# LiHaoy-ux/DQO-MAP

Hardware: AMD Instinct MI355X
Metric: mapping iters/sec (fwd+bwd raster) @ 500k Gaussians 1200×680; PSNR vs ref (higher is better)
Workload: dtype f32; 1 GPU; cfg3: surfel room, ONE map of 500000 Gaussians, 1200x680, 8 object ids, SH degree 3, per-object render (object gate) + per-object masked loss (sum over objects of 0.8 L1 colour + 1.0 depth L1 on the object's own mask) + attach loss, raster fwd+bwd + Adam (6 groups); path=fused (hipGraph replays of 4 iterations each); rccl_ranks=1, backend=none (one rank), list_split=0, list_split_backward=0, graph_unroll=4, sync_mode=lazy, selfcheck=skipped, P=500000, P_visible=196562, view=room, adam=exact-sparse, adam_rows_touched=148371, attach_loss_members=49997

## Files before the change

dqo-map_amd/_dqo_native.py:

```python
import ctypes
import os

_HERE = os.path.dirname(os.path.abspath(__file__))
LIB_PATH = os.path.join(_HERE, "lib", "libdqoraster.so")

c_f = ctypes.c_float
c_i32 = ctypes.c_int32
c_vp = ctypes.c_void_p


class DqoRastParams(ctypes.Structure):
    _fields_ = [("P", c_i32), ("D", c_i32), ("M", c_i32), ("W", c_i32), ("H", c_i32), ("prefiltered", c_i32), ("debug", c_i32),
                ("tanfovx", c_f), ("tanfovy", c_f), ("cx", c_f), ("cy", c_f), ("scale_modifier", c_f), ("color_sigma", c_f),
                ("opaque_threshold", c_f), ("depth_threshold", c_f), ("normal_threshold", c_f), ("T_threshold", c_f)]


class DqoRastInputs(ctypes.Structure):
    _fields_ = [(n, c_vp) for n in ("bg", "means3D", "shs", "colors_precomp", "opacities", "scales", "rotations", "cov3D_precomp",
                                    "viewmatrix", "projmatrix", "campos", "tile_mask", "row_flags")]


class DqoRastOutputs(ctypes.Structure):
    _fields_ = [(n, c_vp) for n in ("out_color", "out_depth", "out_hit_color", "out_hit_depth", "out_hit_color_weight",
                                    "out_hit_depth_weight", "out_T", "n_touched", "radii")]


class DqoLossTap(ctypes.Structure):
    _fields_ = [("gt_color", c_vp), ("gt_depth", c_vp), ("render_mask", c_vp), ("out_color", c_vp), ("out_depth", c_vp),
                ("color_weight", c_f), ("depth_weight", c_f), ("add_depth_thres", c_f), ("loss_out", c_vp), ("grad_scale", c_vp),
                ("per_object", c_i32)]


class DqoObjectGate(ctypes.Structure):
    _fields_ = [("gaussian_object", c_vp), ("pixel_object", c_vp), ("tile_objects", c_vp)]


class DqoRastCtx(ctypes.Structure):
    _fields_ = [("geom", c_vp), ("geom_bytes", ctypes.c_size_t), ("binning", c_vp), ("binning_bytes", ctypes.c_size_t),
                ("image", c_vp), ("image_bytes", ctypes.c_size_t), ("inst_capacity", ctypes.c_int64), ("tile_bucket_capacity", c_i32), ("keep_tile_order", c_i32), ("loss_tap", c_vp),
                ("object_gate", c_vp), ("list_split", c_i32), ("frame_prezeroed", c_i32)]


class DqoRastGrads(ctypes.Structure):
    _fields_ = [(n, c_vp) for n in ("dL_dmeans3D", "dL_dsh", "dL_dcolors", "dL_dopacity", "dL_dscales", "dL_drotations", "dL_dcov3D",
                                    "dL_dmeans2D")] + [("skip_culled_rows", c_i32)]


class DqoRastParamInputs(ctypes.Structure):
    _fields_ = [("features_dc", c_vp), ("features_rest", c_vp), ("rest", c_i32), ("opacity_raw", c_vp), ("scaling_raw", c_vp),
                ("rotation_raw", c_vp)]


class DqoRastParamGrads(ctypes.Structure):
    _fields_ = [(n, c_vp) for n in ("dL_dfeatures_dc", "dL_dfeatures_rest", "dL_dopacity_raw", "dL_dscaling_raw", "dL_drotation_raw")]


class DqoRastHeader(ctypes.Structure):
    _fields_ = [("num_rendered", ctypes.c_uint32), ("num_tiles", ctypes.c_uint32), ("overflow", ctypes.c_uint32),
                ("max_tile_count", ctypes.c_uint32), ("num_visible", ctypes.c_uint32), ("num_candidates", ctypes.c_uint32),
                ("stage", ctypes.c_uint32), ("reserved", ctypes.c_uint32)]


class DqoProfileEntry(ctypes.Structure):
    _fields_ = [("name", ctypes.c_char * 48), ("total_ms", ctypes.c_double), ("calls", ctypes.c_uint32)]


class DqoAdamStep(ctypes.Structure):
    _fields_ = ([("P", c_i32), ("M", c_i32), ("step", c_i32), ("beta1", c_f), ("beta2", c_f), ("eps", c_f), ("lr_xyz", c_f),
                 ("lr_f_dc", c_f), ("lr_f_rest", c_f), ("lr_opacity", c_f), ("lr_scaling", c_f), ("lr_rotation", c_f)] +
                [(n, c_vp) for n in ("xyz", "shs", "opacity_raw", "scaling_raw", "rotation_raw", "g_means3D", "g_sh", "g_opacity",
                                     "g_scales", "g_rotations", "m_xyz", "m_shs", "m_opacity", "m_scaling", "m_rotation", "v_xyz",
                                     "v_shs", "v_opacity", "v_scaling", "v_rotation", "act_opacity", "act_scales", "act_rotations", "radii", "step_dev", "moment_live",
                                     "attach_mask", "init_xyz", "init_scaling_raw", "init_rotation_raw")] +
                [("attach_count", c_i32), ("attach_partial", c_vp), ("frame_header", c_vp), ("block_ticket", c_vp), ("bias_table", c_vp), ("attach_gains", c_vp),
                 ("row_flags", c_vp), ("confidence", c_vp), ("lr_table", c_vp), ("record_ctx", c_vp), ("record_W", c_i32), ("record_H", c_i32)])

ROW_FROZEN, ROW_HIDDEN = 1, 2


class DqoAdamTensor(ctypes.Structure):
    _fields_ = [("p", c_vp), ("g", c_vp), ("m", c_vp), ("v", c_vp), ("n", ctypes.c_int64), ("lr", ctypes.c_double)]


class DqoLifecycle(ctypes.Structure):
    _fields_ = ([(n, c_i32) for n in ("P", "W", "H", "tick", "unstable_time_window", "delete_thresh", "stable_oversized", "use_votes")] +
                [(n, c_f) for n in ("stable_confidence_thres", "add_color_thres", "add_depth_thres")] +
                [(n, c_vp) for n in ("xyz", "opacity_raw", "scaling_raw", "confidence", "alive", "row_flags", "stable", "add_tick",
                                     "depth_error_counter", "color_error_counter", "park", "vote", "workspace")] +
                [("workspace_bytes", ctypes.c_size_t), ("stats", c_vp), ("render_header", c_vp)])


class DqoGrowthSample(ctypes.Structure):
    _fields_ = ([(n, c_i32) for n in ("W", "H", "first_frame", "uniform_sample_num", "capacity", "key_bits", "M", "identity_rotation")] +
                [("seed", ctypes.c_uint64)] +
                [(n, c_f) for n in ("add_transmission_thres", "add_depth_thres", "add_color_thres", "transmission_sample_ratio",
                                    "error_sample_ratio", "init_opacity")] +
                [(n, c_vp) for n in ("vertex", "normal", "color", "depth", "instance", "T", "render_depth", "render_color", "depth_index",
                                     "xyz", "scales", "rotations", "opacity", "shs", "obj_id", "out_normal", "pixel", "header", "workspace")] +
                [("workspace_bytes", ctypes.c_size_t)])


EXPORTS = ("dqo_abi_version", "dqo_abi_sizeof", "dqo_last_error", "dqo_profile_enable", "dqo_profile_collect", "dqo_map_activate",
           "dqo_map_loss_workspace_bytes", "dqo_map_loss_fwd_bwd", "dqo_map_ssim_workspace_bytes", "dqo_map_ssim_fwd_bwd", "dqo_map_adam_step", "dqo_adam_multi_dev", "dqo_map_attach_workspace_bytes",
           "dqo_map_attach_loss_fwd_bwd", "dqo_adam_multi", "dqo_accumulate_gaussian_error", "dqo_accumulate_gaussian_confidence", "dqo_rast_geom_bytes", "dqo_rast_image_bytes",
           "dqo_rast_binning_bytes", "dqo_rast_binning_bytes_bucketed",
           "dqo_rast_backward_workspace_bytes", "dqo_rast_forward_prepare", "dqo_rast_read_header", "dqo_rast_forward_render",
           "dqo_rast_forward", "dqo_rast_forward_async", "dqo_rast_backward", "dqo_rast_backward_adam", "dqo_mark_visible", "dqo_knn3_workspace_bytes", "dqo_knn3",
           "dqo_quadric_iou_fwd_bwd", "dqo_quadric_adam", "dqo_tile_count_mask", "dqo_transmission_mask", "dqo_tile_color_error", "dqo_knn3_query_workspace_bytes",
           "dqo_knn3_query", "dqo_knn3_query_within", "dqo_knn3_query_grouped", "dqo_icp_workspace_bytes", "dqo_icp_normal_equations",
           "dqo_attach_pixels", "dqo_attach_decide", "dqo_growth_scales", "dqo_growth_inside", "dqo_error_maps", "dqo_map_history_merge",
           "dqo_rast_forward_prepare_params", "dqo_rast_forward_render_params", "dqo_rast_forward_async_params", "dqo_rast_backward_params",
           "dqo_icp_gauss_newton", "dqo_track_preprocess_workspace_bytes", "dqo_track_preprocess", "dqo_track_pyramid_pixels",
           "dqo_track_pyramid_workspace_bytes", "dqo_track_pyramid", "dqo_track_fill_model_depth", "dqo_track_p2p_workspace_bytes",
           "dqo_track_p2p_loss", "dqo_map_lifecycle_workspace_bytes", "dqo_map_lifecycle_vote", "dqo_map_lifecycle_rows",
           "dqo_growth_sample_workspace_bytes", "dqo_growth_sample", "dqo_eval_picture_workspace_bytes", "dqo_eval_picture",
           "dqo_eval_ms_ssim_workspace_bytes", "dqo_eval_ms_ssim",
           "dqo_nn1_workspace_bytes", "dqo_nn1", "dqo_eval_pcd_workspace_bytes", "dqo_eval_pcd", "dqo_window_masks_workspace_bytes",
           "dqo_window_masks")

_lib = None


def lib():
    global _lib
    if _lib is None:
        import torch
        if not os.path.exists(LIB_PATH):
            raise RuntimeError(f"{LIB_PATH} not found: the HIP extension is not built (run __graft_entry__.build()). "
                               "There is no CPU fallback for this operator.")
        L = ctypes.CDLL(LIB_PATH)
        L.dqo_last_error.restype = ctypes.c_char_p
        for n in ("dqo_rast_geom_bytes", "dqo_rast_image_bytes", "dqo_rast_binning_bytes", "dqo_rast_backward_workspace_bytes",
                  "dqo_knn3_workspace_bytes"):
            getattr(L, n).restype = ctypes.c_size_t
        L.dqo_rast_geom_bytes.argtypes = [c_i32, c_i32, c_i32]
        L.dqo_rast_image_bytes.argtypes = [c_i32, c_i32]
        L.dqo_rast_binning_bytes.argtypes = [ctypes.c_int64]
        L.dqo_rast_binning_bytes_bucketed.restype = ctypes.c_size_t
        L.dqo_rast_binning_bytes_bucketed.argtypes = [ctypes.c_int64, c_i32, c_i32, c_i32]
        L.dqo_rast_backward_workspace_bytes.argtypes = [ctypes.c_int64]
        L.dqo_knn3_workspace_bytes.argtypes = [c_i32]
        P = ctypes.POINTER
        L.dqo_rast_forward_prepare.argtypes = [P(DqoRastParams), P(DqoRastInputs), P(DqoRastOutputs), P(DqoRastCtx), c_vp]
        L.dqo_rast_forward_render.argtypes = L.dqo_rast_forward_prepare.argtypes
        L.dqo_rast_forward.argtypes = L.dqo_rast_forward_prepare.argtypes
        L.dqo_rast_forward_async.argtypes = L.dqo_rast_forward_prepare.argtypes[:4] + [c_vp, c_vp, c_vp]
        L.dqo_rast_read_header.argtypes = [P(DqoRastCtx), P(DqoRastHeader), c_vp]
        L.dqo_rast_backward.argtypes = [P(DqoRastParams), P(DqoRastInputs), P(DqoRastCtx), c_vp, c_vp, c_vp, P(DqoRastGrads), c_vp,
                                        ctypes.c_size_t, c_vp]
        L.dqo_rast_backward_adam.argtypes = [P(DqoRastParams), P(DqoRastInputs), P(DqoRastCtx), c_vp, c_vp, P(DqoAdamStep), c_vp,
                                             ctypes.c_size_t, c_vp]
        L.dqo_rast_forward_prepare_params.argtypes = [P(DqoRastParams), P(DqoRastInputs), P(DqoRastParamInputs), P(DqoRastOutputs),
                                                      P(DqoRastCtx), c_vp]
        L.dqo_rast_forward_render_params.argtypes = L.dqo_rast_forward_prepare_params.argtypes
        L.dqo_rast_forward_async_params.argtypes = L.dqo_rast_forward_prepare_params.argtypes[:5] + [c_vp, c_vp, c_vp]
        L.dqo_rast_backward_params.argtypes = [P(DqoRastParams), P(DqoRastInputs), P(DqoRastParamInputs), P(DqoRastCtx), c_vp, c_vp, c_vp,
                                               P(DqoRastGrads), P(DqoRastParamGrads), c_vp, ctypes.c_size_t, c_vp]
        L.dqo_mark_visible.argtypes = [c_i32, c_vp, c_vp, c_vp, c_vp, c_vp]
        L.dqo_knn3.argtypes = [c_i32, c_vp, c_vp, c_vp, c_vp, ctypes.c_size_t, c_vp]
        L.dqo_quadric_iou_fwd_bwd.argtypes = [c_i32] + [c_vp] * 12
        L.dqo_quadric_adam.argtypes = [c_i32, c_i32] + [c_vp] * 9
        L.dqo_map_activate.argtypes = [c_i32] + [c_vp] * 7
        L.dqo_map_loss_workspace_bytes.restype = ctypes.c_size_t
        L.dqo_map_loss_workspace_bytes.argtypes = []
        L.dqo_map_ssim_workspace_bytes.restype = ctypes.c_size_t
        L.dqo_map_ssim_workspace_bytes.argtypes = [c_i32, c_i32]
        L.dqo_map_ssim_fwd_bwd.argtypes = [c_i32, c_i32, c_vp, c_vp, c_f, c_vp, c_vp, c_i32, c_vp, c_vp, ctypes.c_size_t, c_vp]
        L.dqo_map_loss_fwd_bwd.argtypes = [c_i32, c_i32] + [c_vp] * 6 + [c_f, c_f, c_f] + [c_vp] * 4 + [ctypes.c_size_t, c_vp]
        L.dqo_map_adam_step.argtypes = [P(DqoAdamStep), c_vp]
        L.dqo_map_attach_workspace_bytes.restype = ctypes.c_size_t
        L.dqo_map_attach_workspace_bytes.argtypes = [c_i32]
        L.dqo_adam_multi.argtypes = [c_vp, c_i32, c_i32, ctypes.c_double, ctypes.c_double, ctypes.c_double, c_vp]
        L.dqo_adam_multi_dev.argtypes = [c_vp, c_i32, c_vp, c_i32, ctypes.c_double, ctypes.c_double, ctypes.c_double, c_vp]
        L.dqo_map_attach_loss_fwd_bwd.argtypes = [c_i32] + [c_vp] * 7 + [c_i32] + [c_vp] * 5 + [ctypes.c_size_t, c_vp]
        L.dqo_accumulate_gaussian_error.argtypes = [c_i32] * 3 + [c_vp] * 5 + [c_f] * 3 + [c_i32] + [c_vp] * 6
        L.dqo_accumulate_gaussian_confidence.argtypes = [c_i32] * 3 + [c_vp] * 7
        L.dqo_knn3_query_workspace_bytes.restype = ctypes.c_size_t
        L.dqo_knn3_query_workspace_bytes.argtypes = [c_i32, c_i32]
        L.dqo_knn3_query.argtypes = [c_i32, c_vp, c_i32, c_vp, c_vp, c_vp, c_vp, ctypes.c_size_t, c_vp]
        L.dqo_knn3_query_within.argtypes = [c_i32, c_vp, c_i32, c_vp, c_f, c_vp, c_vp, c_vp, ctypes.c_size_t, c_vp]
        L.dqo_knn3_query_grouped.argtypes = [c_i32, c_vp, c_vp, c_i32, c_vp, c_vp, c_vp, c_f, c_vp, c_vp, c_vp, ctypes.c_size_t, c_vp]
        L.dqo_attach_pixels.argtypes = [c_i32, c_vp, c_vp, c_f, c_f, c_f, c_f, c_i32, c_i32] + [c_vp] * 5
        L.dqo_attach_decide.argtypes = [c_i32] + [c_vp] * 10 + [c_f, c_f, c_vp, c_vp]
        L.dqo_growth_scales.argtypes = [c_i32] + [c_vp] * 7 + [c_f, c_f, c_f, c_vp, c_vp, c_vp]
        L.dqo_growth_inside.argtypes = [c_i32] + [c_vp] * 5
        L.dqo_error_maps.argtypes = [c_i32, c_i32] + [c_vp] * 9
        L.dqo_icp_workspace_bytes.restype = ctypes.c_size_t
        L.dqo_icp_workspace_bytes.argtypes = []
        L.dqo_icp_normal_equations.argtypes = [c_i32, c_i32] + [c_vp] * 5 + [c_f] * 6 + [c_vp] * 4 + [ctypes.c_size_t, c_vp]
        L.dqo_icp_gauss_newton.argtypes = [c_i32, c_i32] + [c_vp] * 6 + [c_f] * 4 + [c_vp] * 2 + [ctypes.c_size_t, c_vp]
        L.dqo_track_preprocess_workspace_bytes.restype = ctypes.c_size_t
        L.dqo_track_preprocess_workspace_bytes.argtypes = [c_i32, c_i32]
        L.dqo_track_preprocess.argtypes = [c_i32, c_i32, c_vp, c_vp] + [c_f] * 3 + [c_i32] + [c_vp] * 6 + [ctypes.c_size_t, c_vp]
        L.dqo_track_pyramid_pixels.restype = ctypes.c_int64
        L.dqo_track_pyramid_pixels.argtypes = [c_i32, c_i32, c_i32]
        L.dqo_track_pyramid_workspace_bytes.restype = ctypes.c_size_t
        L.dqo_track_pyramid_workspace_bytes.argtypes = []
        L.dqo_track_pyramid.argtypes = [c_i32, c_i32, c_i32] + [c_vp] * 5 + [ctypes.c_size_t, c_vp]
        L.dqo_track_fill_model_depth.argtypes = [c_i32, c_i32] + [c_vp] * 4 + [c_f, c_f, c_vp]
        L.dqo_track_p2p_workspace_bytes.restype = ctypes.c_size_t
        L.dqo_track_p2p_workspace_bytes.argtypes = []
        L.dqo_track_p2p_loss.argtypes = [c_i32, c_i32] + [c_vp] * 4 + [c_f] + [c_vp] * 5 + [ctypes.c_size_t, c_vp]
        L.dqo_tile_count_mask.argtypes = [c_i32, c_i32, c_vp, c_vp, c_vp]
        L.dqo_transmission_mask.argtypes = [c_i32, c_i32, c_vp, c_vp, c_vp, c_vp, c_vp]
        L.dqo_tile_color_error.argtypes = [c_i32, c_i32, c_vp, c_vp, c_vp, c_vp, c_vp]
        L.dqo_window_masks_workspace_bytes.restype = ctypes.c_size_t
        L.dqo_window_masks_workspace_bytes.argtypes = [c_i32, c_i32]
        L.dqo_window_masks.argtypes = [c_i32, c_i32, c_i32, c_vp, c_vp, c_vp, c_f, c_i32, c_vp, c_vp, c_vp, c_vp, c_vp, ctypes.c_size_t, c_vp]
        L.dqo_map_history_merge.argtypes = [c_i32, c_i32, c_f, c_i32] + [c_vp] * 12
        L.dqo_map_lifecycle_workspace_bytes.restype = ctypes.c_size_t
        L.dqo_map_lifecycle_workspace_bytes.argtypes = [c_i32]
        L.dqo_map_lifecycle_vote.argtypes = [P(DqoLifecycle)] + [c_vp] * 7
        L.dqo_map_lifecycle_rows.argtypes = [P(DqoLifecycle), c_vp]
        L.dqo_growth_sample_workspace_bytes.restype = ctypes.c_size_t
        L.dqo_growth_sample_workspace_bytes.argtypes = [c_i32, c_i32]
        L.dqo_growth_sample.argtypes = [P(DqoGrowthSample), c_vp]
        L.dqo_eval_picture_workspace_bytes.restype = ctypes.c_size_t
        L.dqo_eval_picture_workspace_bytes.argtypes = [c_i32, c_i32]
        L.dqo_eval_picture.argtypes = [c_i32, c_i32] + [c_vp] * 5 + [c_f, c_f, c_vp, c_vp, c_i32, c_vp, ctypes.c_size_t, c_vp]
        L.dqo_eval_ms_ssim_workspace_bytes.restype = ctypes.c_size_t
        L.dqo_eval_ms_ssim_workspace_bytes.argtypes = [c_i32, c_i32]
        L.dqo_eval_ms_ssim.argtypes = [c_i32, c_i32, c_vp, c_vp, c_vp, c_vp, c_i32, c_vp, ctypes.c_size_t, c_vp]
        L.dqo_nn1_workspace_bytes.restype = ctypes.c_size_t
        L.dqo_nn1_workspace_bytes.argtypes = [c_i32, c_i32]
        L.dqo_nn1.argtypes = [c_i32, c_vp, c_vp, c_i32] + [c_vp] * 7 + [ctypes.c_size_t, c_vp]
        L.dqo_eval_pcd_workspace_bytes.restype = ctypes.c_size_t
        L.dqo_eval_pcd_workspace_bytes.argtypes = [c_i32, c_i32]
        L.dqo_eval_pcd.argtypes = [c_i32, c_vp, c_vp, c_i32, c_vp, c_vp, c_vp, c_i32, ctypes.POINTER(c_f), c_vp, c_i32, c_vp, ctypes.c_size_t, c_vp]
        L.dqo_profile_enable.argtypes = [ctypes.c_int]
        L.dqo_profile_collect.argtypes = [P(DqoProfileEntry), ctypes.c_int, ctypes.c_int]
        if L.dqo_abi_version() != 5:
            raise RuntimeError("libdqoraster.so ABI version mismatch")
        L.dqo_abi_sizeof.restype = ctypes.c_size_t
        L.dqo_abi_sizeof.argtypes = [c_i32]
        for k, st in enumerate((DqoRastParams, DqoRastInputs, DqoRastOutputs, DqoRastCtx, DqoRastGrads, DqoRastHeader, DqoProfileEntry,
                                DqoAdamStep, DqoLossTap, DqoObjectGate, DqoAdamTensor, DqoRastParamInputs, DqoRastParamGrads, None,
                                DqoLifecycle, DqoGrowthSample)):
            if st is not None and L.dqo_abi_sizeof(k) != ctypes.sizeof(st):
                raise RuntimeError(f"libdqoraster.so: struct {st.__name__} is {L.dqo_abi_sizeof(k)} bytes in the library, "
                                   f"{ctypes.sizeof(st)} in the binding")
        _lib = L
    return _lib


def check(rc):
    if rc != 0:
        raise RuntimeError(lib().dqo_last_error().decode() or f"libdqoraster error {rc}")


def ptr(t):
    if t is None or t.numel() == 0:
        return None
    return t.data_ptr()


def require_gpu(*tensors):
    for t in tensors:
        if t is not None and t.numel() > 0 and not t.is_cuda:
            raise RuntimeError("libdqoraster operators need GPU (ROCm) tensors; there is no CPU path. Got a tensor on "
                               f"{t.device}.")


def current_stream():
    import torch
    return torch.cuda.current_stream().cuda_stream


def profile_enable(on):
    lib().dqo_profile_enable(1 if on else 0)


def profile_collect(reset=True):
    buf = (DqoProfileEntry * 64)()
    n = lib().dqo_profile_collect(buf, 64, 1 if reset else 0)
    return {buf[i].name.decode(): (buf[i].total_ms, buf[i].calls) for i in range(n)}
```

dqo-map_amd/csrc/dqo_capi.hip:

```cpp
#include <stdarg.h>
#include <stdio.h>
#include <string.h>

#include "dqo_common.h"

static thread_local char g_err[512] = "";

void dqo_set_error(const char* fmt, ...) {
    va_list ap;
    va_start(ap, fmt);
    vsnprintf(g_err, sizeof(g_err), fmt, ap);
    va_end(ap);
}

int dqo_launch_mark_visible(int P, const float* means3D, const float* view, const float* proj, uint8_t* present, hipStream_t s);
int dqo_launch_knn3(int P, const float* xyz, float* mean_d2, int32_t* idx3, void* ws, size_t ws_bytes, hipStream_t s);
size_t dqo_knn3_ws_bytes(int P);
size_t dqo_knn3_query_ws_bytes(int Q, int R);
int dqo_launch_knn3_query(int Q, const float* q_xyz, int R, const float* r_xyz, float* dist2, int32_t* idx3, void* ws, size_t ws_bytes,
                          hipStream_t s, float bound2, const int32_t* q_group = nullptr, const int32_t* r_group = nullptr,
                          const float* group_box = nullptr);
int dqo_launch_quadric_iou(int B, const float* axes, const float* R, const float* center, const float* P34, const float* obs,
                           float* bbox, float* loss, int32_t* valid, float* g_axes, float* g_R, float* g_center, hipStream_t s);
int dqo_launch_quadric_adam(int n_obj, int n_iters, const int32_t* view_offset, const float* P34_views, const float* obs_views,
// ... 23 lines not shown
size_t dqo_icp_ws_bytes(void);
int dqo_launch_icp(int H, int W, const float* vertex0, const float* vertex1, const float* normal0, const float* normal1, const float* pose10,
                   float fx, float fy, float cx, float cy, float dist_thr, float normal_thr, float* JtJ, float* JtR, int32_t* valid_count,
                   void* ws, hipStream_t s);
int dqo_launch_icp_gauss_newton(int H, int W, const float* vertex0, const float* vertex1, const float* normal0, const float* normal1, float* pose10,
                                const float* K, float k_scale, float dist_thr, float normal_thr, float damping, int32_t* valid_count, void* ws,
                                hipStream_t s);
size_t dqo_track_preprocess_ws_bytes(int H, int W);
int dqo_launch_track_preprocess(int H, int W, const float* depth, const float* K, float min_depth, float max_depth,
                                float conf_thr, int filter, float* depth_out, float* vertex_out, float* normal_out, float* conf_out,
                                uint8_t* invalid_out, void* ws, hipStream_t s);
size_t dqo_track_pyramid_ws_bytes(void);
int64_t dqo_track_pyramid_pixel_count(int H, int W, int levels);
int dqo_launch_track_pyramid(int H, int W, int levels, const float* depth, const float* K, float* vertex, float* normal,
                             void* ws, hipStream_t s);
int dqo_launch_track_fill(int H, int W, float* render_depth, const float* frame_depth, const float* render_normal, const float* frame_normal,
                          float dist_thr, float normal_thr, hipStream_t s);
size_t dqo_track_p2p_ws_bytes(void);
int dqo_launch_track_p2p(int H, int W, const float* vertex0, const float* vertex1, const float* normal0, const float* pose10, float fail_thr,
                         const int32_t* valid_count, float* loss, int32_t* success, float* valid_ratio, void* ws, hipStream_t s);
int dqo_launch_tile_count(int W, int H, int mode, const uint8_t* mask_in, const float* T_map, uint8_t* mask_out, int32_t* tile_count,
                          int32_t* total, hipStream_t s);
int dqo_launch_tile_color_error(int W, int H, const float* render, const float* gt, float* err_px, float* tile_sum, hipStream_t s);
size_t dqo_window_masks_ws_bytes(int W, int H);
int dqo_launch_window_masks(int W, int H, int mode, const float* T_map, const float* render, const float* gt, float tile_mask_ratio, int k,
                            uint8_t* render_mask, int32_t* tile_mask, float* ratio_out, const DqoRastHeader* header, void* ws, hipStream_t s);
int dqo_launch_growth_scales(int n, const float* xyz, const int32_t* obj, const float* radius, const int32_t* i_new, const float* d2_old,
                             const int32_t* i_old, const float* extra_radius, float reach2, float min_radius, float max_radius, float* scales,
                             uint8_t* invalid, hipStream_t s);
int dqo_launch_growth_inside(int n, const float* d2, const int32_t* idx, const float* radius, uint8_t* inside, hipStream_t s);
int dqo_launch_error_maps(int64_t HW, const float* gt_color, const float* gt_depth, const float* render, const float* depth,
                          const int32_t* depth_index, const uint8_t* mask, float* color_err, float* depth_err, hipStream_t s);
size_t dqo_lifecycle_ws_bytes(int64_t P);
int dqo_launch_lifecycle_vote(const DqoLifecycle* a, const float* gt_color, const float* gt_depth, const float* render, const float* depth,
                              const int32_t* depth_index, const int32_t* color_index, hipStream_t s);
int dqo_launch_lifecycle_rows(const DqoLifecycle* a, hipStream_t s);
size_t dqo_sample_ws_bytes(int64_t HW);
int dqo_launch_growth_sample(const DqoGrowthSample* a, hipStream_t s);
size_t dqo_nn1_ws_bytes(int Q, int R);
int dqo_launch_nn1(int Q, const float* q_xyz, const uint8_t* q_keep, int R, const float* r_xyz, const uint8_t* r_keep, const float* q_xform,
                   const float* r_xform, float* dist2, int32_t* idx, void* ws, hipStream_t s);
size_t dqo_eval_pcd_ws_bytes(int n_gt, int n_rec);
int dqo_launch_eval_pcd(int n_gt, const float* gt_xyz, const uint8_t* gt_keep, int n_rec, const float* rec_xyz, const uint8_t* rec_keep,
                        const float* rec_xform, int n_thres, const float* thres, float* out_row, void* ws, hipStream_t s);
size_t dqo_eval_ws_bytes(int64_t HW);
size_t dqo_msssim_ws_bytes(int W, int H);
int dqo_launch_msssim(int W, int H, const float* render, const float* gt_color, const DqoRastHeader* header, float* out_row, void* ws,
                      hipStream_t s);
int dqo_launch_eval_picture(int W, int H, const float* render, const float* gt_color, const float* depth, const float* gt_depth,
                            const int32_t* depth_index, float min_depth, float max_depth, const DqoRastHeader* header, float* out_row,
                            void* ws, hipStream_t s);
int dqo_launch_attach_pixels(int n, const float* xyz, const float* V, float fx, float fy, float cx, float cy, int W, int H,
                             const int32_t* pixel_object, int32_t* lin, int32_t* sparse, unsigned long long* tile_objects, hipStream_t s);
int dqo_launch_attach_decide(int n, const float* xyz, const float* opacity, const int32_t* obj, const int32_t* lin, const int32_t* hit_index,
                             const float* hit_weight, const float* sxyz, const float* scaling_raw, const float* rotation_raw,
                             const int32_t* gobj, float plane_thr, float opacity_low, uint8_t* out, hipStream_t s);
int dqo_launch_tap_report(const DqoGeomLayout& g, const DqoTapDev& tap, hipStream_t s);
int dqo_launch_accumulate_confidence(int H, int W, int P, const int32_t* index, const float* confidence, float* gmax, float* gmin,
                                     float* gmean, int32_t* counter, hipStream_t s);
int dqo_launch_accumulate_error(int H, int W, int P, const float* color_err, const float* depth_err, const float* normal_err,
                                const int32_t* color_index, const int32_t* depth_index, float color_thr, float depth_thr,
                                float normal_thr, int check_max, float* gs_color, float* gs_depth, float* gs_normal, float* rescale,
                                int32_t* counters, hipStream_t s);

#include <map>
#include <mutex>
#include <string>
#include <vector>
int g_dqo_profile_on = 0;
namespace {
std::mutex g_profile_mu;
struct Pending {
    std::string name;
    hipEvent_t start, stop;
};
std::vector<Pending> g_pending;
std::vector<hipEvent_t> g_event_pool;
std::map<std::string, std::pair<double, uint32_t>> g_profile_acc;
hipEvent_t take_event() {
    if (!g_event_pool.empty()) {
        hipEvent_t e = g_event_pool.back();
        g_event_pool.pop_back();
        return e;
    }
    hipEvent_t e;
    (void)hipEventCreate(&e);
    return e;
}
}
static thread_local size_t t_pending_idx = 0;
void dqo_profile_before(const char* name, hipStream_t s) {
    std::lock_guard<std::mutex> lk(g_profile_mu);
    Pending p{name, take_event(), take_event()};
    (void)hipEventRecord(p.start, s);
    t_pending_idx = g_pending.size();
    g_pending.push_back(p);
}
void dqo_profile_after(hipStream_t s) {
    std::lock_guard<std::mutex> lk(g_profile_mu);
    if (t_pending_idx < g_pending.size()) (void)hipEventRecord(g_pending[t_pending_idx].stop, s);
}

extern "C" {

#define DQO_API __attribute__((visibility("default")))

DQO_API int dqo_profile_enable(int on) {
    g_dqo_profile_on = on ? 1 : 0;
    return DQO_OK;
}

DQO_API int dqo_profile_collect(DqoProfileEntry* out, int max_entries, int reset) {
    std::lock_guard<std::mutex> lk(g_profile_mu);
    for (auto& p : g_pending) {
        float ms = 0.f;
        if (hipEventSynchronize(p.stop) == hipSuccess && hipEventElapsedTime(&ms, p.start, p.stop) == hipSuccess) {
            auto& a = g_profile_acc[p.name];
            a.first += ms;
            a.second += 1;
        }
        g_event_pool.push_back(p.start);
        g_event_pool.push_back(p.stop);
    }
    g_pending.clear();
    int n = 0;
    for (auto& kv : g_profile_acc) {
        if (n >= max_entries || out == nullptr) break;
        strncpy(out[n].name, kv.first.c_str(), sizeof(out[n].name) - 1);
        out[n].name[sizeof(out[n].name) - 1] = 0;
        out[n].total_ms = kv.second.first;
        out[n].calls = kv.second.second;
        n++;
    }
    if (reset) g_profile_acc.clear();
    return n;
}

DQO_API int dqo_abi_version(void) { return DQO_ABI_VERSION; }
DQO_API size_t dqo_abi_sizeof(int32_t which) {
    static const size_t sz[] = {sizeof(DqoRastParams), sizeof(DqoRastInputs), sizeof(DqoRastOutputs), sizeof(DqoRastCtx), sizeof(DqoRastGrads),
                                sizeof(DqoRastHeader), sizeof(DqoProfileEntry), sizeof(DqoAdamStep), sizeof(DqoLossTap), sizeof(DqoObjectGate),
                                sizeof(DqoAdamTensor), sizeof(DqoRastParamInputs), sizeof(DqoRastParamGrads), 0 ,
                                sizeof(DqoLifecycle), sizeof(DqoGrowthSample)};
    return (which >= 0 && which < (int32_t)(sizeof(sz) / sizeof(sz[0]))) ? sz[which] : 0;
}
DQO_API const char* dqo_last_error(void) { return g_err; }

DQO_API size_t dqo_rast_geom_bytes(int32_t P, int32_t W, int32_t H) {
    (void)W;
    (void)H;
    return dqo_geom_layout(nullptr, P < 0 ? 0 : P).total;
}
DQO_API size_t dqo_rast_image_bytes(int32_t W, int32_t H) { return dqo_image_layout(nullptr, W, H).total; }
DQO_API size_t dqo_rast_binning_bytes(int64_t cap) { return dqo_bin_layout(nullptr, cap < 0 ? 0 : cap, cap < 0 ? 0 : cap, 0).total; }
DQO_API size_t dqo_rast_binning_bytes_bucketed(int64_t cap, int32_t W, int32_t H, int32_t bucket) {
    if (cap < 0) cap = 0;
    if (bucket <= 0 || W <= 0 || H <= 0) return dqo_rast_binning_bytes(cap);
    return dqo_bin_layout(nullptr, cap, dqo_list_cap(cap, W, H, bucket), bucket).total;
}
DQO_API size_t dqo_rast_backward_workspace_bytes(int64_t cap) { return dqo_bwd_ws_bytes(cap); }

static int check_common(const DqoRastParams* p, const DqoRastInputs* in, const DqoRastCtx* ctx) {
    DQO_CHECK_ARG(p && in && ctx, "null params / inputs / ctx");
    DQO_CHECK_ARG(p->P >= 0 && p->W > 0 && p->H > 0, "bad sizes P=%d W=%d H=%d", p->P, p->W, p->H);
    DQO_CHECK_ARG(p->D >= 0 && p->D <= 3, "sh degree %d out of range 0..3", p->D);
    DQO_CHECK_ARG((p->W + DQO_TILE - 1) / DQO_TILE < 65536 && (p->H + DQO_TILE - 1) / DQO_TILE < 65536, "image too large");
    DQO_CHECK_ARG(in->viewmatrix && in->projmatrix && in->campos && in->bg, "viewmatrix/projmatrix/campos/bg must be given");
    if (p->P > 0) {
        DQO_CHECK_ARG(in->means3D && in->opacities, "means3D / opacities missing");
        DQO_CHECK_ARG((in->shs != nullptr) != (in->colors_precomp != nullptr),
                      "Please provide excatly one of either SHs or precomputed colors!");
        DQO_CHECK_ARG(in->cov3D_precomp == nullptr,
                      "cov3D_precomp is not supported by the depth rasteriser: its blend kernel reads scales/rotations (forward.cu:780)");
        DQO_CHECK_ARG(in->scales && in->rotations, "scales and rotations are required");
        if (in->shs) DQO_CHECK_ARG(p->M >= (p->D + 1) * (p->D + 1), "sh has %d coefficients, degree %d needs %d", p->M, p->D, (p->D + 1) * (p->D + 1));
        if (in->colors_precomp == nullptr && p->M == 0) {
            dqo_set_error("For non-RGB, provide precomputed Gaussian colors!");
            return DQO_ERR_INVALID_ARG;
        }
    }
    DQO_CHECK_ARG(ctx->geom && ctx->geom_bytes >= dqo_rast_geom_bytes(p->P, p->W, p->H), "geom buffer too small (%zu < %zu)",
                  ctx->geom_bytes, dqo_rast_geom_bytes(p->P, p->W, p->H));
    DQO_CHECK_ARG(ctx->image && ctx->image_bytes >= dqo_rast_image_bytes(p->W, p->H), "image buffer too small (%zu < %zu)",
                  ctx->image_bytes, dqo_rast_image_bytes(p->W, p->H));
    return DQO_OK;
}

static int check_outputs(const DqoRastParams* p, const DqoRastOutputs* o) {
    DQO_CHECK_ARG(o, "null outputs");
    DQO_CHECK_ARG(o->out_color && o->out_depth && o->out_hit_color && o->out_hit_depth && o->out_hit_color_weight &&
                      o->out_hit_depth_weight && o->out_T,
                  "null image output");
    if (p->P > 0) DQO_CHECK_ARG(o->n_touched && o->radii, "null n_touched / radii");
    return DQO_OK;
}

DQO_API int dqo_rast_forward_prepare(const DqoRastParams* p, const DqoRastInputs* in, DqoRastOutputs* out, DqoRastCtx* ctx, void* stream) {
    int rc = check_common(p, in, ctx);
    if (rc) return rc;
    rc = check_outputs(p, out);
    if (rc) return rc;
    rc = dqo_launch_forward_prepare(p, in, out, ctx, (hipStream_t)stream);
    if (rc) return rc;
    return dqo_launch_mark_header_stage0(p, ctx, (hipStream_t)stream);
}

DQO_API int dqo_rast_read_header(const DqoRastCtx* ctx, DqoRastHeader* host_out, void* stream) {
    DQO_CHECK_ARG(ctx && ctx->geom && host_out, "null ctx / out");
    static thread_local uint32_t buf[128 + 64 * DQO_SPREAD];
    DQO_CHECK_HIP(hipMemcpyAsync(buf, ctx->geom, sizeof(buf), hipMemcpyDeviceToHost, (hipStream_t)stream));
    DQO_CHECK_HIP(hipStreamSynchronize((hipStream_t)stream));
    memcpy(host_out, buf, sizeof(DqoRastHeader));
    if (host_out->stage == 2u) return host_out->overflow ? DQO_ERR_OVERFLOW : DQO_OK;
    uint32_t nv = 0, nc = 0;
    for (int j = 0; j < DQO_SPREAD; j++) nv += buf[128 + 64 * j], nc += buf[128 + 64 * j + 1];
    memset(host_out, 0, sizeof(*host_out));
    host_out->stage = 1u;
    host_out->num_visible = nv;
    host_out->num_candidates = nc;
    return host_out->overflow ? DQO_ERR_OVERFLOW : DQO_OK;
}

static int check_render(const DqoRastParams* p, const DqoRastInputs* in, DqoRastOutputs* out, DqoRastCtx* ctx) {
    int rc = check_common(p, in, ctx);
    if (rc) return rc;
    rc = check_outputs(p, out);
    if (rc) return rc;
    DQO_CHECK_ARG(ctx->inst_capacity >= 0 && ctx->inst_capacity < (int64_t)0xffffffffll, "bad inst_capacity");
    DQO_CHECK_ARG(ctx->inst_capacity == 0 || ctx->binning, "null binning buffer");
    DQO_CHECK_ARG(ctx->tile_bucket_capacity >= 0, "negative tile_bucket_capacity");
    DQO_CHECK_ARG(ctx->loss_tap == nullptr || (ctx->loss_tap->gt_color && ctx->loss_tap->gt_depth && ctx->loss_tap->loss_out &&
                                               ctx->loss_tap->grad_scale), "loss tap with a null pointer");
    DQO_CHECK_ARG(ctx->object_gate == nullptr || (ctx->object_gate->gaussian_object && ctx->object_gate->pixel_object),
                  "object gate with a null pointer");
    DQO_CHECK_ARG(ctx->loss_tap == nullptr || !ctx->loss_tap->per_object || ctx->object_gate, "a per-object loss tap needs the object gate");
    if (ctx->binning_bytes < dqo_rast_binning_bytes_bucketed(ctx->inst_capacity, p->W, p->H, ctx->tile_bucket_capacity)) {
        dqo_set_error("binning buffer too small (%zu < %zu)", ctx->binning_bytes,
                      dqo_rast_binning_bytes_bucketed(ctx->inst_capacity, p->W, p->H, ctx->tile_bucket_capacity));
        return DQO_ERR_WORKSPACE;
    }
    return DQO_OK;
}

DQO_API int dqo_rast_forward_render(const DqoRastParams* p, const DqoRastInputs* in, DqoRastOutputs* out, DqoRastCtx* ctx, void* stream) {
    const int rc = check_render(p, in, out, ctx);
    if (rc) return rc;
    return dqo_launch_forward_render(p, in, out, ctx, (hipStream_t)stream);
}

DQO_API int dqo_rast_forward(const DqoRastParams* p, const DqoRastInputs* in, DqoRastOutputs* out, DqoRastCtx* ctx, void* stream) {
    int rc = check_render(p, in, out, ctx);
    if (rc) return rc;
    rc = dqo_launch_forward_prepare(p, in, out, ctx, (hipStream_t)stream);
    if (rc) return rc;
    return dqo_launch_forward_render(p, in, out, ctx, (hipStream_t)stream);
}

DQO_API int dqo_rast_forward_async(const DqoRastParams* p, const DqoRastInputs* in, DqoRastOutputs* out, DqoRastCtx* ctx,
                                   DqoRastHeader* header_host, void* header_event, void* stream) {
    int rc = check_render(p, in, out, ctx);
    if (rc) return rc;
    rc = dqo_launch_forward_prepare(p, in, out, ctx, (hipStream_t)stream);
    if (rc) return rc;
    return dqo_launch_forward_render(p, in, out, ctx, (hipStream_t)stream, header_host, (hipEvent_t)header_event);
}

static int rast_backward(const DqoRastParams* p, const DqoRastInputs* in, const DqoRastCtx* ctx, const float* dL_dcolor, const float* dL_ddepth,
                         const int32_t* hit_image, DqoRastGrads* g, void* ws, size_t ws_bytes, hipStream_t stream, const DqoShRest* pf,
                         float* dL_drest) {
    int rc = check_common(p, in, ctx);
    if (rc) return rc;
    DQO_CHECK_ARG(g, "null grads");
    if (p->P == 0) {
        if (ctx->loss_tap == nullptr) return DQO_OK;
        return dqo_launch_tap_report(dqo_geom_layout(ctx->geom, 0), dqo_tap_dev(ctx->loss_tap), (hipStream_t)stream);
    }
    DQO_CHECK_ARG((dL_dcolor && dL_ddepth) || ctx->loss_tap, "null upstream gradients");
    DQO_CHECK_ARG(ctx->loss_tap == nullptr || (ctx->loss_tap->gt_color && ctx->loss_tap->gt_depth && ctx->loss_tap->out_color &&
                                               ctx->loss_tap->out_depth && ctx->loss_tap->loss_out && ctx->loss_tap->grad_scale),
                  "loss tap with a null pointer");
    DQO_CHECK_ARG(g->dL_dmeans3D && g->dL_dopacity && g->dL_dscales && g->dL_drotations, "null gradient output");
    DQO_CHECK_ARG(p->M == 0 || g->dL_dsh, "null dL_dsh");
    DQO_CHECK_ARG(ctx->binning || ctx->inst_capacity == 0, "null binning buffer");
    if (ws_bytes < dqo_rast_backward_workspace_bytes(ctx->inst_capacity) || (ws == nullptr && ctx->inst_capacity > 0)) {
        dqo_set_error("backward workspace too small (%zu < %zu)", ws_bytes, dqo_rast_backward_workspace_bytes(ctx->inst_capacity));
        return DQO_ERR_WORKSPACE;
    }
    return dqo_launch_backward(p, in, ctx, dL_dcolor, dL_ddepth, hit_image, g, ws, ws_bytes, stream, pf, dL_drest);
}

DQO_API int dqo_rast_backward(const DqoRastParams* p, const DqoRastInputs* in, const DqoRastCtx* ctx, const float* dL_dcolor,
                              const float* dL_ddepth, const int32_t* hit_image, DqoRastGrads* g, void* ws, size_t ws_bytes, void* stream) {
    return rast_backward(p, in, ctx, dL_dcolor, dL_ddepth, hit_image, g, ws, ws_bytes, (hipStream_t)stream, nullptr, nullptr);
}

static int pf_inputs(const DqoRastParams* p, const DqoRastInputs* in, const DqoRastParamInputs* pin, DqoRastParams* p2, DqoRastInputs* in2,
                     DqoShRest* rest) {
    DQO_CHECK_ARG(p && in && pin, "null params / inputs / parameter inputs");
    DQO_CHECK_ARG(in->shs == nullptr && in->opacities == nullptr && in->scales == nullptr && in->rotations == nullptr,
                  "parameter form: DqoRastInputs.shs / opacities / scales / rotations must be NULL (they come from DqoRastParamInputs)");
    DQO_CHECK_ARG(in->colors_precomp == nullptr, "parameter form: colors_precomp is not supported");
    DQO_CHECK_ARG(pin->rest >= 0, "parameter form: negative rest coefficient count %d", pin->rest);
    DQO_CHECK_ARG(p->M == 1 + pin->rest, "parameter form: params M = %d, must be 1 + rest = %d", p->M, 1 + pin->rest);
    DQO_CHECK_ARG(p->D < 0 || p->D > 3 || 1 + pin->rest >= (p->D + 1) * (p->D + 1),
                  "parameter form: features_rest has %d coefficients, degree %d needs %d", pin->rest, p->D, (p->D + 1) * (p->D + 1) - 1);
    if (p->P > 0) {
// ... 610 lines not shown
```

dqo-map_amd/csrc/dqo_common.h:

```cpp
#pragma once
#include <hip/hip_runtime.h>
#include <stdint.h>

#include "../../include/dqo_raster.h"
#include "dqo_activate.h"

#define DQO_TILE 16
#define DQO_WAVE 64
#define DQO_SPREAD 64
#define DQO_GATE_OBJECTS 64
#define DQO_OBJ_SPREAD 16
#ifndef DQO_TSTRIDE
#define DQO_TSTRIDE 64
#endif

void dqo_set_error(const char* fmt, ...);
#define DQO_CHECK_ARG(cond, ...)          \
    do {                                  \
        if (!(cond)) {                    \
            dqo_set_error(__VA_ARGS__);   \
            return DQO_ERR_INVALID_ARG;   \
        }                                 \
    } while (0)
#define DQO_CHECK_HIP(expr)                                                          \
// ... 57 lines not shown
    float4* grad_sum;
    size_t total;
};

static inline DqoGeomLayout dqo_geom_layout(void* base, int64_t P) {
    DqoGeomLayout L;
    char* p = (char*)base;
    auto take = [&](size_t bytes) {
        char* r = p;
        p += dqo_align_up(bytes, 256);
        return r;
    };
    L.header = (DqoRastHeader*)take(256);
    L.counters = (uint32_t*)take(256);
    L.spread = (uint32_t*)take(256 * DQO_SPREAD);
    L.obj_tap = (unsigned long long*)take(sizeof(unsigned long long) * 4 * DQO_GATE_OBJECTS * DQO_OBJ_SPREAD);
    L.conic_opacity = (float4*)take(sizeof(float4) * P);
    L.xy_depth = (float4*)take(sizeof(float4) * P);
    L.rgb_smax = (float4*)take(sizeof(float4) * P);
    L.normal_c = (float4*)take(sizeof(float4) * P);
    L.point_c = (float4*)take(sizeof(float4) * P);
    L.drgb_dir = (float4*)take(sizeof(float4) * 3 * P);
    L.rect16 = (uint2*)take(sizeof(uint2) * P);
    L.tiles_touched = (uint32_t*)take(sizeof(uint32_t) * P);
    L.slot_base = (uint32_t*)take(sizeof(uint32_t) * P);
    L.clamped = (uint8_t*)take(P);
    L.grad_sum = (float4*)take(sizeof(float4) * 4 * P);
    L.total = (size_t)(p - (char*)base);
    return L;
}

struct DqoTapDev {
    const float* gt_color;
    const float* gt_depth;
    const uint8_t* mask;
    const float* out_color;
    const float* out_depth;
    float color_weight, depth_weight, add_depth_thres;
    float* loss_out;
    float* scale;
    int per_object;
};
struct DqoGateDev {
    const int32_t* gobj;
    const int32_t* pobj;
};
static inline DqoGateDev dqo_gate_dev(const DqoObjectGate* g) {
    DqoGateDev d;
    d.gobj = g ? g->gaussian_object : nullptr, d.pobj = g ? g->pixel_object : nullptr;
    return d;
}
static inline DqoTapDev dqo_tap_dev(const DqoLossTap* t) {
    DqoTapDev d;
    d.per_object = 0;
    if (t == nullptr) {
        d.gt_color = d.gt_depth = d.out_color = d.out_depth = nullptr, d.mask = nullptr, d.loss_out = d.scale = nullptr;
        d.color_weight = d.depth_weight = d.add_depth_thres = 0.f;
        return d;
    }
    d.per_object = t->per_object;
    d.gt_color = t->gt_color, d.gt_depth = t->gt_depth, d.mask = t->render_mask, d.out_color = t->out_color, d.out_depth = t->out_depth;
    d.color_weight = t->color_weight, d.depth_weight = t->depth_weight, d.add_depth_thres = t->add_depth_thres;
    d.loss_out = t->loss_out, d.scale = t->grad_scale;
    return d;
}
constexpr double DQO_TAP_FIXED = 4294967296.0;
#ifdef __HIPCC__
typedef unsigned dqo_swap_uint2 __attribute__((ext_vector_type(2)));
template <int D>
__device__ __forceinline__ uint32_t dqo_lane_xor(uint32_t x, int lane) {
    if constexpr (D == 1) return (uint32_t)__builtin_amdgcn_update_dpp(0, (int)x, 0xB1, 0xF, 0xF, false);
    else if constexpr (D == 2) return (uint32_t)__builtin_amdgcn_update_dpp(0, (int)x, 0x4E, 0xF, 0xF, false);
    else if constexpr (D == 4) {
        const int t = __builtin_amdgcn_update_dpp(0, (int)x, 0x104, 0xF, 0x5, false);
        return (uint32_t)__builtin_amdgcn_update_dpp(t, (int)x, 0x114, 0xF, 0xA, false);
    } else if constexpr (D == 8) return (uint32_t)__builtin_amdgcn_update_dpp(0, (int)x, 0x128, 0xF, 0xF, false);
    else if constexpr (D == 16) {
        const dqo_swap_uint2 r = __builtin_amdgcn_permlane16_swap(x, x, false, false);
        return (lane & 16) ? r.x : r.y;
    } else {
        static_assert(D == 32, "power of two up to 32");
        const dqo_swap_uint2 r = __builtin_amdgcn_permlane32_swap(x, x, false, false);
        return (lane & 32) ? r.x : r.y;
    }
}
__device__ __forceinline__ float dqo_wave_sum_xor(float x, int lane) {
    x += __uint_as_float(dqo_lane_xor<32>(__float_as_uint(x), lane));
    x += __uint_as_float(dqo_lane_xor<16>(__float_as_uint(x), lane));
    x += __uint_as_float(dqo_lane_xor<8>(__float_as_uint(x), lane));
    x += __uint_as_float(dqo_lane_xor<4>(__float_as_uint(x), lane));
    x += __uint_as_float(dqo_lane_xor<2>(__float_as_uint(x), lane));
    x += __uint_as_float(dqo_lane_xor<1>(__float_as_uint(x), lane));
    return x;
}
__device__ __forceinline__ uint32_t dqo_wave_max_u32(uint32_t x, int lane) {
    x = max(x, dqo_lane_xor<32>(x, lane)), x = max(x, dqo_lane_xor<16>(x, lane)), x = max(x, dqo_lane_xor<8>(x, lane));
    x = max(x, dqo_lane_xor<4>(x, lane)), x = max(x, dqo_lane_xor<2>(x, lane)), x = max(x, dqo_lane_xor<1>(x, lane));
    return x;
}
__device__ __forceinline__ uint32_t dqo_wave_sum_u32(uint32_t x, int lane) {
    x += dqo_lane_xor<32>(x, lane), x += dqo_lane_xor<16>(x, lane), x += dqo_lane_xor<8>(x, lane);
    x += dqo_lane_xor<4>(x, lane), x += dqo_lane_xor<2>(x, lane), x += dqo_lane_xor<1>(x, lane);
    return x;
}
template <int D>
__device__ __forceinline__ double dqo_lane_xor_f64(double x, int lane) {
    return __hiloint2double((int)dqo_lane_xor<D>((uint32_t)__double2hiint(x), lane), (int)dqo_lane_xor<D>((uint32_t)__double2loint(x), lane));
}
__device__ __forceinline__ double dqo_wave_sum_f64(double x, int lane) {
    x += dqo_lane_xor_f64<32>(x, lane), x += dqo_lane_xor_f64<16>(x, lane), x += dqo_lane_xor_f64<8>(x, lane);
    x += dqo_lane_xor_f64<4>(x, lane), x += dqo_lane_xor_f64<2>(x, lane), x += dqo_lane_xor_f64<1>(x, lane);
    return x;
}
__device__ __forceinline__ void dqo_tap_counts(const uint32_t* spread, int lane, uint32_t& n_col, uint32_t& n_dep) {
    uint32_t a = 0u, b = 0u;
    for (int j = lane; j < DQO_SPREAD; j += 64) {
        const unsigned long long* l = reinterpret_cast<const unsigned long long*>(spread + (size_t)j * 64 + 8);
        a += (uint32_t)l[1], b += (uint32_t)l[3];
    }
    n_col = dqo_wave_sum_u32(a, lane), n_dep = dqo_wave_sum_u32(b, lane);
}
__device__ __forceinline__ void dqo_tap_totals(const uint32_t* spread, int lane, double tot[4]) {
    unsigned long long t[4] = {0ull, 0ull, 0ull, 0ull};
    for (int j = lane; j < DQO_SPREAD; j += 64) {
        const unsigned long long* l = reinterpret_cast<const unsigned long long*>(spread + (size_t)j * 64 + 8);
#pragma unroll
        for (int c = 0; c < 4; c++) t[c] += l[c];
    }
#pragma unroll
    for (int off = 32; off > 0; off >>= 1)
#pragma unroll
        for (int c = 0; c < 4; c++) t[c] += (unsigned long long)__shfl_xor((long long)t[c], off);
    tot[0] = (double)t[0] / DQO_TAP_FIXED, tot[1] = (double)t[1], tot[2] = (double)t[2] / DQO_TAP_FIXED, tot[3] = (double)t[3];
}
__device__ __forceinline__ unsigned long long dqo_tap_fixed(float s) {
    return (s >= 0.f && s < 2147483648.f) ? (unsigned long long)((double)s * DQO_TAP_FIXED + 0.5) : ~0ull >> 1;
}
#endif

static inline int dqo_list_split(const DqoRastCtx* ctx) { return ctx->list_split <= 0 ? 0 : (ctx->list_split < 64 ? 64 : ctx->list_split); }
struct DqoImageLayout {
    uint32_t* tile_count;
    uint32_t* tile_flag;
    uint32_t* tile_cursor;
    uint2* ranges;
    uint32_t* walk4;
    uint32_t* tile_order;
    uint4* slot_info;
    float* final_T;
    uint32_t* n_contrib;
    uint32_t* hit_pos;
    uint32_t* long_tiles;
    uint32_t* split_tiles;
    size_t total;
};

static inline DqoImageLayout dqo_image_layout(void* base, int W, int H) {
    DqoImageLayout L;
    const size_t gx = (W + DQO_TILE - 1) / DQO_TILE, gy = (H + DQO_TILE - 1) / DQO_TILE;
    const size_t T = gx * gy, HW = (size_t)W * H;
    char* p = (char*)base;
    auto take = [&](size_t bytes) {
        char* r = p;
        p += dqo_align_up(bytes, 256);
        return r;
    };
    L.tile_count = (uint32_t*)take(4 * T * DQO_TSTRIDE);
    L.tile_flag = (uint32_t*)take(4 * T);
    L.tile_cursor = (uint32_t*)take(4 * T * DQO_TSTRIDE);
    L.ranges = (uint2*)take(8 * T);
    L.walk4 = (uint32_t*)take(16 * T);
    L.tile_order = (uint32_t*)take(4 * 8 * ((T + 7) / 8));
    L.slot_info = (uint4*)take(16 * 8 * ((T + 7) / 8));
    L.final_T = (float*)take(4 * HW);
    L.n_contrib = (uint32_t*)take(4 * HW);
    L.hit_pos = (uint32_t*)take(4 * HW);
    L.long_tiles = (uint32_t*)take(4 * T);
    L.split_tiles = (uint32_t*)take(4 * T);
    L.total = (size_t)(p - (char*)base);
    return L;
}

struct DqoBinLayout {
    uint4* recs;
    uint32_t* point_list;
    uint32_t* slot_list;
    uint8_t* live_q;
    uint2* slot_info;
    uint32_t* slot_gid;
    uint32_t* rec_valid;
    int64_t list_cap;
    int32_t bucket;
    size_t total;
};
static inline int64_t dqo_list_cap(int64_t cap, int W, int H, int bucket) {
    const int64_t T = (int64_t)((W + DQO_TILE - 1) / DQO_TILE) * ((H + DQO_TILE - 1) / DQO_TILE);
    return bucket > 0 ? T * bucket : cap;
}

static inline DqoBinLayout dqo_bin_layout(void* base, int64_t cap, int64_t list_cap, int bucket) {
    DqoBinLayout L;
    L.list_cap = list_cap, L.bucket = bucket;
    char* p = (char*)base;
    auto take = [&](size_t bytes) {
        char* r = p;
        p += dqo_align_up(bytes, 256);
        return r;
    };
    L.recs = (uint4*)take(16 * (size_t)list_cap);
    L.point_list = (uint32_t*)take(4 * (size_t)list_cap);
    L.slot_list = (uint32_t*)take(4 * (size_t)list_cap);
    L.live_q = (uint8_t*)take(4 * (size_t)list_cap);
    L.slot_info = (uint2*)take(8 * (size_t)cap);
    L.slot_gid = (uint32_t*)take(4 * (size_t)cap);
    L.rec_valid = (uint32_t*)take(4 * (size_t)cap);
    L.total = (size_t)(p - (char*)base);
    return L;
}

struct __attribute__((aligned(16))) DqoGradRec {
    float dcolor[3];
    float m1[2];
    float m2[3];
    float m0;
    float hit[5];
    float pad[2];
};
static_assert(sizeof(DqoGradRec) == 64, "record must be one 64-byte line");

static inline size_t dqo_bwd_recs_bytes(int64_t cap) { return dqo_align_up(sizeof(DqoGradRec) * 4 * (size_t)(cap < 0 ? 0 : cap), 256); }
static inline size_t dqo_bwd_ws_bytes(int64_t cap) { return dqo_bwd_recs_bytes(cap) + 256; }

__host__ __device__ static inline int dqo_spread_index(int logical, int P) {
    const int G = (P + 15) >> 4;
    const int rows = (G + 15) >> 4;
    const int L = logical >> 4;
    const int phys = (L & 15) * rows + (L >> 4);
    return phys < G ? phys * 16 + (logical & 15) : P;
}

static inline int dqo_spread_blocks(int P) {
    const int G = (P + 15) >> 4, rows = (G + 15) >> 4;
    return (rows * 16 * 16 + 255) / 256;
}

struct DqoView {
    const float* view;
    const float* proj;
    const float* campos;
    const float* bg;
    float tanfovx, tanfovy, focal_x, focal_y, cx, cy;
    float scale_mod, color_sigma, opaque_thr, depth_thr, normal_thr, T_thr;
    int W, H, gx, gy;
    int P, D, M;
    const uint8_t* row_flags;
};

struct DqoK1Late {
    DqoView v;
    const float *means3D, *scales, *rotations, *shs, *colors_precomp;
    int first_block;
};

static inline DqoView dqo_make_view(const DqoRastParams* p, const DqoRastInputs* in) {
    DqoView v;
    v.view = in->viewmatrix;
    v.row_flags = in->row_flags;
    v.proj = in->projmatrix;
    v.campos = in->campos;
    v.bg = in->bg;
    v.tanfovx = p->tanfovx;
    v.tanfovy = p->tanfovy;
    v.focal_y = p->H / (2.0f * p->tanfovy);
    v.focal_x = p->W / (2.0f * p->tanfovx);
    v.cx = p->cx;
    v.cy = p->cy;
    v.scale_mod = p->scale_modifier;
    v.color_sigma = p->color_sigma;
    v.opaque_thr = p->opaque_threshold;
    v.depth_thr = p->depth_threshold;
    v.normal_thr = p->normal_threshold;
    v.T_thr = p->T_threshold;
    v.W = p->W;
    v.H = p->H;
    v.gx = (p->W + DQO_TILE - 1) / DQO_TILE;
    v.gy = (p->H + DQO_TILE - 1) / DQO_TILE;
    v.P = p->P;
    v.D = p->D;
    v.M = p->M;
    return v;
}

static inline size_t dqo_frame_scalar_words(const DqoRastCtx* ctx) {
    const size_t obj_words = (ctx->loss_tap != nullptr && ctx->loss_tap->per_object)
                                 ? sizeof(unsigned long long) * 4 * DQO_GATE_OBJECTS * DQO_OBJ_SPREAD / 4 : 0;
    return (256 + 256 * DQO_SPREAD) / 4 + obj_words;
}

#define DQO_CLEARED_STAMP 0xC1EA5EDu
bool dqo_fuse_k1(const DqoRastParams* p, const DqoRastCtx* ctx);

__device__ __forceinline__ void dqo_header_from_spread(const DqoGeomLayout& g, int64_t capacity, int bucket, int lane) {
    uint32_t nv = 0, nc = 0, mx = 0, nt = 0, total = 0;
    for (int j = lane; j < DQO_SPREAD; j += 64) {
        const uint32_t* line = g.spread + (size_t)j * 64;
        nv += line[0], nc += line[1], mx = max(mx, line[2]), nt += line[3], total += line[4] + line[5];
    }
#pragma unroll
    for (int off = 32; off > 0; off >>= 1) {
        nv += __shfl_xor((int)nv, off), nc += __shfl_xor((int)nc, off), nt += __shfl_xor((int)nt, off);
        total += __shfl_xor((int)total, off);
        mx = max(mx, (uint32_t)__shfl_xor((int)mx, off));
    }
    if (lane == 0) {
        DqoRastHeader h;
        h.num_rendered = total;
        h.num_tiles = nt;
        (void)capacity;
        h.overflow = (g.counters[7] != 0u || g.counters[8] != 0u || mx > (uint32_t)bucket) ? 1u : 0u;
        h.max_tile_count = mx;
        h.num_visible = nv;
        h.num_candidates = nc;
        h.stage = 2u, h.reserved = 0u;
        *g.header = h;
    }
}

bool dqo_skip_long_sort(const DqoRastParams* p, const DqoRastCtx* ctx);

int dqo_launch_zero_words(uint32_t* p, size_t n_words, hipStream_t s);

int dqo_launch_bin_count_k1(const DqoView& v, const DqoRastInputs* in, const DqoRastOutputs* out, const int32_t* gobj, const DqoGeomLayout& g,
                            const DqoImageLayout& img, const DqoBinLayout& bin, int64_t capacity, const unsigned long long* tile_objects,
                            hipStream_t s, bool pf = false);
int dqo_launch_forward_prepare(const DqoRastParams* p, const DqoRastInputs* in, DqoRastOutputs* out, DqoRastCtx* ctx, hipStream_t s,
                               const DqoShRest* pf = nullptr);
int dqo_launch_mark_header_stage0(const DqoRastParams* p, DqoRastCtx* ctx, hipStream_t s);
int dqo_launch_forward_render(const DqoRastParams* p, const DqoRastInputs* in, DqoRastOutputs* out, DqoRastCtx* ctx, hipStream_t s,
                              DqoRastHeader* header_host = nullptr, hipEvent_t header_event = nullptr, const DqoShRest* pf = nullptr);
int dqo_launch_backward(const DqoRastParams* p, const DqoRastInputs* in, const DqoRastCtx* ctx, const float* dL_dcolor,
                        const float* dL_ddepth, const int32_t* hit_image, DqoRastGrads* g, void* ws, size_t ws_bytes, hipStream_t s,
                        const DqoShRest* pf = nullptr, float* dL_drest = nullptr);
```

dqo-map_amd/csrc/rast_binning.hip:

```cpp
#include "dqo_common.h"
#include "dqo_cull.h"
#include "dqo_k1_early.h"

namespace {

constexpr int BIN_THREADS = 256;
constexpr int BIN_CHUNK = BIN_THREADS;
constexpr int BIN_WINDOW = 16384;
constexpr int BIN_FLIGHT = 4;
#ifndef BIN_WAVES
#define BIN_WAVES 8
#endif

__device__ __forceinline__ uint32_t lane_id() { return __builtin_amdgcn_mbcnt_hi(~0u, __builtin_amdgcn_mbcnt_lo(~0u, 0u)); }

__device__ __forceinline__ uint32_t popcount_range(const uint32_t* bits, uint32_t a, uint32_t b) {
    if (a >= b) return 0;
    uint32_t wa = a >> 5, wb = (b - 1) >> 5;
    const uint32_t ma = ~0u << (a & 31), mb = ~0u >> (31 - ((b - 1) & 31));
    if (wa == wb) return __popc(bits[wa] & ma & mb);
    uint32_t n = __popc(bits[wa] & ma) + __popc(bits[wb] & mb);
    for (uint32_t w = wa + 1; w < wb; w++) n += __popc(bits[w]);
    return n;
}

__device__ __forceinline__ uint32_t block_exclusive_scan(uint32_t v, uint32_t* s_wave, uint32_t lane, uint32_t wave, uint32_t* total) {
    uint32_t incl = v;
    incl += (uint32_t)__builtin_amdgcn_update_dpp(0, (int)incl, 0x111, 0xF, 0xF, false);
    incl += (uint32_t)__builtin_amdgcn_update_dpp(0, (int)incl, 0x112, 0xF, 0xF, false);
    incl += (uint32_t)__builtin_amdgcn_update_dpp(0, (int)incl, 0x114, 0xF, 0xF, false);
    incl += (uint32_t)__builtin_amdgcn_update_dpp(0, (int)incl, 0x118, 0xF, 0xF, false);
    incl += (uint32_t)__builtin_amdgcn_update_dpp(0, (int)incl, 0x142, 0xA, 0xF, false);
    incl += (uint32_t)__builtin_amdgcn_update_dpp(0, (int)incl, 0x143, 0xC, 0xF, false);
    __syncthreads();
    if (lane == 63) s_wave[wave] = incl;
    __syncthreads();
    uint32_t wbase = 0, tot = 0;
#pragma unroll
    for (uint32_t w = 0; w < BIN_THREADS / 64; w++) {
        const uint32_t t = s_wave[w];
        if (w < wave) wbase += t;
        tot += t;
    }
    *total = tot;
    return wbase + incl - v;
}

struct Cand {
    int gi, tile;
};

struct DqoK1Raw {
    DqoView v;
    const float *means3D, *scales, *rotations, *opacities;
    const int32_t* gobj;
    int32_t *radii_out, *n_touched_out;
};

template <bool K1, bool PF>
__global__ __launch_bounds__(BIN_THREADS, BIN_WAVES) void bin_count_kernel(int P, int gx, const int32_t* __restrict__ tile_mask, DqoGeomLayout g,
                                                                uint32_t* __restrict__ tile_count, uint32_t* __restrict__ tile_flag,
                                                                DqoBinLayout bin, int64_t capacity,
                                                                const unsigned long long* __restrict__ tile_objects, const DqoK1Raw k1,
                                                                const uint8_t* __restrict__ row_flags) {
    static_assert(K1 || !PF, "the parameter form only differs in the early part");
    __shared__ uint32_t s_off[BIN_CHUNK + 1];
    __shared__ uint2 s_rect[BIN_CHUNK];
    __shared__ float4 s_con[BIN_CHUNK];
    __shared__ float4 s_xyq[BIN_CHUNK];
    __shared__ uint32_t s_cnt[BIN_CHUNK];
    __shared__ uint32_t s_prev[BIN_CHUNK];
    __shared__ uint32_t s_gb[BIN_CHUNK];
    __shared__ uint32_t s_bits[BIN_WINDOW / 32];
    __shared__ uint32_t s_wave[BIN_THREADS / 64];
    __shared__ uint32_t s_base;
    __shared__ int s_gobj[BIN_CHUNK];
    const int tid = threadIdx.x;
    const uint32_t lane = lane_id(), wave = tid >> 6;
    const int chunk0 = blockIdx.x * BIN_CHUNK;
    const int my_idx = dqo_spread_index(chunk0 + tid, P);

    uint32_t area = 0;
    {
        uint2 rc = make_uint2(0u, 0u);
        float4 co = make_float4(0.f, 0.f, 0.f, 0.f), xy = co;
        if constexpr (K1) {
            float view[16], proj[16];
#pragma unroll
            for (int i = 0; i < 16; i++) view[i] = k1.v.view[i], proj[i] = k1.v.proj[i];
            if (blockIdx.x == 0 && tid == 0) {
                g.header->stage = 1u;
                if (g.counters[9] != DQO_CLEARED_STAMP) atomicOr(&g.counters[8], 1u);
                g.counters[9] = 0u;
            }
            bool vis = false;
            uint32_t ncand = 0;
            if (my_idx < P) {
                const K1Early e = k1_early<false, PF>(k1.v, view, proj, 0.f, 0.f, 0.f, my_idx, k1.means3D, k1.scales, k1.rotations, k1.opacities,
                                                  nullptr, nullptr, k1.gobj, g, k1.radii_out, k1.n_touched_out, DqoShRest{});
                rc = make_uint2((uint32_t)e.rminx | ((uint32_t)e.rmaxx << 16), (uint32_t)e.rminy | ((uint32_t)e.rmaxy << 16));
                co = e.co, xy = e.xy;
                ncand = (uint32_t)((e.rmaxx - e.rminx) * (e.rmaxy - e.rminy));
                area = ncand;
                vis = e.radius > 0;
            }
            const uint32_t nv = (uint32_t)__popcll(__builtin_amdgcn_ballot_w64(vis));
            const uint32_t nc = dqo_wave_sum_u32(ncand, (int)lane);
            if (lane == 0 && (nv | nc) != 0u) {
                uint32_t* const my_line = g.spread + (size_t)((blockIdx.x * (BIN_THREADS / 64) + wave) % DQO_SPREAD) * 64;
                if (nv) atomicAdd(&my_line[0], nv);
                if (nc) atomicAdd(&my_line[1], nc);
            }
        } else if (my_idx < P) {
            rc = g.rect16[my_idx];
            co = g.conic_opacity[my_idx];
            xy = g.xy_depth[my_idx];
            area = ((rc.x >> 16) - (rc.x & 0xffffu)) * ((rc.y >> 16) - (rc.y & 0xffffu));
        }
        s_rect[tid] = rc;
        if (area) {
            s_con[tid] = co;
            s_xyq[tid] = make_float4(xy.x, xy.y, dqo_q_threshold(co.w), xy.z);
            s_gobj[tid] = __float_as_int(xy.w);
        }
        s_cnt[tid] = 0;
        s_prev[tid] = 0;
    }
    uint32_t total;
    const uint32_t my_off = block_exclusive_scan(area, s_wave, lane, wave, &total);
    s_off[tid] = my_off;
    if (tid == BIN_THREADS - 1) s_off[BIN_CHUNK] = total;
    __syncthreads();
    if (total == 0) {
        if (my_idx < P) g.tiles_touched[my_idx] = 0, g.slot_base[my_idx] = 0;
        return;
    }

    auto decode = [&](uint32_t w) {
        int lo = 0, hi = BIN_CHUNK;
        while (hi - lo > 1) {
            const int mid = (lo + hi) >> 1;
            if (s_off[mid] <= w) lo = mid;
            else hi = mid;
        }
        const uint32_t r = w - s_off[lo];
        const uint2 rc = s_rect[lo];
        const uint32_t minx = rc.x & 0xffffu, rw = (rc.x >> 16) - minx, miny = rc.y & 0xffffu;
        const uint32_t ry = r / rw, rx = r - ry * rw;
        Cand c;
        c.gi = lo;
        c.tile = (int)((miny + ry) * (uint32_t)gx + minx + rx);
        return c;
    };
    auto cull_window = [&](uint32_t win, uint32_t wend, bool flag_dead) {
        for (int i = tid; i < BIN_WINDOW / 32; i += BIN_THREADS) s_bits[i] = 0;
        __syncthreads();
        for (uint32_t w = win + tid; w < wend; w += BIN_THREADS) {
            const Cand c = decode(w);
            if (tile_mask != nullptr && !tile_mask[c.tile]) continue;
            const float4 co = s_con[c.gi], xyq = s_xyq[c.gi];
            const int x = c.tile % gx, y = c.tile / gx;
            bool live = dqo_splat_hits_rect(xyq.x, xyq.y, co.x, co.y, co.z, xyq.z, (float)(x * DQO_TILE), (float)(y * DQO_TILE),
                                            (float)(x * DQO_TILE + DQO_TILE - 1), (float)(y * DQO_TILE + DQO_TILE - 1));
            if (tile_objects != nullptr) live = live && ((tile_objects[c.tile] >> (s_gobj[c.gi] & 63)) & 1ull) != 0ull;
            if (live) {
                atomicOr(&s_bits[(w - win) >> 5], 1u << ((w - win) & 31));
            } else if (flag_dead && tile_flag[c.tile] == 0u) {
                tile_flag[c.tile] = 1u;
            }
        }
        __syncthreads();
    };
    auto carry_window = [&](uint32_t win, uint32_t wend, uint32_t* acc) {
        const uint32_t a = max(my_off, win), b = min(my_off + area, wend);
        if (a < b) acc[tid] += popcount_range(s_bits, a - win, b - win);
    };

    const bool one_window = total <= (uint32_t)BIN_WINDOW;
    for (uint32_t win = 0; win < total; win += BIN_WINDOW) {
        const uint32_t wend = min(total, win + (uint32_t)BIN_WINDOW);
        cull_window(win, wend, true);
        carry_window(win, wend, s_cnt);
        if (!one_window) __syncthreads();
    }
    const bool no_slots = bin.bucket > 0 && row_flags != nullptr && my_idx < P && (row_flags[my_idx] & DQO_ROW_FROZEN) != 0u;
    const uint32_t my_cnt = no_slots ? 0u : s_cnt[tid];
    __shared__ uint8_t s_noslot[BIN_CHUNK];
    s_noslot[tid] = no_slots ? (uint8_t)1 : (uint8_t)0;
    if (row_flags != nullptr && bin.bucket > 0) {
        const uint32_t nf = dqo_wave_sum_u32(no_slots ? s_cnt[tid] : 0u, (int)lane);
        if (lane == 0 && nf != 0u) atomicAdd(&g.spread[(size_t)((blockIdx.x * (BIN_THREADS / 64) + wave) % DQO_SPREAD) * 64 + 5], nf);
    }
    uint32_t block_live;
    const uint32_t my_gb = block_exclusive_scan(my_cnt, s_wave, lane, wave, &block_live);
    s_gb[tid] = my_gb;
    if (tid == 0) {
        if (block_live == 0u) {
            s_base = 0u;
        } else if (bin.bucket <= 0) {
            s_base = atomicAdd(&g.counters[0], block_live);
        } else {
            const uint32_t regions = min((uint32_t)DQO_SPREAD, max(1u, gridDim.x / 16u));
            const uint32_t r = blockIdx.x % regions, share = (uint32_t)(capacity / regions);
            const uint32_t off = atomicAdd(&g.spread[(size_t)r * 64 + 4], block_live);
            if (off + block_live > share) {
                g.counters[7] = 1u;
                s_base = (uint32_t)capacity;
            } else {
                s_base = r * share + off;
            }
        }
    }
    __syncthreads();
    const uint32_t base = s_base;
    if (my_idx < P) {
        g.tiles_touched[my_idx] = my_cnt;
        g.slot_base[my_idx] = base + my_gb;
    }
    if (block_live == 0) return;
    if (bin.bucket > 0) {
        for (uint32_t i = tid; i < block_live; i += BIN_THREADS)
            if ((int64_t)(base + i) < capacity) bin.rec_valid[base + i] = 0u;
    }

    for (uint32_t win = 0; win < total; win += BIN_WINDOW) {
        const uint32_t wend = min(total, win + (uint32_t)BIN_WINDOW);
        if (!one_window) cull_window(win, wend, false);
        for (uint32_t w0 = win + tid; w0 < wend; w0 += BIN_THREADS * BIN_FLIGHT) {
            uint32_t slot[BIN_FLIGHT], rank[BIN_FLIGHT];
            int tile[BIN_FLIGHT], gid[BIN_FLIGHT];
            float depth[BIN_FLIGHT];
            bool ok[BIN_FLIGHT];
#pragma unroll
            for (int u = 0; u < BIN_FLIGHT; u++) {
                const uint32_t w = w0 + u * BIN_THREADS;
                ok[u] = w < wend && ((s_bits[(w - win) >> 5] >> ((w - win) & 31)) & 1u);
                if (ok[u]) {
                    const Cand c = decode(w);
                    const uint32_t first = max(s_off[c.gi], win);
                    slot[u] = s_noslot[c.gi] ? 0xffffffffu : base + s_gb[c.gi] + s_prev[c.gi] + popcount_range(s_bits, first - win, w - win);
                    tile[u] = c.tile;
                    gid[u] = dqo_spread_index(chunk0 + c.gi, P);
                    depth[u] = s_xyq[c.gi].w;
                    rank[u] = atomicAdd(&tile_count[(size_t)c.tile * DQO_TSTRIDE], 1u);
                }
            }
#pragma unroll
            for (int u = 0; u < BIN_FLIGHT; u++) {
                if (ok[u] && ((int64_t)slot[u] < capacity || slot[u] == 0xffffffffu)) {
                    if (bin.bucket > 0) {
                        if (rank[u] < (uint32_t)bin.bucket) {
                            const size_t pos = (size_t)tile[u] * (size_t)bin.bucket + rank[u];
                            bin.recs[pos] = make_uint4((uint32_t)gid[u], __float_as_uint(depth[u]), slot[u], 0u);
                        }
                    } else {
                        bin.slot_info[slot[u]] = make_uint2((uint32_t)tile[u], rank[u]);
                        bin.slot_gid[slot[u]] = (uint32_t)gid[u];
                    }
                }
            }
        }
        if (!one_window) {
            __syncthreads();
            carry_window(win, wend, s_prev);
            __syncthreads();
        }
    }
}

__global__ __launch_bounds__(256) void bin_place_kernel(DqoGeomLayout g, DqoImageLayout img, DqoBinLayout bin, int64_t capacity) {
    const int64_t slot = (int64_t)blockIdx.x * blockDim.x + threadIdx.x;
    const int64_t n = min((int64_t)g.counters[0], capacity);
    if (slot >= n) return;
    const uint2 info = bin.slot_info[slot];
    const uint32_t gid = bin.slot_gid[slot];
    const uint2 range = img.ranges[info.x];
    const uint32_t pos = range.x + info.y;
    if (pos >= range.y) {
        bin.rec_valid[slot] = 0u;
        return;
    }
    bin.recs[pos] = make_uint4(gid, __float_as_uint(g.xy_depth[gid].z), (uint32_t)slot, 0u);
    bin.rec_valid[slot] = 0u;
}

}

int dqo_launch_bin_count(int P, int gx, const int32_t* tile_mask, const DqoGeomLayout& g, const DqoImageLayout& img, const DqoBinLayout& bin,
                         int64_t capacity, const unsigned long long* tile_objects, hipStream_t s, const uint8_t* row_flags) {
    DqoK1Raw none{};
    DQO_LAUNCH("bin_count_kernel", (bin_count_kernel<false, false>), dim3(dqo_spread_blocks(P)), dim3(BIN_THREADS), s, P, gx, tile_mask, g,
               img.tile_count, img.tile_flag, bin, capacity, tile_objects, none, row_flags);
    return DQO_OK;
}

int dqo_launch_bin_count_k1(const DqoView& v, const DqoRastInputs* in, const DqoRastOutputs* out, const int32_t* gobj, const DqoGeomLayout& g,
                            const DqoImageLayout& img, const DqoBinLayout& bin, int64_t capacity, const unsigned long long* tile_objects,
                            hipStream_t s, bool pf) {
    DqoK1Raw k1;
    k1.v = v, k1.means3D = in->means3D, k1.scales = in->scales, k1.rotations = in->rotations, k1.opacities = in->opacities;
    k1.gobj = gobj, k1.radii_out = out->radii, k1.n_touched_out = out->n_touched;
#define DQO_BIN_K1(PF)                                                                                                                \
    DQO_LAUNCH(PF ? "bin_count_pf_kernel" : "bin_count_kernel", (bin_count_kernel<true, PF>), dim3(dqo_spread_blocks(v.P)), dim3(BIN_THREADS), \
               s, v.P, v.gx, in->tile_mask, g, img.tile_count, img.tile_flag, bin, capacity, tile_objects, k1, v.row_flags)
    if (pf) DQO_BIN_K1(true);
    else DQO_BIN_K1(false);
#undef DQO_BIN_K1
    return DQO_OK;
}

int dqo_launch_bin_place(const DqoGeomLayout& g, const DqoImageLayout& img, const DqoBinLayout& bin, int64_t capacity, hipStream_t s) {
    if (capacity <= 0) return DQO_OK;
    DQO_LAUNCH("bin_place_kernel", bin_place_kernel, dim3((unsigned)((capacity + 255) / 256)), dim3(256), s, g, img, bin, capacity);
    return DQO_OK;
}
```

dqo-map_amd/csrc/rast_forward.hip:

```cpp
#include <cstdlib>

#include "dqo_common.h"
#include "dqo_cull.h"
#include "dqo_gauss_chain.h"
#include "dqo_k1_early.h"

#ifndef K1_WAVES
#define K1_WAVES 4
#endif
#ifndef SORTW_WAVES
#define SORTW_WAVES 7
#endif
#ifndef SORTW_LATE_WAVES
#define SORTW_LATE_WAVES 4
#endif
namespace {

__device__ __forceinline__ uint32_t lane_id() { return __builtin_amdgcn_mbcnt_hi(~0u, __builtin_amdgcn_mbcnt_lo(~0u, 0u)); }

constexpr int K1_THREADS = 256;
constexpr int K1_ITEMS = 1;

template <bool LATE, bool PF>
__global__ __launch_bounds__(K1_THREADS, K1_WAVES) void preprocess_kernel(const DqoView v, const float* __restrict__ means3D,
// ... 400 lines not shown
    else if (n <= 256) wave_sort_tile<4>(bin, rg.x, n, lane);
    else wave_sort_tile<8>(bin, rg.x, n, lane);
}

constexpr int SORTL_SEG = 4096;
constexpr int SORTL_RUN = SORTP_RUN;

template <bool LATE, bool PF>
__global__ __launch_bounds__(SORT_THREADS, LATE ? 4 : 6) void tile_sort_kernel(int T, DqoImageLayout img, DqoBinLayout bin, DqoGeomLayout g, int64_t capacity,
                                                                 int keep_order, const DqoK1Late late, const DqoFormArg<PF, DqoShRest> rest_arg) {
    static_assert(LATE || !PF, "the parameter form only differs in the late part");
    DqoShRest rest{};
    if constexpr (PF) rest = rest_arg;
    if constexpr (LATE) {
        if ((int)blockIdx.x >= late.first_block) {
            k1_late_block<SORT_THREADS, PF>(late, g, (int)blockIdx.x - late.first_block, rest);
            return;
        }
    }
    const uint32_t sort_blocks = LATE ? (uint32_t)late.first_block : gridDim.x;
    __shared__ uint64_t s_keys[SORTL_SEG];
    __shared__ uint32_t s_vals[SORTL_SEG];
    if (keep_order && blockIdx.x == 0 && threadIdx.x < 64) dqo_header_from_spread(g, capacity, bin.bucket, (int)threadIdx.x);
    const int tid = threadIdx.x, wave = tid >> 6, lane = tid & 63;
    const uint32_t n_long = min(g.counters[1], (uint32_t)T);
    for (uint32_t q = blockIdx.x; q < n_long; q += sort_blocks) {
    const uint32_t tile = img.long_tiles[q];
    const uint2 rg = img.ranges[tile];
    const int n = (int)(rg.y - rg.x);
    uint4* gr = bin.recs + rg.x;
    int n2 = 2 * SORTL_RUN;
    while (n2 < n) n2 <<= 1;
    const int seg_len = min(n2, SORTL_SEG);

    auto lds_step = [&](int k, int j, bool flip) {
        for (int t = tid; t < seg_len / 2; t += SORT_THREADS) {
            int i, p;
            if (flip) {
                const int h = k >> 1, blk = t / h, off = t - blk * h;
                i = blk * k + off, p = blk * k + k - 1 - off;
            } else {
                i = 2 * j * (t / j) + (t % j), p = i + j;
            }
            const uint64_t a = s_keys[i], b = s_keys[p];
            if (a > b) {
                s_keys[i] = b, s_keys[p] = a;
                const uint32_t va = s_vals[i];
                s_vals[i] = s_vals[p], s_vals[p] = va;
            }
        }
        __syncthreads();
    };
    auto runs_in_registers = [&](bool full_sort) {
        for (int run = wave; run < seg_len / SORTL_RUN; run += SORT_THREADS / 64) {
            uint64_t key[SORTP_E];
            uint32_t val[SORTP_E];
            const int base = run * SORTL_RUN + lane * SORTP_E;
#pragma unroll
            for (int r = 0; r < SORTP_E; r++) key[r] = s_keys[base + r], val[r] = s_vals[base + r];
            if (full_sort) wave_bitonic<SORTP_E>(key, val, lane);
            else wave_bitonic_phase<SORTP_E>(key, val, lane, 2 * SORTL_RUN);
#pragma unroll
            for (int r = 0; r < SORTP_E; r++) s_keys[base + r] = key[r], s_vals[base + r] = val[r];
        }
        __syncthreads();
    };
    auto load_segment = [&](int s0) {
        for (int i = tid; i < seg_len; i += SORT_THREADS) {
            const bool in = s0 + i < n;
            const uint4 e = in ? gr[s0 + i] : make_uint4(~0u, ~0u, 0u, 0u);
            s_keys[i] = ((uint64_t)e.y << 32) | e.x;
            s_vals[i] = e.z;
        }
        __syncthreads();
    };
    auto store_segment = [&](int s0, bool final_lists) {
        for (int i = tid; i < seg_len; i += SORT_THREADS) {
            if (s0 + i >= n) continue;
            if (final_lists) {
                bin.point_list[rg.x + s0 + i] = (uint32_t)(s_keys[i] & 0xffffffffu);
                bin.slot_list[rg.x + s0 + i] = s_vals[i];
            } else {
                gr[s0 + i] = make_uint4((uint32_t)s_keys[i], (uint32_t)(s_keys[i] >> 32), s_vals[i], 0u);
            }
        }
        __syncthreads();
    };
    const int nseg = n2 / seg_len;
    for (int sg = 0; sg < nseg; sg++) {
        load_segment(sg * seg_len);
        runs_in_registers(true);
        for (int k = 2 * SORTL_RUN; k <= seg_len; k <<= 1) {
            lds_step(k, 0, true);
            for (int j = k >> 2; j >= SORTL_RUN; j >>= 1) lds_step(k, j, false);
            runs_in_registers(false);
        }
        store_segment(sg * seg_len, nseg == 1);
    }
    for (int k = 2 * seg_len; k <= n2 && nseg > 1; k <<= 1) {
        for (int j = k >> 1; j >= seg_len; j >>= 1) {
            const bool flip = j == (k >> 1);
            for (int t = tid; t < n2 / 2; t += SORT_THREADS) {
                int i, p;
                if (flip) {
                    const int blk = t / j, off = t - blk * j;
                    i = blk * k + off, p = blk * k + k - 1 - off;
                } else {
                    i = 2 * j * (t / j) + (t % j), p = i + j;
                }
                if (p < n) {
                    const uint4 a = gr[i], b = gr[p];
                    if ((((uint64_t)a.y << 32) | a.x) > (((uint64_t)b.y << 32) | b.x)) gr[i] = b, gr[p] = a;
                }
            }
            __syncthreads();
        }
        const bool last = (k << 1) > n2;
        for (int sg = 0; sg < nseg; sg++) {
            if (sg * seg_len >= n) break;
            load_segment(sg * seg_len);
            for (int j = seg_len >> 1; j >= SORTL_RUN; j >>= 1) lds_step(2 * j, j, false);
            runs_in_registers(false);
            store_segment(sg * seg_len, last);
        }
    }
    }
}

__global__ void zero_words_kernel(uint32_t* __restrict__ p, size_t n) {
    const size_t i = (size_t)blockIdx.x * blockDim.x + threadIdx.x;
    if (i < n) p[i] = 0u;
}

__global__ void mark_visible_kernel(int P, const float* __restrict__ means3D, const float* __restrict__ view,
                                    const float* __restrict__ proj, uint8_t* __restrict__ present) {
#pragma clang fp contract(off)
    const int idx = blockIdx.x * blockDim.x + threadIdx.x;
    if (idx >= P) return;
    const float px = means3D[3 * idx], py = means3D[3 * idx + 1], pz = means3D[3 * idx + 2];
    const float hx = proj[0] * px + proj[4] * py + proj[8] * pz + proj[12];
    const float hy = proj[1] * px + proj[5] * py + proj[9] * pz + proj[13];
    const float hw = proj[3] * px + proj[7] * py + proj[11] * pz + proj[15];
    const float p_w = 1.0f / (hw + 0.0000001f);
    const float projx = hx * p_w, projy = hy * p_w;
    const float tvz = view[2] * px + view[6] * py + view[10] * pz + view[14];
    present[idx] = !(tvz <= 0.2f || (double)projx < -1.3 || (double)projx > 1.3 || (double)projy < -1.3 || (double)projy > 1.3);
}

}

int dqo_launch_blend_forward(const DqoView& v, const DqoGeomLayout& g, const DqoImageLayout& img, const DqoBinLayout& bin,
                             const DqoRastOutputs& out, int T, const DqoTapDev& tap, const DqoGateDev& gate, int list_split, hipStream_t s,
                             int64_t header_capacity);
int dqo_launch_bin_count(int P, int gx, const int32_t* tile_mask, const DqoGeomLayout& g, const DqoImageLayout& img, const DqoBinLayout& bin,
                         int64_t capacity, const unsigned long long* tile_objects, hipStream_t s, const uint8_t* row_flags);
int dqo_launch_bin_place(const DqoGeomLayout& g, const DqoImageLayout& img, const DqoBinLayout& bin, int64_t capacity, hipStream_t s);

int dqo_launch_zero_words(uint32_t* p, size_t n_words, hipStream_t s) {
    if (n_words == 0) return DQO_OK;
    DQO_LAUNCH("zero_words_kernel", zero_words_kernel, dim3((unsigned)((n_words + 255) / 256)), dim3(256), s, p, n_words);
    return DQO_OK;
}

int dqo_launch_forward_prepare(const DqoRastParams* p, const DqoRastInputs* in, DqoRastOutputs* out, DqoRastCtx* ctx, hipStream_t s,
                               const DqoShRest* pf) {
    const DqoView v = dqo_make_view(p, in);
    DqoGeomLayout g = dqo_geom_layout(ctx->geom, p->P);
    DqoImageLayout img = dqo_image_layout(ctx->image, p->W, p->H);
    const int T = v.gx * v.gy;
    if (!(ctx->frame_prezeroed != 0 && p->P > 0)) {
        int rc = dqo_launch_zero_words(reinterpret_cast<uint32_t*>(g.header), 256 / 4 + dqo_frame_scalar_words(ctx), s);
        if (rc) return rc;
    }
    const size_t zero_words = (size_t)((img.tile_flag + T) - img.tile_count);
    if (p->P <= 0) {
        int rc = dqo_launch_zero_words(img.tile_count, zero_words, s);
        if (rc) return rc;
    }
    if (p->P > 0 && !dqo_fuse_k1(p, ctx)) {
        const int per_block = K1_THREADS * K1_ITEMS;
        const int grid = (p->P + per_block - 1) / per_block;
        const int32_t* gobj = ctx->object_gate ? ctx->object_gate->gaussian_object : nullptr;
        const int prez = ctx->frame_prezeroed != 0 ? 1 : 0;
        const DqoShRest rest = pf != nullptr ? *pf : DqoShRest{};
#define DQO_K1(LATE, PF)                                                                                                                \
    DQO_LAUNCH(PF ? "preprocess_pf_kernel" : "preprocess_kernel", (preprocess_kernel<LATE, PF>), dim3(grid), dim3(K1_THREADS), s, v,     \
               in->means3D, in->scales, in->rotations, in->opacities, in->shs, dqo_form_arg<!PF>(in->colors_precomp), in->tile_mask, g, \
               out->radii, out->n_touched, img.tile_count, zero_words, gobj, prez, dqo_form_arg<PF>(rest))
        const bool late_here = dqo_k1_where(p->P) == 0;
        if (pf != nullptr) {
            if (late_here) DQO_K1(true, true);
            else DQO_K1(false, true);
        } else {
            if (late_here) DQO_K1(true, false);
            else DQO_K1(false, false);
        }
#undef DQO_K1
    }
    return DQO_OK;
}

int dqo_launch_forward_render(const DqoRastParams* p, const DqoRastInputs* in, DqoRastOutputs* out, DqoRastCtx* ctx, hipStream_t s,
                              DqoRastHeader* header_host, hipEvent_t header_event, const DqoShRest* pf) {
    const DqoView v = dqo_make_view(p, in);
    DqoGeomLayout g = dqo_geom_layout(ctx->geom, p->P);
    DqoImageLayout img = dqo_image_layout(ctx->image, p->W, p->H);
    const int bucket = ctx->tile_bucket_capacity;
    const int64_t cap = (int64_t)ctx->inst_capacity;
    DqoBinLayout bin = dqo_bin_layout(ctx->binning, cap, dqo_list_cap(cap, p->W, p->H, bucket), bucket);
    const int T = v.gx * v.gy;
    if (p->P > 0) {
        const unsigned long long* tobj = ctx->object_gate ? reinterpret_cast<const unsigned long long*>(ctx->object_gate->tile_objects) : nullptr;
        int rc = dqo_fuse_k1(p, ctx) ? dqo_launch_bin_count_k1(v, in, out, ctx->object_gate ? ctx->object_gate->gaussian_object : nullptr, g, img,
                                                               bin, cap, tobj, s, pf != nullptr)
                                     : dqo_launch_bin_count(p->P, v.gx, in->tile_mask, g, img, bin, cap, tobj, s, v.row_flags);
        if (rc) return rc;
    }
    const int keep_order = (bucket > 0 && ctx->keep_tile_order != 0 && p->P > 0) ? 1 : 0;
    if (!keep_order) DQO_LAUNCH("tile_scan_kernel", tile_scan_kernel, dim3(1), dim3(SCAN_THREADS), s, T, img, g, cap, bucket);
    if (p->P > 0) {
        if (bucket <= 0) {
            int rc = dqo_launch_bin_place(g, img, bin, cap, s);
            if (rc) return rc;
        }
        const int slots = 8 * ((T + 7) / 8);
        DqoK1Late late;
        late.v = v, late.means3D = in->means3D, late.scales = in->scales, late.rotations = in->rotations, late.shs = in->shs;
        late.colors_precomp = in->colors_precomp, late.first_block = slots;
        const DqoShRest rest = pf != nullptr ? *pf : DqoShRest{};
        const int where = dqo_k1_where(p->P);
        const int late_w = where == 1 ? (p->P + SORTW_THREADS - 1) / SORTW_THREADS : 0;
#define DQO_SORTW(LATE, PF)                                                                                                          \
    DQO_LAUNCH(PF ? "tile_sort_wave_pf_kernel" : "tile_sort_wave_kernel", (tile_sort_wave_kernel<LATE, PF>), dim3(slots + late_w), \
               dim3(SORTW_THREADS), s, T, img, bin, g, cap, keep_order, dqo_list_split(ctx), late, dqo_form_arg<PF>(rest))
        if (where == 1 && pf != nullptr) DQO_SORTW(true, true);
        else if (where == 1) DQO_SORTW(true, false);
        else DQO_SORTW(false, false);
#undef DQO_SORTW
        if (dqo_skip_long_sort(p, ctx)) {
        } else {
            if (where == 2) late.first_block = SORT_GRID;
            const int late_l = where == 2 ? (p->P + SORT_THREADS - 1) / SORT_THREADS : 0;
#define DQO_SORTL(LATE, PF)                                                                                                 \
    DQO_LAUNCH(PF ? "tile_sort_pf_kernel" : "tile_sort_kernel", (tile_sort_kernel<LATE, PF>), dim3(SORT_GRID + late_l), \
               dim3(SORT_THREADS), s, T, img, bin, g, cap, keep_order, late, dqo_form_arg<PF>(rest))
            if (where == 2 && pf != nullptr) DQO_SORTL(true, true);
            else if (where == 2) DQO_SORTL(true, false);
            else DQO_SORTL(false, false);
#undef DQO_SORTL
        }
    }
    const bool header_in_blend = dqo_skip_long_sort(p, ctx);
    auto hand_over_header = [&]() -> int {
        if (header_host != nullptr) DQO_CHECK_HIP(hipMemcpyAsync(header_host, g.header, sizeof(DqoRastHeader), hipMemcpyDeviceToHost, s));
        if (header_event != nullptr) DQO_CHECK_HIP(hipEventRecord(header_event, s));
        return DQO_OK;
    };
    if (!header_in_blend) {
        const int rc = hand_over_header();
        if (rc) return rc;
    }
    const int rc = dqo_launch_blend_forward(v, g, img, bin, *out, T, dqo_tap_dev(ctx->loss_tap), dqo_gate_dev(ctx->object_gate),
                                            dqo_list_split(ctx), s, header_in_blend ? cap : (int64_t)-1);
    if (rc) return rc;
    return header_in_blend ? hand_over_header() : DQO_OK;
}

int dqo_launch_mark_header_stage0(const DqoRastParams* p, DqoRastCtx* ctx, hipStream_t s) {
    if (!dqo_fuse_k1(p, ctx)) return DQO_OK;
    DqoGeomLayout g = dqo_geom_layout(ctx->geom, p->P);
    return dqo_launch_zero_words(&g.header->stage, 1, s);
}

bool dqo_skip_long_sort(const DqoRastParams* p, const DqoRastCtx* ctx) {
    return p->P > 0 && ctx->tile_bucket_capacity > 0 && ctx->tile_bucket_capacity <= SORTW_CAP && ctx->keep_tile_order != 0 &&
           dqo_k1_where(p->P) != 2 && dqo_list_split(ctx) == 0;
}

bool dqo_fuse_k1(const DqoRastParams* p, const DqoRastCtx* ctx) {
    static const bool on = [] {
        const char* e = getenv("DQO_K1_FUSE");
        return !(e != nullptr && e[0] == '0');
    }();
    return on && ctx->frame_prezeroed != 0 && p->P > 0 && ctx->tile_bucket_capacity > 0 && dqo_k1_where(p->P) != 0;
}

int dqo_launch_mark_visible(int P, const float* means3D, const float* view, const float* proj, uint8_t* present, hipStream_t s) {
    if (P <= 0) return DQO_OK;
    DQO_LAUNCH("mark_visible_kernel", mark_visible_kernel, dim3((P + 255) / 256), dim3(256), s, P, means3D, view, proj, present);
    return DQO_OK;
}
```

dqo-map_amd/diff_gaussian_rasterization_depth/__init__.py:

```python
import ctypes
from typing import NamedTuple

import torch
import torch.nn as nn

import _dqo_native as N

import threading
import weakref

_lock = threading.RLock()
_list_split = 0
_sync_mode = "exact"
_cap_hint = {}
_pending = []
_last = {"num_rendered": None, "num_visible": None, "header": None}
_ring = {}
_RING = 64
_pool = {}
_pool_on = True
_POOL_SETS = 3
_POOL_KEYS = 4
_shape_hint = {}


class _CtxSet:
    __slots__ = ("geom", "img", "binning", "cap", "bucket", "order_valid", "clean", "leased",
                 "captured")


class _Lease:
    __slots__ = ("set",)

    def __init__(self, s):
        self.set = s
        s.leased = True

    def __del__(self):
        self.set.leased = False


class _Pinned:
    __slots__ = ("set",)

    def __init__(self, s):
        self.set = s
        s.leased = True


_captured = []


def take_captured_contexts():
    with _lock:
        out = list(_captured)
        del _captured[:]
    return out


def set_context_pool(on):
    global _pool_on
    with _lock:
        _pool_on = bool(on)
        if not _pool_on:
            _pool.clear()


def _bucket_for(longest):
    b = 256
    while b < 2 * longest:
        b *= 2
    if b == 2048 and 1.3 * longest <= 1024:
        b = 1024
    return b


def _pooled_set(lib, key, stream, dev, W, H, pin=False):
    if not _pool_on:
        return None
    hint = _shape_hint.get(key)
    if hint is None or hint[1] <= 0:
        return None
    cap, bucket = int(hint[0] * 1.25) + 4096, _bucket_for(hint[1])
    if pin:
        for pkey, sets in _pool.items():
            if (pkey[0],) + pkey[2:] != key:
                continue
            for cs in sets:
                if not cs.leased and cs.cap >= cap and cs.bucket >= bucket:
                    sets.remove(cs)
                    return cs
    pkey = (key[0], stream) + key[1:]
    sets = _pool.pop(pkey, [])
    _pool[pkey] = sets
    while len(_pool) > _POOL_KEYS:
        del _pool[next(iter(_pool))]
    for cs in sets:
        if not cs.leased and cs.cap >= cap and cs.bucket >= bucket:
            return cs
    sets[:] = [cs for cs in sets if cs.leased or (cs.cap >= cap and cs.bucket >= bucket)]
    if len(sets) >= _POOL_SETS:
        return None
    u8 = dict(dtype=torch.uint8, device=dev)
    cs = _CtxSet()
    cs.cap, cs.bucket = int(cap * 1.2), bucket
    cs.geom = torch.empty((lib.dqo_rast_geom_bytes(key[1], W, H),), **u8)
    cs.img = torch.empty((lib.dqo_rast_image_bytes(W, H),), **u8)
    cs.binning = torch.empty((lib.dqo_rast_binning_bytes_bucketed(cs.cap, W, H, cs.bucket),), **u8)
    cs.order_valid = cs.clean = cs.leased = False
    if not pin:
        sets.append(cs)
    return cs


def _ring_slot(dev_index):
    ring, pos = _ring.setdefault(dev_index, ([], [0]))
    if len(ring) < _RING:
        host, ev = torch.empty((8,), dtype=torch.int32).pin_memory(), torch.cuda.Event()
        host.zero_()
        ev.record()
        ring.append((host, ev, host.data_ptr(), ev.cuda_event))
        return ring[-1]
    pos[0] = (pos[0] + 1) % _RING
    slot = ring[pos[0]]
    if any(p[1] is slot[0] for p in _pending):
        _verify_pending(block=True)
    return slot


def last_header():
    hd = _last["header"]
    if hd is None:
        return None
    if torch.is_tensor(hd):
        h = hd[:32].view(torch.int32).cpu().tolist()
        return dict(num_rendered=h[0], num_tiles=h[1], overflow=h[2], max_tile_count=h[3], num_visible=h[4], num_candidates=h[5])
    ev, host = hd
    ev.synchronize()
    h = host.tolist()
    return dict(num_rendered=h[0], num_tiles=h[1], overflow=h[2], max_tile_count=h[3], num_visible=h[4], num_candidates=h[5])


def last_num_rendered():
    return _last["num_rendered"]


def set_list_split(longer_than):
    global _list_split
    if int(longer_than) < 0:
        raise ValueError("list_split is 0 (off) or a list length")
    _list_split = int(longer_than)


def set_sync_mode(mode):
    global _sync_mode
    if mode not in ("exact", "lazy", "deferred", "graph"):
        raise ValueError(mode)
    if _pending:
        _verify_pending(block=True)
    _sync_mode = mode
    if mode == "exact":
        with _lock:
            _pool.clear()


def set_capacity(P, W, H, instances, device_index=None):
    dev_index = torch.cuda.current_device() if device_index is None else int(device_index)
    key = (dev_index, int(P), int(W), int(H))
    with _lock:
        _cap_hint[key] = max(_cap_hint.get(key, 0), int(instances))


def verify_pending():
    _verify_pending(block=True)


def _verify_pending(block):
    err = None
    with _lock:
        keep = []
        for i, (ev, host, key, cap, pooled) in enumerate(_pending):
            if not block and not ev.query():
                keep.append((ev, host, key, cap, pooled))
                continue
            ev.synchronize()
            n, overflow = int(host[0]), int(host[2])
            _cap_hint[key] = max(_cap_hint.get(key, 0), int(n * 1.25) + 4096)
            sh = _shape_hint.setdefault(key, [0, 0])
            sh[0], sh[1] = max(sh[0], int(host[5])), max(sh[1], int(host[3]))
            if overflow and pooled:
                sh[0] = max(sh[0], int(cap * 1.2))
            if overflow:
                keep.extend(_pending[i + 1:])
                err = (n, cap, pooled)
                break
        _pending[:] = keep
    if err is not None and err[2]:
        raise RuntimeError(f"diff_gaussian_rasterization_depth (lazy mode, pooled context): a previous forward produced {err[0]} "
                           f"Gaussian-tile instances or a tile list that did not fit its context ({err[1]} instance slots in per-tile "
                           "buckets); its outputs are invalid. The sizes have been raised — re-run that iteration (or use "
                           "set_sync_mode('exact')).")
    if err is not None:
        raise RuntimeError(f"diff_gaussian_rasterization_depth (lazy mode): a previous forward produced {err[0]} Gaussian-tile "
                           f"instances but only {err[1]} fitted its binning buffer; its outputs are invalid. The capacity has "
                           "been raised — re-run that iteration (or use set_sync_mode('exact')).")


_gate_checked = {}


def _check_gate_ids(gaussian_object, pixel_object):
    if _sync_mode == "graph":
        return
    for t, lo_ok in ((gaussian_object, False), (pixel_object, True)):
        hit = _gate_checked.get(id(t))
        if hit is not None and hit[0]() is t and hit[1] == t._version:
            continue
        if t.numel():
            mn, mx = int(t.min().item()), int(t.max().item())
            if mx > 63 or (mn < 0 and not lo_ok):
                raise RuntimeError("object gate: object ids must lie in [0, 64) (negative pixel ids = no owner); got "
                                   f"[{mn}, {mx}] in {'pixel_object' if lo_ok else 'gaussian_object'}")
        key = id(t)
        _gate_checked[key] = (weakref.ref(t, lambda _r, k=key: _gate_checked.pop(k, None)), t._version)


def gate_ids_checked(t):
    key = id(t)
    _gate_checked[key] = (weakref.ref(t, lambda _r, k=key: _gate_checked.pop(k, None)), t._version)


def _f32(t, name):
    if t.dtype != torch.float32:
        raise RuntimeError(f"expected scalar type Float but found {t.dtype} ({name})")
    return t.contiguous()


def rasterize_gaussians(means3D, sh, colors_precomp, opacities, scales, rotations, cov3Ds_precomp, tile_mask, raster_settings):
    return _RasterizeGaussians.apply(means3D, sh, colors_precomp, opacities, scales, rotations, cov3Ds_precomp, tile_mask,
                                     raster_settings)


def rasterize_gaussians_gated(means3D, sh, colors_precomp, opacities, scales, rotations, cov3Ds_precomp, tile_mask, raster_settings,
                              gaussian_object, pixel_object, tile_objects=None):
    return _RasterizeGaussians.apply(means3D, sh, colors_precomp, opacities, scales, rotations, cov3Ds_precomp, tile_mask,
                                     raster_settings, gaussian_object, pixel_object, tile_objects)


def _params(rs, P, M):
    return N.DqoRastParams(P=P, D=int(rs.sh_degree), M=M, W=int(rs.image_width), H=int(rs.image_height),
                           prefiltered=int(bool(rs.prefiltered)), debug=int(bool(rs.debug)), tanfovx=float(rs.tanfovx),
                           tanfovy=float(rs.tanfovy), cx=float(rs.cx), cy=float(rs.cy), scale_modifier=float(rs.scale_modifier),
                           color_sigma=float(rs.color_sigma), opaque_threshold=float(rs.opaque_threshold),
                           depth_threshold=float(rs.depth_threshold), normal_threshold=float(rs.normal_threshold),
                           T_threshold=float(rs.T_threshold))


def _inputs(rs, means3D, sh, colors_precomp, opacities, scales, rotations, cov3Ds_precomp, tile_mask, row_flags=None):
    return N.DqoRastInputs(bg=N.ptr(rs.bg), means3D=N.ptr(means3D), shs=N.ptr(sh), colors_precomp=N.ptr(colors_precomp),
                           opacities=N.ptr(opacities), scales=N.ptr(scales), rotations=N.ptr(rotations),
                           cov3D_precomp=N.ptr(cov3Ds_precomp), viewmatrix=N.ptr(rs.viewmatrix), projmatrix=N.ptr(rs.projmatrix),
                           campos=N.ptr(rs.campos), tile_mask=N.ptr(tile_mask), row_flags=N.ptr(row_flags))


def _new_outputs(P, H, W, device):
    f32, i32 = dict(dtype=torch.float32, device=device), dict(dtype=torch.int32, device=device)
    out = (torch.empty((3, H, W), **f32), torch.empty((1, H, W), **f32), torch.empty((1, H, W), **i32), torch.empty((1, H, W), **i32),
           torch.empty((1, H, W), **f32), torch.empty((1, H, W), **f32), torch.empty((1, H, W), **f32), torch.empty((P,), **i32),
           torch.empty((P,), **i32))
    return out, N.DqoRastOutputs(*(N.ptr(t) for t in out))


def _forward_call(lib, stage, params, inputs, pinputs, outputs, cctx, *rest):
    if pinputs is None:
        return getattr(lib, "dqo_rast_forward_" + stage)(ctypes.byref(params), ctypes.byref(inputs), ctypes.byref(outputs),
                                                         ctypes.byref(cctx), *rest)
    return getattr(lib, "dqo_rast_forward_" + stage + "_params")(ctypes.byref(params), ctypes.byref(inputs), ctypes.byref(pinputs),
                                                                 ctypes.byref(outputs), ctypes.byref(cctx), *rest)


def _forward(ctx, means3D, sh, colors_precomp, opacities, scales, rotations, cov3Ds_precomp, tile_mask, raster_settings,
             gaussian_object=None, pixel_object=None, tile_objects=None, pf=None):
    rs = raster_settings
    lib = N.lib()
    if means3D.ndimension() != 2 or means3D.size(1) != 3:
        raise RuntimeError("means3D must have dimensions (num_points, 3)")
    N.require_gpu(means3D, sh, colors_precomp, opacities, scales, rotations, cov3Ds_precomp, tile_mask, rs.bg, rs.viewmatrix,
                  rs.projmatrix, rs.campos)
    if not means3D.is_cuda:
        raise RuntimeError("libdqoraster operators need GPU (ROCm) tensors; there is no CPU path.")
    dev = means3D.device
    means3D, opacities = _f32(means3D, "means3D"), _f32(opacities, "opacities")
    sh, colors_precomp = _f32(sh, "sh"), _f32(colors_precomp, "colors_precomp")
    scales, rotations, cov3Ds_precomp = _f32(scales, "scales"), _f32(rotations, "rotations"), _f32(cov3Ds_precomp, "cov3D_precomp")
    bg, view, proj, campos = (_f32(rs.bg, "bg"), _f32(rs.viewmatrix, "viewmatrix"), _f32(rs.projmatrix, "projmatrix"),
                              _f32(rs.campos, "campos"))
    rs = rs._replace(bg=bg, viewmatrix=view, projmatrix=proj, campos=campos)
    if tile_mask is not None:
        if tile_mask.dtype != torch.int32:
            raise RuntimeError(f"expected scalar type Int but found {tile_mask.dtype} (tile_mask)")
        tile_mask = tile_mask.contiguous()
    P = means3D.size(0)
    H, W = int(rs.image_height), int(rs.image_width)
    M = sh.size(1) if sh.numel() != 0 else 0
    pinputs = None
    if pf is not None:
        f_dc, f_rest, o_raw, s_raw, r_raw = pf
        M = 1 + f_rest.size(1)
        pinputs = N.DqoRastParamInputs(features_dc=N.ptr(f_dc), features_rest=N.ptr(f_rest), rest=M - 1, opacity_raw=N.ptr(o_raw),
                                       scaling_raw=N.ptr(s_raw), rotation_raw=N.ptr(r_raw))
    gate = None
    if (gaussian_object is None) != (pixel_object is None):
        raise RuntimeError("object gate: gaussian_object and pixel_object go together")
    if gaussian_object is not None:
        N.require_gpu(gaussian_object, pixel_object)
        if gaussian_object.dtype != torch.int32 or pixel_object.dtype != torch.int32:
            raise RuntimeError("expected scalar type Int (object gate)")
        if gaussian_object.numel() != P or pixel_object.numel() != H * W:
            raise RuntimeError("object gate: gaussian_object must have num_points elements, pixel_object H x W")
        gaussian_object, pixel_object = gaussian_object.contiguous(), pixel_object.contiguous()
        _check_gate_ids(gaussian_object, pixel_object)
        gate = N.DqoObjectGate(gaussian_object=N.ptr(gaussian_object), pixel_object=N.ptr(pixel_object))
        if tile_objects is not None:
            N.require_gpu(tile_objects)
            if tile_objects.dtype != torch.int64 or tile_objects.numel() != ((H + 15) // 16) * ((W + 15) // 16):
                raise RuntimeError("object gate: tile_objects must be int64 with ceil(H/16) x ceil(W/16) elements")
            tile_objects = tile_objects.contiguous()
            gate.tile_objects = N.ptr(tile_objects)
    elif tile_objects is not None:
        raise RuntimeError("object gate: tile_objects without gaussian_object / pixel_object")
    row_flags = getattr(ctx, "row_flags", None)
    if row_flags is not None:
        N.require_gpu(row_flags)
        if row_flags.dtype != torch.uint8 or row_flags.numel() != P or not row_flags.is_contiguous():
            raise RuntimeError("row_flags must be a contiguous uint8 tensor with num_points elements")
    u8 = dict(dtype=torch.uint8, device=dev)
    with torch.cuda.device(dev):
        stream = N.current_stream()
        out, outputs = _new_outputs(P, H, W, dev)
        _, _, hit_color, hit_depth, _, _, _, n_touched, radii = out
        geomBuffer = torch.empty((lib.dqo_rast_geom_bytes(P, W, H),), **u8)
        imgBuffer = torch.empty((lib.dqo_rast_image_bytes(W, H),), **u8)
        params = _params(rs, P, M)
        inputs = _inputs(rs, means3D, sh, colors_precomp, opacities, scales, rotations, cov3Ds_precomp, tile_mask, row_flags=row_flags)
        cctx = N.DqoRastCtx(geom=geomBuffer.data_ptr(), geom_bytes=geomBuffer.numel(), binning=None, binning_bytes=0,
                            image=imgBuffer.data_ptr(), image_bytes=imgBuffer.numel(), inst_capacity=0, list_split=_list_split)
        if gate is not None:
            cctx.object_gate = ctypes.addressof(gate)
        key = (dev.index, P, W, H)
        cap = None
        lease = None
        if _sync_mode == "graph":
            with _lock:
                cap = _cap_hint.get(key)
            if cap is None:
                raise RuntimeError("diff_gaussian_rasterization_depth ('graph' mode): no instance capacity known for "
                                   f"P={P}, {W}x{H}: run one forward in 'lazy' mode first (the warm-up before the capture) or call "
                                   "set_capacity(P, W, H, instances)")
            num_rendered = -1
            with _lock:
                capturing = P > 0 and torch.cuda.is_current_stream_capturing()
                pooled = _pooled_set(lib, key, stream, dev, W, H, pin=True) if capturing else None
                if pooled is not None:
                    lease = _Pinned(pooled)
                    _captured.append(pooled)
                    geomBuffer, imgBuffer, binningBuffer, cap = pooled.geom, pooled.img, pooled.binning, pooled.cap
                    cctx.geom, cctx.geom_bytes = geomBuffer.data_ptr(), geomBuffer.numel()
                    cctx.image, cctx.image_bytes = imgBuffer.data_ptr(), imgBuffer.numel()
                    cctx.tile_bucket_capacity = pooled.bucket
                    cctx.keep_tile_order = 1 if pooled.order_valid else 0
                    cctx.frame_prezeroed = 1 if (pooled.clean and _list_split == 0 and any(ctx.needs_input_grad)) else 0
                    pooled.clean = False
                    pooled.captured = (int(cctx.keep_tile_order), int(cctx.frame_prezeroed))
                else:
                    binningBuffer = torch.empty((lib.dqo_rast_binning_bytes(cap),), **u8)
            cctx.binning, cctx.binning_bytes, cctx.inst_capacity = binningBuffer.data_ptr(), binningBuffer.numel(), cap
            N.check(_forward_call(lib, "async", params, inputs, pinputs, outputs, cctx, None, None, stream))
            _last["header"] = geomBuffer
        elif _sync_mode != "exact":
            _verify_pending(block=False)
            with _lock:
                cap = _cap_hint.get(key)
        if _sync_mode == "graph":
            pass
        elif cap is None:
            N.check(_forward_call(lib, "prepare", params, inputs, pinputs, outputs, cctx, stream))
            hdr = N.DqoRastHeader()
            N.check(lib.dqo_rast_read_header(ctypes.byref(cctx), ctypes.byref(hdr), stream))
            num_rendered = int(hdr.num_candidates)
            cap = max(num_rendered, 1)
            if _sync_mode == "exact":
                _last["num_rendered"], _last["num_visible"] = num_rendered, int(hdr.num_visible)
            else:
                cap = num_rendered + 4096
                with _lock:
                    cap = _cap_hint[key] = max(_cap_hint.get(key, 0), cap)
                num_rendered = -1
            binningBuffer = torch.empty((lib.dqo_rast_binning_bytes(cap),), **u8)
            cctx.binning, cctx.binning_bytes, cctx.inst_capacity = binningBuffer.data_ptr(), binningBuffer.numel(), cap
            N.check(_forward_call(lib, "render", params, inputs, pinputs, outputs, cctx, stream))
            if _sync_mode == "exact":
                _last["header"] = geomBuffer
            else:
                with _lock:
                    host, ev, _, _ = _ring_slot(dev.index)
                    host.copy_(geomBuffer[:32].view(torch.int32), non_blocking=True)
                    ev.record()
                    _pending.append((ev, host, key, cap, False))
                    _last["header"] = (ev, host)
        else:
            num_rendered = -1
            with _lock:
                pooled = _pooled_set(lib, key, stream, dev, W, H) if P > 0 else None
                if pooled is not None:
                    lease = _Lease(pooled)
                    geomBuffer, imgBuffer, binningBuffer, cap = pooled.geom, pooled.img, pooled.binning, pooled.cap
                    cctx.geom, cctx.geom_bytes = geomBuffer.data_ptr(), geomBuffer.numel()
                    cctx.image, cctx.image_bytes = imgBuffer.data_ptr(), imgBuffer.numel()
                    cctx.tile_bucket_capacity = pooled.bucket
                    cctx.keep_tile_order = 1 if pooled.order_valid else 0
                    cctx.frame_prezeroed = 1 if (pooled.clean and _list_split == 0) else 0
                    pooled.clean = False
                else:
                    binningBuffer = torch.empty((lib.dqo_rast_binning_bytes(cap),), **u8)
                cctx.binning, cctx.binning_bytes, cctx.inst_capacity = binningBuffer.data_ptr(), binningBuffer.numel(), cap
                host, ev, host_ptr, ev_handle = _ring_slot(dev.index)
                N.check(_forward_call(lib, "async", params, inputs, pinputs, outputs, cctx, host_ptr, ev_handle, stream))
                if pooled is not None:
                    pooled.order_valid = True
                _pending.append((ev, host, key, cap, pooled is not None))
                _last["header"] = (ev, host)
    if hasattr(ctx, "set_materialize_grads"):
        ctx.set_materialize_grads(False)
    ctx.pooled = lease
    ctx.raster_settings = rs
    ctx.num_rendered = num_rendered
    ctx.inst_capacity = cap
    ctx.list_split = _list_split
    ctx.M = M
    ctx.object_gate = None if gate is None else (gaussian_object, pixel_object)
    ctx.save_for_backward(colors_precomp, hit_depth, means3D, scales, rotations, cov3Ds_precomp, radii, sh, geomBuffer,
                          binningBuffer, imgBuffer, opacities, tile_mask if tile_mask is not None else torch.empty(0),
                          *(pf if pf is not None else ()))
    ctx.mark_non_differentiable(hit_color, hit_depth, n_touched, radii)
    return out


def _backward(ctx, grad_out_color, grad_out_depth):
    rs = ctx.raster_settings
    lib = N.lib()
    (colors_precomp, hit_depth, means3D, scales, rotations, cov3Ds_precomp, radii, sh, geomBuffer, binningBuffer, imgBuffer,
     opacities, tile_mask) = ctx.saved_tensors[:13]
    pf = ctx.saved_tensors[13:] or None
    if tile_mask.numel() == 0:
        tile_mask = None
    if _sync_mode in ("lazy", "deferred"):
        _verify_pending(block=(_sync_mode == "lazy"))
    P, M = means3D.size(0), ctx.M
    H, W = int(rs.image_height), int(rs.image_width)
    dev = means3D.device
    f32 = dict(dtype=torch.float32, device=dev)
    if grad_out_color is None:
        grad_out_color = torch.zeros((3, H, W), **f32)
    if grad_out_depth is None:
        grad_out_depth = torch.zeros((1, H, W), **f32)
    grad_out_color, grad_out_depth = _f32(grad_out_color, "grad_out_color"), _f32(grad_out_depth, "grad_out_depth")
    with torch.cuda.device(dev):
        stream = N.current_stream()
        want_colors, want_cov = colors_precomp.numel() != 0, cov3Ds_precomp.numel() != 0
        g_means3D = torch.empty((P, 3), **f32)
        g_colors = torch.empty((P, 3), **f32) if want_colors else None
        g_opacity = torch.empty((P, 1), **f32)
        g_cov3D = torch.empty((P, 6), **f32) if want_cov else None
        g_sh = torch.empty((P, M, 3), **f32) if pf is None else None
        g_scales = torch.empty((P, 3), **f32)
        g_rot = torch.empty((P, 4), **f32)
        pinputs = pgrads = None
        if pf is not None:
            f_dc, f_rest, o_raw, s_raw, r_raw = pf
            g_dc, g_rest = torch.empty((P, 1, 3), **f32), torch.empty((P, M - 1, 3), **f32)
            pinputs = N.DqoRastParamInputs(features_dc=N.ptr(f_dc), features_rest=N.ptr(f_rest), rest=M - 1,
                                           opacity_raw=N.ptr(o_raw), scaling_raw=N.ptr(s_raw), rotation_raw=N.ptr(r_raw))
            pgrads = N.DqoRastParamGrads(dL_dfeatures_dc=N.ptr(g_dc), dL_dfeatures_rest=N.ptr(g_rest), dL_dopacity_raw=N.ptr(g_opacity),
                                         dL_dscaling_raw=N.ptr(g_scales), dL_drotation_raw=N.ptr(g_rot))
        if P > 0:
            cap = ctx.inst_capacity
            ws = torch.empty((lib.dqo_rast_backward_workspace_bytes(cap),), dtype=torch.uint8, device=dev)
            params = _params(rs, P, M)
            inputs = _inputs(rs, means3D, sh, colors_precomp, opacities, scales, rotations, cov3Ds_precomp, tile_mask,
                             row_flags=getattr(ctx, "row_flags", None))
            cctx = N.DqoRastCtx(geom=geomBuffer.data_ptr(), geom_bytes=geomBuffer.numel(), binning=binningBuffer.data_ptr(),
                                binning_bytes=binningBuffer.numel(), image=imgBuffer.data_ptr(), image_bytes=imgBuffer.numel(),
                                inst_capacity=cap, list_split=getattr(ctx, "list_split", 0))
            lease = getattr(ctx, "pooled", None)
            if lease is not None:
                cctx.tile_bucket_capacity = lease.set.bucket
                cctx.frame_prezeroed = 1 if cctx.list_split == 0 else 0
            if getattr(ctx, "object_gate", None) is not None:
                gate = N.DqoObjectGate(gaussian_object=N.ptr(ctx.object_gate[0]), pixel_object=N.ptr(ctx.object_gate[1]))
                cctx.object_gate = ctypes.addressof(gate)
            grads = N.DqoRastGrads(dL_dmeans3D=g_means3D.data_ptr(), dL_dsh=N.ptr(g_sh), dL_dcolors=N.ptr(g_colors),
                                   dL_dopacity=g_opacity.data_ptr(), dL_dscales=g_scales.data_ptr(),
                                   dL_drotations=g_rot.data_ptr(), dL_dcov3D=N.ptr(g_cov3D), dL_dmeans2D=None,
                                   skip_culled_rows=1 if getattr(ctx, "sparse_grad_rows", False) else 0)
            if pf is None:
                N.check(lib.dqo_rast_backward(ctypes.byref(params), ctypes.byref(inputs), ctypes.byref(cctx),
                                              grad_out_color.data_ptr(), grad_out_depth.data_ptr(), hit_depth.data_ptr(),
                                              ctypes.byref(grads), ws.data_ptr(), ws.numel(), stream))
            else:
                grads.dL_dopacity = grads.dL_dscales = grads.dL_drotations = None
                N.check(lib.dqo_rast_backward_params(ctypes.byref(params), ctypes.byref(inputs), ctypes.byref(pinputs),
                                                     ctypes.byref(cctx), grad_out_color.data_ptr(), grad_out_depth.data_ptr(),
                                                     hit_depth.data_ptr(), ctypes.byref(grads), ctypes.byref(pgrads), ws.data_ptr(),
                                                     ws.numel(), stream))
            if lease is not None and cctx.frame_prezeroed:
                with _lock:
                    lease.set.clean = True
    if pf is not None:
        if P == 0:
            g_dc, g_rest = torch.empty((0, 1, 3), **f32), torch.empty((0, M - 1, 3), **f32)
        return (g_means3D, g_dc, g_rest, g_opacity.view_as(pf[2]), g_scales, g_rot)
    def slot(g, inp):
        return g if (g is not None and inp.numel() != 0) else None
    return (g_means3D, slot(g_sh, sh), slot(g_colors, colors_precomp), g_opacity.view_as(opacities) if opacities.numel() else None,
            slot(g_scales, scales), slot(g_rot, rotations), slot(g_cov3D, cov3Ds_precomp), None, None, None, None, None)


class _RasterizeGaussians(torch.autograd.Function):
    @staticmethod
    def forward(ctx, means3D, sh, colors_precomp, opacities, scales, rotations, cov3Ds_precomp, tile_mask, raster_settings,
                gaussian_object=None, pixel_object=None, tile_objects=None):
        return _forward(ctx, means3D, sh, colors_precomp, opacities, scales, rotations, cov3Ds_precomp, tile_mask, raster_settings,
                        gaussian_object, pixel_object, tile_objects)

    @staticmethod
    def backward(ctx, grad_out_color, grad_out_depth, grad_hit_color, grad_hit_depth, grad_hit_color_weight,
                 grad_hit_depth_weight, grad_T_map, grad_n_touched, _):
        return _backward(ctx, grad_out_color, grad_out_depth)


def rasterize_gaussian_params(means3D, features_dc, features_rest, opacity_raw, scaling_raw, rotation_raw, tile_mask, raster_settings):
    return _RasterizeGaussianParams.apply(means3D, features_dc, features_rest, opacity_raw, scaling_raw, rotation_raw, tile_mask,
                                          raster_settings)


class _RasterizeGaussianParams(torch.autograd.Function):
    @staticmethod
    def forward(ctx, means3D, features_dc, features_rest, opacity_raw, scaling_raw, rotation_raw, tile_mask, raster_settings):
        if means3D.ndimension() != 2 or means3D.size(1) != 3:
            raise RuntimeError("means3D must have dimensions (num_points, 3)")
        N.require_gpu(features_dc, features_rest, opacity_raw, scaling_raw, rotation_raw)
        pf = (_f32(features_dc, "features_dc"), _f32(features_rest, "features_rest"), _f32(opacity_raw, "opacity_raw"),
              _f32(scaling_raw, "scaling_raw"), _f32(rotation_raw, "rotation_raw"))
        P = means3D.size(0)
        for t, name, shape in zip(pf, ("features_dc", "features_rest", "opacity_raw", "scaling_raw", "rotation_raw"),
                                  ((P, 1, 3), None, (P, 1), (P, 3), (P, 4))):
            if shape is not None and (t.numel() != P * shape[1] * (shape[2] if len(shape) > 2 else 1) or t.size(0) != P):
                raise RuntimeError(f"{name} must have shape {list(shape)} (num_points = {P})")
        if pf[1].ndimension() != 3 or pf[1].size(0) != P or pf[1].size(2) != 3:
            raise RuntimeError(f"features_rest must have shape [{P}, R, 3]")
        if 1 + pf[1].size(1) < (int(raster_settings.sh_degree) + 1) ** 2:
            raise RuntimeError(f"features_rest has {pf[1].size(1)} coefficients, sh_degree {int(raster_settings.sh_degree)} needs "
                               f"{(int(raster_settings.sh_degree) + 1) ** 2 - 1}")
        empty = torch.empty(0, device=means3D.device)
        return _forward(ctx, means3D, empty, empty, empty, empty, empty, empty, tile_mask, raster_settings, pf=pf)

    @staticmethod
    def backward(ctx, grad_out_color, grad_out_depth, grad_hit_color, grad_hit_depth, grad_hit_color_weight,
                 grad_hit_depth_weight, grad_T_map, grad_n_touched, _):
        return _backward(ctx, grad_out_color, grad_out_depth) + (None, None)


class GaussianRasterizationSettings(NamedTuple):
    image_height: int
    image_width: int
    tanfovx: float
    tanfovy: float
# ... 57 lines not shown
```

dqo-map_amd/dqo_harness/fused_mapping.py:

```python
import collections
import ctypes
import os
import threading

import numpy as np
import torch

import _dqo_native as N
import diff_gaussian_rasterization_depth as dgr
from dqo_harness import mapping


def _normalised_settings(st, device):
    def fix(t, name, n):
        if not torch.is_tensor(t):
            raise RuntimeError(f"raster settings: {name} must be a tensor")
        if t.dtype != torch.float32:
            raise RuntimeError(f"expected scalar type Float but found {t.dtype} ({name})")
        if not t.is_cuda:
            raise RuntimeError("libdqoraster operators need GPU (ROCm) tensors; there is no CPU path.")
        if t.numel() != n:
            raise RuntimeError(f"raster settings: {name} must have {n} elements")
        return t.to(device).contiguous()
    return st._replace(bg=fix(st.bg, "bg", 3), viewmatrix=fix(st.viewmatrix, "viewmatrix", 16), projmatrix=fix(st.projmatrix, "projmatrix", 16),
# ... 292 lines not shown
            self._act_valid = True
        return self.opacity, self.scales, self.rotations

    def radius(self):
        sc = torch.exp(self.scaling_raw)
        return (sc.sum(dim=1) - sc.min(dim=1).values) / 2

    def normals(self, rows=None):
        q = self.rotation_raw if rows is None else self.rotation_raw[rows]
        sc = self.scaling_raw if rows is None else self.scaling_raw[rows]
        q = q / torch.sqrt((q * q).sum(1, keepdim=True))
        r, x, y, z = q[:, 0], q[:, 1], q[:, 2], q[:, 3]
        cols = (torch.stack([1 - 2 * (y * y + z * z), 2 * (x * y + r * z), 2 * (x * z - r * y)], 1),
                torch.stack([2 * (x * y - r * z), 1 - 2 * (x * x + z * z), 2 * (y * z + r * x)], 1),
                torch.stack([2 * (x * z + r * y), 2 * (y * z - r * x), 1 - 2 * (x * x + y * y)], 1))
        k = torch.argmin(sc, dim=1)
        nrm = torch.where((k == 0)[:, None], cols[0], torch.where((k == 1)[:, None], cols[1], cols[2]))
        return nrm / (torch.sqrt((nrm * nrm).sum(1, keepdim=True)) + 1e-8)

    def _park_position(self):
        V = self.settings.viewmatrix
        return (self.settings.campos.reshape(3) - 1.0e4 * V[:3, 2]).to(torch.float32)

    def _rows(self, *groups):
        for b in _ROW_BUFFERS:
            if not groups or b.group in groups:
                a = self.state[b.of[0]][b.of[1]] if b.of else getattr(self, b.name)
                if a is not None:
                    yield b, a

    def _set_rows(self, b, a):
        if b.of:
            pair = list(self.state[b.of[0]])
            pair[b.of[1]] = a
            self.state[b.of[0]] = tuple(pair)
        else:
            setattr(self, b.name, a)

    def _spare_value(self, b):
        if b.spare == "park":
            return self._park_position()
        if b.spare == "unit_q":
            import dqo_mapgrowth as mg
            return mg.const_tensor([1.0, 0.0, 0.0, 0.0], self.device)
        return b.spare

    @staticmethod
    def _write_rows(a, rows, value):
        if torch.is_tensor(value):
            a[rows] = value
        else:
            a.index_fill_(0, rows, value)

    def _free_rows(self, rows):
        for b, a in self._rows("param", "meta"):
            if b.freed:
                self._write_rows(a, rows, self._spare_value(b))

    def _fill_rows(self, rows, new):
        for b, a in self._rows("param", "meta"):
            self._write_rows(a, rows, new.get(b.name, b.live))

    def _compact_and_append(self, keep_old, new, carry_call):
        n = new["xyz"].shape[0]
        for b, a in self._rows("param", "meta", *(("moment", "snapshot") if carry_call else ())):
            add = new.get(b.name, new.get(b.src))
            if add is None:
                add = torch.zeros((n,) + tuple(a.shape[1:]), dtype=a.dtype, device=self.device)
            self._set_rows(b, torch.cat([a if keep_old is None else a[keep_old], add]).contiguous())
        self.P = self.xyz.shape[0]
        if not carry_call:
            for b, a in self._rows("moment", "snapshot"):
                self._set_rows(b, None if b.group == "snapshot" else torch.zeros((self.P,) + tuple(a.shape[1:]), dtype=a.dtype, device=self.device))

    def _drop_graphs(self):
        self._g, self._frames, self._mixed = None, [], {}

    def _row_count_changed(self):
        for b in _ROW_BUFFERS:
            if b.group == "dropped":
                setattr(self, b.name, None)
            elif b.group == "sized":
                make = torch.empty if b.spare is None else torch.zeros
                setattr(self, b.name, make(b.shape(self.P), dtype=torch.float32, device=self.device))
        self._attach_n, self._act_valid = 0, False
        self._lifecycle, self._maintain_ctx = {}, None
        self._window_flags = None
        self._drop_graphs()

    @torch.no_grad()
    def reserve(self, spare_rows):
        n = int(spare_rows)
        if n <= 0:
            return self
        if self.alive is None:
            self.alive = torch.ones((self.P,), dtype=torch.uint8, device=self.device)
        for b, a in self._rows("param", "moment", "snapshot", "meta"):
            fill = self._spare_value(b)
            tail = torch.empty((n,) + tuple(a.shape[1:]), dtype=a.dtype, device=self.device)
            tail[:] = fill.to(a.dtype) if torch.is_tensor(fill) else fill
            self._set_rows(b, torch.cat([a, tail]).contiguous())
        self._spare_rows = n
        self._n_spare = int(self.alive.numel() - int(self.alive.sum().item()))
        self.P += n
        self._row_count_changed()
        return self

    @property
    def n_alive(self):
        return self.P if self.alive is None else int(self.alive.sum().item())

    def _refresh_spare_count(self):
        if self._n_spare_stale:
            self._n_spare, self._n_spare_stale = int(self.alive.numel() - int(self.alive.sum().item())), False

    @torch.no_grad()
    def track_lifecycle(self, stable_mask=None, tick=0):
        dev, P = self.device, self.P
        live = torch.ones((P,), dtype=torch.bool, device=dev) if self.alive is None else self.alive.bool()
        stable = torch.zeros((P,), dtype=torch.bool, device=dev) if stable_mask is None else stable_mask.to(dev).bool().reshape(-1)
        if stable.numel() != P:
            raise RuntimeError("FusedMapper.track_lifecycle: stable_mask must have one entry per row")
        self.stable = (stable & live).to(torch.uint8)
        self.add_tick = live.to(torch.int32) * int(tick)
        self.depth_error_counter = torch.zeros((P,), dtype=torch.int32, device=dev)
        self.color_error_counter = torch.zeros((P,), dtype=torch.int32, device=dev)
        self._lifecycle = {}
        return self

    def _require_lifecycle(self, who):
        if self.stable is None:
            raise RuntimeError(f"FusedMapper.{who}: this mapper does not track its Gaussians' lifecycle; call track_lifecycle() first")

    def stable_rows(self):
        self._require_lifecycle("stable_rows")
        return (self.stable != 0) if self.alive is None else (self.stable != 0) & (self.alive != 0)

    MAINTAIN_DEFAULTS = dict(stable_confidence_thres=500.0, unstable_time_window=200, add_color_thres=0.1, add_depth_thres=None, delete_thresh=10)

    def _maintain_render(self, st, row_flags=None):
        lib, dev, P, M = N.lib(), self.device, self.P, self.M
        H, W = int(st.image_height), int(st.image_width)
        if (H, W) != (int(self.settings.image_height), int(self.settings.image_width)):
            raise RuntimeError("FusedMapper.maintain: every frame of a mapper has the mapper's image size")
        stream = N.current_stream()
        b = ctypes.byref
        c = self._maintain_ctx
        first = c is None or c["key"] != (P, H, W)
        if first:
            u8 = dict(dtype=torch.uint8, device=dev)
            out, outputs = dgr._new_outputs(P, H, W, dev)
            c = dict(key=(P, H, W), out=out, outputs=outputs, geom=torch.empty((lib.dqo_rast_geom_bytes(P, W, H),), **u8),
                     img=torch.empty((lib.dqo_rast_image_bytes(W, H),), **u8))
        params = dgr._params(st, P, M)
        inputs = dgr._inputs(st, self.xyz, self.shs, self._empty, self.opacity, self.scales, self.rotations, self._empty, self.tile_mask,
                             row_flags=row_flags)
        cctx = N.DqoRastCtx(geom=c["geom"].data_ptr(), geom_bytes=c["geom"].numel(), binning=None, binning_bytes=0,
                            image=c["img"].data_ptr(), image_bytes=c["img"].numel(), inst_capacity=0)
        if first:
            hdr = N.DqoRastHeader()
            N.check(lib.dqo_rast_forward_prepare(b(params), b(inputs), b(c["outputs"]), b(cctx), stream))
            N.check(lib.dqo_rast_read_header(b(cctx), b(hdr), stream))
            c["cap"] = int(1.5 * int(hdr.num_candidates)) + 4096
            c["binning"] = torch.empty((lib.dqo_rast_binning_bytes(c["cap"]),), dtype=torch.uint8, device=dev)
        cctx.binning, cctx.binning_bytes, cctx.inst_capacity = c["binning"].data_ptr(), c["binning"].numel(), c["cap"]
        if first:
            N.check(lib.dqo_rast_forward_render(b(params), b(inputs), b(c["outputs"]), b(cctx), stream))
            self._maintain_ctx = c
        else:
            N.check(lib.dqo_rast_forward(b(params), b(inputs), b(c["outputs"]), b(cctx), stream))
        return c

    def maintain_overflowed(self):
        c = self._maintain_ctx
        if c is None:
            return False
        over = int(c["geom"][:32].view(torch.int32)[2].item()) != 0
        if over:
            self._maintain_ctx = None
        return over

    @torch.no_grad()
    def maintain(self, tick, gt_color, gt_depth, settings=None, stable_oversized=False, **thresholds):
        import dqo_mapgrowth as mg
        self._require_lifecycle("maintain")
        if self.attach_count_reducer is not None:
            raise NotImplementedError("FusedMapper.maintain: a sharded mapper would need the whole map's mean radii (DESIGN.md §6)")
        unknown = set(thresholds) - set(self.MAINTAIN_DEFAULTS)
        if unknown:
            raise TypeError(f"FusedMapper.maintain: unknown thresholds {sorted(unknown)}")
        th = dict(self.MAINTAIN_DEFAULTS, **thresholds)
        if th["add_depth_thres"] is None:
            th["add_depth_thres"] = self.add_depth_thres
        dev = self.device
        st = self.settings if settings is None else _normalised_settings(settings, dev)
        if self.alive is None:
            self.alive = torch.ones((self.P,), dtype=torch.uint8, device=dev)
        with torch.cuda.device(dev):
            self.activate()
            c = self._maintain_render(st)
            state = dict({b.name: a for b, a in self._rows("param", "meta")}, **self._lifecycle)
            stats = mg.lifecycle_step(state, tick, gt_color, gt_depth, c["out"][0], c["out"][1], c["out"][3], c["out"][2],
                                      stable_oversized=stable_oversized, park=self._park_position(), render_header=c["geom"], **th)
            self._lifecycle = {"_lifecycle": state["_lifecycle"]}
        self._n_spare_stale = True
        self._act_valid = False
        self.activate()
        return stats

    @torch.no_grad()
    def evaluate(self, frames, min_depth=0.3, max_depth=5.0, out=None):
        return self._evaluate(frames, min_depth, max_depth, out, None)

    @torch.no_grad()
    def evaluate_ms_ssim(self, frames, ms_ssim, min_depth=0.3, max_depth=5.0, out=None):
        import dqo_eval
        H, W = int(self.settings.image_height), int(self.settings.image_width)
        if min(H, W) < dqo_eval.MS_MIN_SIDE:
            raise RuntimeError(f"FusedMapper.evaluate_ms_ssim: both image sides must be above 160, the mapper's image is {W} x {H}")
        K = len(frames)
        if (not torch.is_tensor(ms_ssim) or tuple(ms_ssim.shape) != (K, 20) or ms_ssim.dtype != torch.float32 or not ms_ssim.is_contiguous()
                or not ms_ssim.is_cuda):
            raise RuntimeError(f"FusedMapper.evaluate_ms_ssim: ms_ssim must be a contiguous float32 [{K},20] device table")
        return self._evaluate(frames, min_depth, max_depth, out, ms_ssim)

    def _evaluate(self, frames, min_depth, max_depth, out, ms_ssim):
        import dqo_eval
        if self.attach_count_reducer is not None:
            raise NotImplementedError("FusedMapper.evaluate: a sharded mapper would need the whole map's render, a shard's shows its "
                                      "objects only (DESIGN.md §6)")
        dev, K = self.device, len(frames)
        H, W = int(self.settings.image_height), int(self.settings.image_width)
        if ms_ssim is not None and self._eval_ms_ws is None:
            self._eval_ms_ws = dqo_eval.ms_ssim_workspace(W, H, dev)
        if self._eval_ws is None:
            self._eval_ws = dqo_eval.workspace(W, H, dev)
        table = out
        if table is None:
            table = self._eval_tables.get(K)
            if table is None:
                table = self._eval_tables[K] = torch.empty((K, 8), dtype=torch.float32, device=dev)
        with torch.cuda.device(dev):
            self.activate()
            for k, (settings, gt_color, gt_depth) in enumerate(frames):
                c = self._maintain_render(self.settings if settings is None else _normalised_settings(settings, dev))
                o = c["out"]
                dqo_eval.eval_picture(dict(render=o[0], depth=o[1], depth_index_map=o[3]), gt_color, gt_depth, min_depth, max_depth, out=table,
                                      row=k, workspace_buffer=self._eval_ws, render_header=c["geom"])
                if ms_ssim is not None:
                    dqo_eval.ms_ssim(o[0], gt_color, out=ms_ssim, row=k, workspace_buffer=self._eval_ms_ws, render_header=c["geom"])
        return table

    @torch.no_grad()
    def evaluate_geometry(self, gt_points, dist_thres=(0.03,), transform=None, out=None, row=0):
        import dqo_eval
        return dqo_eval.eval_pcd(gt_points, self.xyz.detach(), dist_thres, transform, rec_keep=self.alive, out=out, row=row)

    SAMPLE_DEFAULTS = dict(uniform_sample_num=50000, add_transmission_thres=0.5, add_depth_thres=None, add_color_thres=0.1,
                           transmission_sample_ratio=1.0, error_sample_ratio=0.05, init_opacity=0.99, xyz_factor=(1.0, 1.0, 0.1),
                           capacity=None, key_bits=32)

    @torch.no_grad()
    def sample_new(self, frame_map, settings=None, *, seed, tick, first_frame=False, model_map=None, **thresholds):
        import dqo_mapgrowth as mg
        unknown = set(thresholds) - set(self.SAMPLE_DEFAULTS)
        if unknown:
            raise TypeError(f"FusedMapper.sample_new: unknown thresholds {sorted(unknown)}")
        th = dict(self.SAMPLE_DEFAULTS, **thresholds)
        if th["add_depth_thres"] is None:
            th["add_depth_thres"] = self.add_depth_thres
        dev = self.device
        H, W = int(self.settings.image_height), int(self.settings.image_width)
        if th["capacity"] is None:
            th["capacity"] = mg.sample_capacity(H, W, first_frame, th["uniform_sample_num"], th["transmission_sample_ratio"], th["error_sample_ratio"])
        with torch.cuda.device(dev):
            if first_frame:
                model_map = None
            elif model_map is None:
                st = self.settings if settings is None else _normalised_settings(settings, dev)
                self.activate()
                c = self._maintain_render(st)
                if self.maintain_overflowed():
                    c = self._maintain_render(st)
                out = c["out"]
                model_map = dict(render_color=out[0].permute(1, 2, 0), render_depth=out[1].permute(1, 2, 0),
                                 render_depth_index=out[3].permute(1, 2, 0), render_transmission=out[6].permute(1, 2, 0))
            s = self._sample_ctx
            if s is None or s["key"] != (th["capacity"], self.M):
                s = self._sample_ctx = dict(key=(th["capacity"], self.M), buffers=mg.sample_buffers(th["capacity"], self.M, dev),
                                            workspace=torch.empty((N.lib().dqo_growth_sample_workspace_bytes(W, H),), dtype=torch.uint8, device=dev))
            new, self.sample_header = mg.temp_points_init(frame_map, model_map, seed=seed, tick=tick, sh_coeffs=self.M, buffers=s["buffers"],
                                                          workspace=s["workspace"], **th)
            if self.gaussian_object is not None:
                if "obj_id" not in new:
                    raise RuntimeError("FusedMapper.sample_new: with an object gate the frame needs 'instance_img'")
                held = torch.zeros((64,), dtype=torch.bool, device=dev)
                held[(self.gaussian_object if self.alive is None else self.gaussian_object[self.alive.bool()]).long()] = True
                keep = held[new["obj_id"].clamp(0, 63).long()] & (new["obj_id"] >= 0) & (new["obj_id"] < 64)
                new = {k: v[keep] for k, v in new.items()}
        return new

    @torch.no_grad()
    def grow(self, new, delete_mask=None, min_radius=0.001, max_radius=0.05, xyz_factor=(1.0, 1.0, 0.1), scale_factor=1.0,
             new_mapping_call=False, stable_mask=None, unstable_opacity_low=0.1, attach_async=True, tick=None):
        self._refresh_spare_count()
        c = self._grow_candidates(new)
# ... 172 lines not shown
        out = mapping.render(st, data, object_gate=None)
        cim = out["color_index_map"]
        zero_fill = (cim == 0) & (out["color_hit_weight"] == 0)
        cim = torch.where(zero_fill, first.to(cim.dtype).reshape(1, 1, 1), cim)
        return mg.temp_points_attach_indices(temp_xyz, temp_opacity, st.viewmatrix.T.contiguous(), K, W, H, cim, self.xyz,
                                             lambda rows: self.normals(rows), self.add_depth_thres, unstable_opacity_low)

    def attach_loss(self):
        return self.attach_partial[:self._attach_n].sum()

    def _attach_fields(self):
        if not self.use_attach:
            return dict(attach_mask=None, init_xyz=None, init_scaling_raw=None, init_rotation_raw=None, attach_count=0, attach_partial=None)
        return dict(attach_mask=N.ptr(self.attach_mask), init_xyz=N.ptr(self.init_xyz), init_scaling_raw=N.ptr(self.init_scaling),
                    init_rotation_raw=N.ptr(self.init_rotation), attach_count=self.attach_count, attach_partial=N.ptr(self.attach_partial),
                    attach_gains=N.ptr(self.attach_gains))

    @staticmethod
    def pick_list_split_pair(list_split, tile_mask, st, longest=0):
        if isinstance(list_split, (tuple, list)):
            f, b = int(list_split[0]), int(list_split[1])
            if f < 0 or b not in (0, f):
                raise ValueError("list_split pair: (forward threshold, 0 or the same threshold)")
            return f, b
        if list_split != "auto":
            if int(list_split) < 0:
                raise ValueError("list_split is 0 (off), a list length, a pair or 'auto'")
            return int(list_split), int(list_split)
        tiles = int((tile_mask != 0).sum().item()) if tile_mask is not None else ((st.image_width + 15) // 16) * ((st.image_height + 15) // 16)
        if tiles <= 1300:
            t = 256 if tiles <= 500 else 512 if tiles <= 800 else 1024
            return (t, t) if longest >= 1024 else (0, 0)
        if tiles <= 2600:
            return (1024, 0) if longest >= 2048 else (0, 0)
        return (2048, 0) if longest >= 4096 else (0, 0)

    @staticmethod
    def pick_list_split(list_split, tile_mask, st, longest=0):
        return FusedMapper.pick_list_split_pair(list_split, tile_mask, st, longest)[1]

    def capture(self, gt_color, gt_depth, render_mask, tile_mask=None, capacity_margin=1.15, tile_buckets=True, keep_tile_order=True,
                loss_tap=True, reuse_probe=False, fused_tail=True, list_split=0, unroll=1, settings=None, pixel_object=None, frame=None,
                run_unroll=1,
                short_bucket_margin=1.3):
        dev = self.device
        st = self.settings if settings is None else _normalised_settings(settings, dev)
        st = st._replace(bg=st.bg.clone(), viewmatrix=st.viewmatrix.clone(), projmatrix=st.projmatrix.clone(), campos=st.campos.clone())
        H, W = int(st.image_height), int(st.image_width)
        if (H, W) != (int(self.settings.image_height), int(self.settings.image_width)):
            raise RuntimeError("FusedMapper.capture: every frame of a mapper has the mapper's image size")
        tile_mask = self.tile_mask if tile_mask is None else _checked_tile_mask(tile_mask, dev, H, W)
        pix_obj, tile_obj = self.pixel_object, self.tile_objects
        if pixel_object is not None:
            if self.gaussian_object is None:
                raise RuntimeError("FusedMapper.capture: a per-frame pixel_object needs set_object_gate first")
            pix_obj = torch.as_tensor(pixel_object).to(dev, torch.int32).contiguous().reshape(H, W)
            tile_obj = tile_object_sets(pix_obj)
        for name, t_, shape in (("gt_color", gt_color, (3, H, W)), ("gt_depth", gt_depth, (1, H, W))):
            if t_.dtype != torch.float32 or not t_.is_cuda or not t_.is_contiguous() or tuple(t_.shape) != shape:
                raise RuntimeError(f"FusedMapper.capture: {name} must be a contiguous float32 GPU tensor of shape {shape} "
                                   "(the graph reads it in place at every replay)")
        mask = None if render_mask is None else render_mask.to(torch.uint8).contiguous()
        g = _FrameGraph(frame, st, pix_obj, tile_obj, gt_color, gt_depth, mask, tile_mask,
                        dict(tile_buckets=tile_buckets, keep_tile_order=keep_tile_order, loss_tap=loss_tap, fused_tail=fused_tail,
                             list_split=list_split, unroll=unroll, run_unroll=run_unroll, short_bucket_margin=short_bucket_margin))
        with torch.cuda.device(dev):
            self._settle_replays()
            if frame is None:
                self._drop_graphs()
            self.activate()
            reuse_probe, longest = self._size_graph(g, capacity_margin, reuse_probe)
            self._g = g
            if isinstance(frame, tuple):
                self._mixed[frame] = g
            elif frame is not None:
                while len(self._frames) <= frame:
                    self._frames.append(None)
                self._frames[frame] = g
            self._allocate_graph(g)
            self._build_graph_structs(g, longest)
            if not self._warm_up_and_record(g, reuse_probe):
                self._last_probe = None
                return self._recapture(g, capacity_margin)
        return self

    def _recapture(self, g, capacity_margin):
        own_pixel_object = self.gaussian_object is not None and g.pixel_object is not self.pixel_object
        return self.capture(g.gt_color, g.gt_depth, g.mask, tile_mask=g.tile_mask, capacity_margin=capacity_margin, settings=g.settings,
                            pixel_object=g.pixel_object if own_pixel_object else None, frame=g.frame, **g.options)

    def _size_graph(self, g, capacity_margin, reuse_probe):
        P, last = self.P, self._last_probe
        if reuse_probe and last is not None and last[2] > 0:
            grown = max(1.0, P / last[2])
            cand, longest = int(last[0] * grown) + 1, int(last[1] * grown) + 1
        else:
            reuse_probe = False
            cand, longest = self._probe(g.tile_mask, g.settings, g.pixel_object, g.tile_objects)
        self._last_probe = (cand, longest, P)
        g.cap = int(cand * capacity_margin) + 4096
        if g.options["tile_buckets"]:
            g.bucket = 256
            while g.bucket < 2 * longest:
                g.bucket *= 2
            if g.bucket == 2048 and float(g.options["short_bucket_margin"]) * longest <= 1024:
                g.bucket = 1024
        return reuse_probe, longest

    def _allocate_graph(self, g):
        lib, dev, P, M = N.lib(), self.device, self.P, self.M
        H, W = int(g.settings.image_height), int(g.settings.image_width)
        f, u8 = dict(dtype=torch.float32, device=dev), dict(dtype=torch.uint8, device=dev)
        g.out, g.outputs = dgr._new_outputs(P, H, W, dev)
        g.geom = torch.empty((lib.dqo_rast_geom_bytes(P, W, H),), **u8)
        g.img = torch.empty((lib.dqo_rast_image_bytes(W, H),), **u8)
        g.binning = torch.empty((lib.dqo_rast_binning_bytes_bucketed(g.cap, W, H, g.bucket),), **u8)
        g.ws = torch.empty((lib.dqo_rast_backward_workspace_bytes(g.cap),), **u8)
        g.grads = dict(means3D=torch.empty((P, 3), **f), sh=torch.empty((P, M, 3), **f),
                       opacity=torch.empty((P, 1), **f), scales=torch.empty((P, 3), **f), rot=torch.empty((P, 4), **f))
        g.step_dev, g.ticket, g.bias = self._step_dev, self._ticket, self._bias

    def _build_graph_structs(self, g, longest):
        st, opt = g.settings, g.options
        g.fused_tail = bool(opt["fused_tail"]) and self.M <= 16
        g.params = dgr._params(st, self.P, self.M)
        g.inputs = dgr._inputs(st, self.xyz, self.shs, self._empty, self.opacity, self.scales, self.rotations, self._empty, g.tile_mask,
                               row_flags=self.row_flags)
        g.cctx = N.DqoRastCtx(geom=g.geom.data_ptr(), geom_bytes=g.geom.numel(), binning=g.binning.data_ptr(),
                              binning_bytes=g.binning.numel(), image=g.img.data_ptr(), image_bytes=g.img.numel(), inst_capacity=g.cap,
                              tile_bucket_capacity=g.bucket)
        g.ls_fwd, g.ls_bwd = self.pick_list_split_pair(opt["list_split"], g.tile_mask, st, longest)
        g.cctx.list_split = g.ls_fwd
        loss_tap = opt["loss_tap"] and not (g.mask is None and self.ssim_weight != 0)
        if loss_tap:
            g.grad_scale = torch.zeros((2,), dtype=torch.float32, device=self.device)
            g.tap = N.DqoLossTap(gt_color=N.ptr(g.gt_color), gt_depth=N.ptr(g.gt_depth), render_mask=N.ptr(g.mask),
                                 out_color=g.out[0].data_ptr(), out_depth=g.out[1].data_ptr(), color_weight=self.color_weight,
                                 depth_weight=self.depth_weight, add_depth_thres=self.add_depth_thres, loss_out=N.ptr(self.loss),
                                 grad_scale=g.grad_scale.data_ptr(),
                                 per_object=1 if (self.per_object_loss and self.gaussian_object is not None) else 0)
            g.cctx.loss_tap = ctypes.addressof(g.tap)
        if self.gaussian_object is not None:
            g.gate = N.DqoObjectGate(gaussian_object=N.ptr(self.gaussian_object), pixel_object=N.ptr(g.pixel_object),
                                     tile_objects=N.ptr(g.tile_objects))
            g.cctx.object_gate = ctypes.addressof(g.gate)
            if self.per_object_loss and not loss_tap:
                raise RuntimeError("FusedMapper.capture: the per-object loss is computed by the loss tap (loss_tap=True)")
        gr = [g.grads[k].data_ptr() for k in ("means3D", "sh", "opacity", "scales", "rot")]
        g.cgrads = N.DqoRastGrads(dL_dmeans3D=gr[0], dL_dsh=gr[1], dL_dcolors=None, dL_dopacity=gr[2], dL_dscales=gr[3],
                                  dL_drotations=gr[4], dL_dcov3D=None, dL_dmeans2D=None, skip_culled_rows=1)
        g.adam = self._adam_step_args(gr, radii=g.out[8].data_ptr(), frame_header=g.geom.data_ptr(), step_dev=g.step_dev)
        g.adam.record_ctx = ctypes.addressof(g.cctx)
        g.adam.record_W, g.adam.record_H = int(st.image_width), int(st.image_height)

    def _warm_up_and_record(self, g, reuse_probe):
        self._step_dev.fill_(self.step_count + 1)
        self._expected_step = self.step_count + 1
        side = torch.cuda.Stream(device=self.device)
        side.wait_stream(torch.cuda.current_stream())
        with torch.cuda.stream(side):
            self._static_iteration()
        torch.cuda.current_stream().wait_stream(side)
        if not self.graph_overflowed():
            self.step_count += 1
        elif reuse_probe:
            return False
        g.cctx.keep_tile_order = 1 if (g.bucket > 0 and g.options["keep_tile_order"]) else 0
        g.cctx.frame_prezeroed = 1 if g.fused_tail else 0
        g.graph = torch.cuda.CUDAGraph()
        g.unroll = max(1, int(g.options["unroll"]))
        with torch.cuda.graph(g.graph, capture_error_mode="thread_local"):
            for _ in range(g.unroll):
                self._static_iteration()
        g.run_unroll = max(1, int(g.options["run_unroll"]))
        if g.run_unroll > 1:
            g.run_graph = torch.cuda.CUDAGraph()
            with torch.cuda.graph(g.run_graph, capture_error_mode="thread_local"):
                for _ in range(g.run_unroll):
                    self._static_iteration()
        self._expected_step = self.step_count + 1
        return True

    def _adam_step_args(self, grads, radii, frame_header, step=0, step_dev=None):
        stt, ticket = self.state, step_dev is not None and self.use_block_ticket
        return N.DqoAdamStep(P=self.P, M=self.M, step=step, beta1=self.betas[0], beta2=self.betas[1], eps=self.eps, lr_xyz=self.lrs["xyz"],
                             lr_f_dc=self.lrs["f_dc"], lr_f_rest=self.lrs["f_rest"], lr_opacity=self.lrs["opacity"],
                             lr_scaling=self.lrs["scaling"], lr_rotation=self.lrs["rotation"], xyz=N.ptr(self.xyz), shs=N.ptr(self.shs),
                             opacity_raw=N.ptr(self.opacity_raw), scaling_raw=N.ptr(self.scaling_raw),
                             rotation_raw=N.ptr(self.rotation_raw), g_means3D=grads[0], g_sh=grads[1], g_opacity=grads[2],
                             g_scales=grads[3], g_rotations=grads[4], m_xyz=N.ptr(stt["xyz"][0]), m_shs=N.ptr(stt["shs"][0]),
                             m_opacity=N.ptr(stt["opacity"][0]), m_scaling=N.ptr(stt["scaling"][0]), m_rotation=N.ptr(stt["rotation"][0]),
                             v_xyz=N.ptr(stt["xyz"][1]), v_shs=N.ptr(stt["shs"][1]), v_opacity=N.ptr(stt["opacity"][1]),
                             v_scaling=N.ptr(stt["scaling"][1]), v_rotation=N.ptr(stt["rotation"][1]), act_opacity=N.ptr(self.opacity),
                             act_scales=N.ptr(self.scales), act_rotations=N.ptr(self.rotations), radii=radii, step_dev=N.ptr(step_dev),
                             moment_live=N.ptr(self.moment_live), frame_header=frame_header,
                             block_ticket=N.ptr(self._ticket) if ticket else None, bias_table=N.ptr(self._bias) if ticket else None,
                             row_flags=N.ptr(self.row_flags), confidence=N.ptr(self.confidence) if self.count_confidence else None,
                             lr_table=N.ptr(self.lr_table) if step_dev is not None else None, **self._attach_fields())

    def _trained_state(self):
        return [a for _, a in self._rows("param", "moment")] + [self.confidence] + [a for b, a in self._rows("meta") if b.name in _LIFECYCLE_ROWS]

    def _snapshot_state(self):
        return dict(rows=[a.clone() for a in self._trained_state()], step=self.step_count)

    def _restore_state(self, snap):
        self._settle_replays()
        for a, old in zip(self._trained_state(), snap["rows"]):
            a.copy_(old)
        self.step_count = snap["step"]
        self._step_dev.fill_(self.step_count + 1)
        self._expected_step, self._unsettled = self.step_count + 1, False
        self._bias.zero_()
        self._act_valid = False
        self.activate()

    def capture_window(self, frames, **kw):
        snap = self._snapshot_state()
        self._settle_replays()
        self._drop_graphs()
        self._window_kw, self._window_frames = dict(kw), list(frames)
        for k, fr in enumerate(frames):
            if k:
                self._restore_state(snap)
            self.capture(fr["gt_color"], fr["gt_depth"], fr.get("render_mask"), tile_mask=fr.get("tile_mask"), settings=fr.get("settings"),
                         pixel_object=fr.get("pixel_object"), frame=k, **kw)
            torch.cuda.synchronize()
        self._restore_state(snap)
        return self

    @staticmethod
    def window_schedule(n_iters, n_frames, rng, final=False, random_keyframes=False, global_opt=False):
        out = []
        for it in range(int(n_iters)):
            k = rng.randint(0, n_frames - 1)
            if it > n_iters / 2 and not final and not random_keyframes:
                k = (k, n_frames - 1) if (global_opt and k != n_frames - 1) else n_frames - 1
            out.append(k)
        return out

    def _graph_of(self, frame):
        if not isinstance(frame, tuple):
            return self._frames[frame]
        if frame not in self._mixed:
            k, m = frame
            fk, fm_ = self._window_frames[k], self._window_frames[m]
            snap = self._snapshot_state()
            cur = self._g
            self.capture(fk["gt_color"], fk["gt_depth"], fm_.get("render_mask"), tile_mask=fm_.get("tile_mask"), settings=fk.get("settings"),
                         pixel_object=fk.get("pixel_object"), frame=frame, **self._window_kw)
            self._restore_state(snap)
            self._g = cur
            g2, gm = self._mixed[frame], self._frames[m]
            for src, dst in ((gm.mask, g2.mask), (gm.tile_mask, g2.tile_mask)) if gm is not None else ():
                if src is not None and dst is not None and dst.data_ptr() not in (src.data_ptr(), self.tile_mask.data_ptr()):
                    dst.copy_(src.view(dst.shape))
        return self._mixed[frame]

    def run_window(self, schedule, check_every=64, capacity_margin=1.5):
        recaptures, i = 0, 0
        while i < len(schedule):
            batch = schedule[i:i + check_every]
            start = self.step_count
            self.replay_schedule(batch)
            lost = (start + len(batch)) - (int(self._step_dev.item()) - 1)
            if lost > 0:
                self._settle_replays()
                bad = [k for k in sorted(set(batch), key=str) if self.graph_overflowed(self._graph_of(k))]
                if not bad or recaptures > 8 * max(1, len(self._frames)):
                    raise RuntimeError("FusedMapper.run_window: the map keeps outgrowing the captured capacities")
                for k in bad:
                    g = self._graph_of(k)
                    snap = self._snapshot_state()
                    self._recapture(g, capacity_margin)
                    self._restore_state(snap)
                    recaptures += 1
                for j in range(lost):
                    self.replay(frame=bad[j % len(bad)])
                torch.cuda.synchronize()
            i += len(batch)
        return recaptures

    @torch.no_grad()
    def set_frame(self, frame, gt_color=None, gt_depth=None, render_mask=None, tile_mask=None, settings=None, pixel_object=None):
        cams = [self._frames[frame]] + [g for (k, m), g in self._mixed.items() if k == frame]
        masks = [self._frames[frame]] + [g for (k, m), g in self._mixed.items() if m == frame]
        done = set()

        def once(t):
            if t.data_ptr() in done:
                return False
            done.add(t.data_ptr())
            return True

        for g in cams:
            if gt_color is not None and once(g.gt_color):
                g.gt_color.copy_(gt_color)
            if gt_depth is not None and once(g.gt_depth):
                g.gt_depth.copy_(gt_depth)
        for g in masks:
            if render_mask is not None:
                if g.mask is None:
                    raise RuntimeError("FusedMapper.set_frame: the frame was captured without a render mask")
                if once(g.mask):
                    g.mask.copy_(render_mask.to(torch.uint8))
            if tile_mask is not None and once(g.tile_mask):
                g.tile_mask.copy_(_checked_tile_mask(tile_mask, self.device, int(g.settings.image_height), int(g.settings.image_width)))
        if settings is not None:
            new = _normalised_settings(settings, self.device)
            for g in cams:
                for name in ("image_height", "image_width", "tanfovx", "tanfovy", "cx", "cy", "sh_degree", "scale_modifier", "opaque_threshold",
                             "depth_threshold", "normal_threshold", "color_sigma", "T_threshold"):
                    if getattr(new, name) != getattr(g.settings, name):
                        raise RuntimeError(f"FusedMapper.set_frame: {name} is a captured kernel argument; capture the frame again")
                for name in ("bg", "viewmatrix", "projmatrix", "campos"):
                    getattr(g.settings, name).copy_(getattr(new, name))
        if pixel_object is not None:
            for g in cams:
                if g.pixel_object is None:
                    raise RuntimeError("FusedMapper.set_frame: the frame was captured without an object gate")
                if once(g.pixel_object):
                    g.pixel_object.copy_(torch.as_tensor(pixel_object).to(self.device, torch.int32).reshape(g.pixel_object.shape))
                    g.tile_objects.copy_(tile_object_sets(g.pixel_object))
        return self

    @torch.no_grad()
    def refresh_window(self, frames=None, *, global_opt=False, sample_ratio=-1, rows=None, out=None):
        import dqo_tilemask
        if self.attach_count_reducer is not None:
            raise NotImplementedError("FusedMapper.refresh_window: a sharded mapper would need the whole map's render, a shard's shows its "
                                      "objects only (DESIGN.md §6)")
        dev = self.device
        H, W = int(self.settings.image_height), int(self.settings.image_width)
        gy, gx = (H + 15) // 16, (W + 15) // 16
        slots = [k for k, g in enumerate(self._frames) if g is not None] if frames is None else [int(k) for k in frames]
        for k in slots:
            if not 0 <= k < len(self._frames) or self._frames[k] is None:
                raise RuntimeError(f"FusedMapper.refresh_window: frame {k} of the window is not captured")
            g = self._frames[k]
            if (int(g.settings.image_height), int(g.settings.image_width)) != (H, W):
                raise RuntimeError("FusedMapper.refresh_window: every frame of a mapper has the mapper's image size")
            if g.mask is None:
                raise RuntimeError(f"FusedMapper.refresh_window: frame {k} was captured without a render mask")
            if g.tile_mask is self.tile_mask or g.tile_mask.data_ptr() == self.tile_mask.data_ptr():
                raise RuntimeError(f"FusedMapper.refresh_window: frame {k} was captured without a tile mask of its own (it reads the "
                                   "mapper's shared all-ones tile mask, which every default-mask render reads too)")
            if g.mask.numel() != H * W or g.tile_mask.numel() != gy * gx:
                raise RuntimeError("FusedMapper.refresh_window: every frame of a mapper has the mapper's image size")
        if rows is None:
            rows = self.trained_rows()
        elif not torch.is_tensor(rows) or rows.dtype != torch.bool or rows.numel() != self.P or rows.device != self.row_flags.device:
            raise RuntimeError("FusedMapper.refresh_window: rows must be a bool GPU tensor with one entry per row")
        K = len(slots)
        table = out
        if table is None:
            table = self._window_ratios.get(K)
            if table is None:
                table = self._window_ratios[K] = torch.empty((K,), dtype=torch.float32, device=dev)
        elif table.dtype != torch.float32 or tuple(table.shape) != (K,) or not table.is_contiguous() or table.device != self.row_flags.device:
            raise RuntimeError(f"FusedMapper.refresh_window: out must be a contiguous float32 [{K}] tensor on the mapper's device")
        with torch.cuda.device(dev):
            if self._window_ws is None:
                self._window_ws = dqo_tilemask.window_masks_workspace(H, W, dev)
            if self._window_flags is None:
                self._window_flags = torch.empty((self.P,), dtype=torch.uint8, device=dev)
            hidden = ~rows.reshape(-1)
            if self.alive is not None:
                hidden |= self.alive == 0
            self._window_flags.copy_(hidden).mul_(N.ROW_HIDDEN)
            self.activate()
            done = set()
            for i, k in enumerate(slots):
                g = self._frames[k]
                c = self._maintain_render(g.settings, row_flags=self._window_flags)
                o = c["out"]
                dqo_tilemask.window_masks(o[6], o[0], g.gt_color, global_opt=global_opt, sample_ratio=sample_ratio,
                                          render_mask=g.mask.view(H, W), tile_mask=g.tile_mask.view(gy, gx), ratio_out=table[i:i + 1],
                                          render_header=c["geom"], workspace=self._window_ws)
                done.update((g.mask.data_ptr(), g.tile_mask.data_ptr()))
            for k in slots:
                g = self._frames[k]
                for (_, m), g2 in self._mixed.items():
                    if m != k:
                        continue
                    for src, dst in ((g.mask, g2.mask), (g.tile_mask, g2.tile_mask)):
                        if dst is not None and dst.data_ptr() not in done and dst.data_ptr() != self.tile_mask.data_ptr():
                            done.add(dst.data_ptr())
                            dst.copy_(src.view(dst.shape))
        return table

    def capture_placed(self, *args, trials=4, probe_replays=12, **kw):
        if int(trials) <= 1:
            return self.capture(*args, **kw)
        self._settle_replays()
        snap = self._snapshot_state()

        def restore():
            self._restore_state(snap)

        cands = []
        for t in range(int(trials)):
            if t:
                restore()
                self._g = None
            self.capture(*args, **kw)
            torch.cuda.synchronize()
            e0, e1 = torch.cuda.Event(enable_timing=True), torch.cuda.Event(enable_timing=True)
            for _ in range(3):
                self.replay()
            e0.record()
            for _ in range(int(probe_replays)):
                self.replay()
            e1.record()
            torch.cuda.synchronize()
            self._settle_replays()
            if self.graph_overflowed():
                continue
            cands.append((e0.elapsed_time(e1) / probe_replays / self._g.unroll, self._g))
        if not cands:
            raise RuntimeError("FusedMapper.capture_placed: every trial overflowed its captured capacities")
        best = min(range(len(cands)), key=lambda i: cands[i][0])
        self.placement_trials_ms = [round(c[0], 4) for c in cands]
        restore()
        self._g = cands[best][1]
        if self._g.frame is not None:
            self._frames[self._g.frame] = self._g
        del cands
        self.step_static()
        torch.cuda.synchronize()
        return self

    def _probe(self, tile_mask, st=None, pixel_object=None, tile_objects=None):
        lib, dev, P, M = N.lib(), self.device, self.P, self.M
        st = self.settings if st is None else st
        if pixel_object is None:
            pixel_object, tile_objects = self.pixel_object, self.tile_objects
        H, W = int(st.image_height), int(st.image_width)
        u8 = dict(dtype=torch.uint8, device=dev)
        out, outputs = dgr._new_outputs(P, H, W, dev)
        geom = torch.empty((lib.dqo_rast_geom_bytes(P, W, H),), **u8)
        img = torch.empty((lib.dqo_rast_image_bytes(W, H),), **u8)
        params = dgr._params(st, P, M)
        inputs = dgr._inputs(st, self.xyz, self.shs, self._empty, self.opacity, self.scales, self.rotations, self._empty, tile_mask,
                             row_flags=self.row_flags)
        cctx = N.DqoRastCtx(geom=geom.data_ptr(), geom_bytes=geom.numel(), binning=None, binning_bytes=0, image=img.data_ptr(),
                            image_bytes=img.numel(), inst_capacity=0)
        if self.gaussian_object is not None:
            gate = N.DqoObjectGate(gaussian_object=N.ptr(self.gaussian_object), pixel_object=N.ptr(pixel_object), tile_objects=N.ptr(tile_objects))
            cctx.object_gate = ctypes.addressof(gate)
        stream = N.current_stream()
        hdr = N.DqoRastHeader()
        N.check(lib.dqo_rast_forward_prepare(ctypes.byref(params), ctypes.byref(inputs), ctypes.byref(outputs), ctypes.byref(cctx), stream))
        N.check(lib.dqo_rast_read_header(ctypes.byref(cctx), ctypes.byref(hdr), stream))
        cand = int(hdr.num_candidates)
        binning = torch.empty((lib.dqo_rast_binning_bytes(max(cand, 1)),), **u8)
        cctx.binning, cctx.binning_bytes, cctx.inst_capacity = binning.data_ptr(), binning.numel(), max(cand, 1)
        N.check(lib.dqo_rast_forward_render(ctypes.byref(params), ctypes.byref(inputs), ctypes.byref(outputs), ctypes.byref(cctx), stream))
        N.check(lib.dqo_rast_read_header(ctypes.byref(cctx), ctypes.byref(hdr), stream))
        return cand, int(hdr.max_tile_count)

    def _static_iteration(self):
        lib, g = N.lib(), self._g
        st = self.settings
        H, W = int(st.image_height), int(st.image_width)
        stream = N.current_stream()
        g.cctx.list_split = g.ls_fwd
        N.check(lib.dqo_rast_forward(ctypes.byref(g.params), ctypes.byref(g.inputs), ctypes.byref(g.outputs), ctypes.byref(g.cctx), stream))
        g.cctx.list_split = g.ls_bwd
        o = g.out
        if g.tap is None:
            N.check(lib.dqo_map_loss_fwd_bwd(W, H, o[0].data_ptr(), o[1].data_ptr(), o[3].data_ptr(), N.ptr(g.gt_color), N.ptr(g.gt_depth),
                                             N.ptr(g.mask), self.color_weight, self.depth_weight, self.add_depth_thres, N.ptr(self.loss),
                                             N.ptr(self.dL_dcolor), N.ptr(self.dL_ddepth), N.ptr(self.loss_ws), self.loss_ws.numel(), stream))
            if g.mask is None and self.ssim_weight != 0:
                self._ssim_term(o[0].data_ptr(), g.gt_color, stream)
        dLc, dLd = (self.dL_dcolor.data_ptr(), self.dL_ddepth.data_ptr()) if g.tap is None else (None, None)
        self._attach_n = ((self.P + 255) // 256) * (4 if g.fused_tail else 1)
        if g.fused_tail:
            N.check(lib.dqo_rast_backward_adam(ctypes.byref(g.params), ctypes.byref(g.inputs), ctypes.byref(g.cctx), dLc, dLd,
                                               ctypes.byref(g.adam), g.ws.data_ptr(), g.ws.numel(), stream))
            return
        N.check(lib.dqo_rast_backward(ctypes.byref(g.params), ctypes.byref(g.inputs), ctypes.byref(g.cctx), dLc, dLd, o[3].data_ptr(),
                                      ctypes.byref(g.cgrads), g.ws.data_ptr(), g.ws.numel(), stream))
        N.check(lib.dqo_map_adam_step(ctypes.byref(g.adam), stream))

    def _ssim_term(self, color_ptr, gt_color, stream):
        lib = N.lib()
        H, W = int(self.settings.image_height), int(self.settings.image_width)
        if self.ssim_ws is None:
            self.ssim_ws = torch.empty((lib.dqo_map_ssim_workspace_bytes(W, H),), dtype=torch.uint8, device=self.device)
            self.ssim_out = torch.zeros((2,), dtype=torch.float32, device=self.device)
        N.check(lib.dqo_map_ssim_fwd_bwd(W, H, color_ptr, N.ptr(gt_color), self.ssim_weight, N.ptr(self.ssim_out), N.ptr(self.dL_dcolor), 1,
                                         N.ptr(self.loss), N.ptr(self.ssim_ws), self.ssim_ws.numel(), stream))

    def replay(self, frame=None):
        if frame is not None:
            self._g = self._graph_of(frame)
        return self._launch(self._g, self._g.graph, self._g.unroll)

    def replay_run(self, frame, n):
        g = self._graph_of(frame)
        k = g.run_unroll
        out = None
        while n >= k and k > 1:
            self._g = g
            out = self._launch(g, g.run_graph, k)
            n -= k
        for _ in range(n):
            out = self.replay(frame=frame)
        return out

    def replay_schedule(self, schedule):
        i = 0
        while i < len(schedule):
            j = i
            while j < len(schedule) and schedule[j] == schedule[i]:
                j += 1
            self.replay_run(schedule[i], j - i)
            i = j

    def _settle_replays(self):
        if not self._unsettled:
            return
        dev_step = int(self._step_dev.item())
        invalid = int(self._expected_step) - dev_step
        if invalid > 0:
            self.step_count -= invalid
        self._expected_step = dev_step
        self._unsettled = False

    def _resync_step_count(self):
        self._settle_replays()
        self._step_dev.fill_(self.step_count + 1)
        self._expected_step = self.step_count + 1

    def run(self, n_iters, check_every=64, capacity_margin=1.5):
        if self._g.unroll != 1:
            raise RuntimeError("FusedMapper.run counts single iterations: capture with unroll=1")
        target = self.step_count + n_iters
        recaptures = 0
        while self.step_count < target:
            k = min(check_every, target - self.step_count)
            for _ in range(k):
                self.replay()
            if int(self._step_dev.item()) - 1 != self.step_count or self.graph_overflowed():
                if recaptures > 8:
                    raise RuntimeError("FusedMapper.run: the map keeps outgrowing the captured capacities")
                self._recapture(self._g, capacity_margin)
                recaptures += 1
        return recaptures

    def step_static(self):
        return self._launch(self._g, None, 1)

    def _launch(self, g, graph, n):
        if g.stale:
            raise RuntimeError("FusedMapper: the attach set / object gate changed since capture(); capture again")
        if self._expected_step != self.step_count + 1:
            self._resync_step_count()
        if graph is None:
            with torch.cuda.device(self.device):
                self._static_iteration()
        else:
            graph.replay()
        self._unsettled = True
        self._attach_n = ((self.P + 255) // 256) * (4 if g.fused_tail else 1)
        self.step_count += n
        self._expected_step = self.step_count + 1
        return g.out

    def header(self, g=None):
        h = (self._g if g is None else g).geom[:32].view(torch.int32).cpu().tolist()
        return dict(num_rendered=h[0], num_tiles=h[1], overflow=h[2], max_tile_count=h[3], num_visible=h[4], num_candidates=h[5])

    def graph_overflowed(self, g=None):
        return bool((self._g if g is None else g).geom[:12].view(torch.int32)[2].item())

    def _params(self):
        return dict(xyz=self.xyz, shs=self.shs, opacity=self.opacity_raw, scaling=self.scaling_raw, rotation=self.rotation_raw)

    @torch.no_grad()
    def step(self, gt_color, gt_depth, render_mask, tile_mask=None):
        lib = N.lib()
        self._settle_replays()
        with torch.cuda.device(self.device):
            stream = N.current_stream()
            self.activate()
            ctx = _Ctx()
            ctx.row_flags = self.row_flags
            out = dgr._RasterizeGaussians.forward(ctx, self.xyz, self.shs, self._empty, self.opacity, self.scales, self.rotations,
                                                  self._empty, self.tile_mask if tile_mask is None else tile_mask, self.settings,
                                                  self.gaussian_object, self.pixel_object)
            color, depth, hit_depth = out[0], out[1], out[3]
            H, W = color.shape[1], color.shape[2]
            mask_u8 = None if render_mask is None else render_mask
            if mask_u8 is not None and mask_u8.dtype != torch.uint8:
                mask_u8 = mask_u8.to(torch.uint8)
            if self.per_object_loss and self.gaussian_object is not None:
                with torch.enable_grad():
# ... 22 lines not shown
```

include/dqo_raster.h:

```cpp
#ifndef DQO_RASTER_H_
#define DQO_RASTER_H_

#include <stddef.h>
#include <stdint.h>

#ifdef __cplusplus
extern "C" {
#endif

#define DQO_ABI_VERSION 5

typedef enum DqoStatus {
    DQO_OK = 0,
    DQO_ERR_INVALID_ARG = -1,
    DQO_ERR_WORKSPACE = -2,
    DQO_ERR_LAUNCH = -3,
    DQO_ERR_OVERFLOW = -4
} DqoStatus;

typedef struct DqoRastParams {
    int32_t P;
    int32_t D;
    int32_t M;
    int32_t W, H;
    int32_t prefiltered;
    int32_t debug;
    float tanfovx, tanfovy;
    float cx, cy;
    float scale_modifier;
    float color_sigma;
    float opaque_threshold;
    float depth_threshold;
    float normal_threshold;
    float T_threshold;
} DqoRastParams;

typedef struct DqoRastInputs {
    const float* bg;
    const float* means3D;
    const float* shs;
    const float* colors_precomp;
    const float* opacities;
    const float* scales;
    const float* rotations;
    const float* cov3D_precomp;
    const float* viewmatrix;
    const float* projmatrix;
    const float* campos;
    const int32_t* tile_mask;
    const uint8_t* row_flags;
} DqoRastInputs;
#define DQO_ROW_FROZEN 1u
#define DQO_ROW_HIDDEN 2u

typedef struct DqoRastOutputs {
    float* out_color;
    float* out_depth;
    int32_t* out_hit_color;
    int32_t* out_hit_depth;
    float* out_hit_color_weight;
    float* out_hit_depth_weight;
    float* out_T;
    int32_t* n_touched;
    int32_t* radii;
} DqoRastOutputs;

typedef struct DqoLossTap {
    const float* gt_color;
    const float* gt_depth;
    const uint8_t* render_mask;
    const float* out_color;
    const float* out_depth;
    float color_weight, depth_weight, add_depth_thres;
    float* loss_out;
    float* grad_scale;
    int32_t per_object;
} DqoLossTap;

typedef struct DqoObjectGate {
    const int32_t* gaussian_object;
    const int32_t* pixel_object;
    const uint64_t* tile_objects;
} DqoObjectGate;

typedef struct DqoRastCtx {
    void* geom;
    size_t geom_bytes;
    void* binning;
    size_t binning_bytes;
    void* image;
    size_t image_bytes;
    int64_t inst_capacity;
    int32_t tile_bucket_capacity;
    int32_t keep_tile_order;
    const DqoLossTap* loss_tap;
    const DqoObjectGate* object_gate;
    int32_t list_split;
    int32_t frame_prezeroed;
} DqoRastCtx;

typedef struct DqoRastGrads {
    float* dL_dmeans3D;
    float* dL_dsh;
    float* dL_dcolors;
    float* dL_dopacity;
    float* dL_dscales;
    float* dL_drotations;
    float* dL_dcov3D;
    float* dL_dmeans2D;
    int32_t skip_culled_rows;
} DqoRastGrads;

typedef struct DqoRastHeader {
    uint32_t num_rendered;
    uint32_t num_tiles;
    uint32_t overflow;
    uint32_t max_tile_count;
    uint32_t num_visible;
    uint32_t num_candidates;
    uint32_t stage;
    uint32_t reserved;
} DqoRastHeader;

int dqo_abi_version(void);
const char* dqo_last_error(void);
size_t dqo_abi_sizeof(int32_t which);

typedef struct DqoProfileEntry {
    char name[48];
    double total_ms;
    uint32_t calls;
} DqoProfileEntry;
int dqo_profile_enable(int on);
int dqo_profile_collect(DqoProfileEntry* out, int max_entries, int reset);

size_t dqo_rast_geom_bytes(int32_t P, int32_t W, int32_t H);
size_t dqo_rast_image_bytes(int32_t W, int32_t H);
size_t dqo_rast_binning_bytes(int64_t inst_capacity);
size_t dqo_rast_binning_bytes_bucketed(int64_t inst_capacity, int32_t W, int32_t H, int32_t tile_bucket_capacity);
size_t dqo_rast_backward_workspace_bytes(int64_t inst_capacity);

int dqo_rast_forward_prepare(const DqoRastParams*, const DqoRastInputs*, DqoRastOutputs*, DqoRastCtx*, void* hipStream);
int dqo_rast_read_header(const DqoRastCtx*, DqoRastHeader* host_out, void* hipStream);
int dqo_rast_forward_render(const DqoRastParams*, const DqoRastInputs*, DqoRastOutputs*, DqoRastCtx*, void* hipStream);
int dqo_rast_forward(const DqoRastParams*, const DqoRastInputs*, DqoRastOutputs*, DqoRastCtx*, void* hipStream);

int dqo_rast_forward_async(const DqoRastParams*, const DqoRastInputs*, DqoRastOutputs*, DqoRastCtx*, DqoRastHeader* header_host,
                           void* header_event, void* hipStream);

int dqo_rast_backward(const DqoRastParams*, const DqoRastInputs*, const DqoRastCtx*, const float* dL_dout_color,
                      const float* dL_dout_depth, const int32_t* hit_image, DqoRastGrads*, void* workspace,
                      size_t workspace_bytes, void* hipStream);

int dqo_mark_visible(int32_t P, const float* means3D, const float* viewmatrix, const float* projmatrix, uint8_t* present,
                     void* hipStream);

typedef struct DqoRastParamInputs {
    const float* features_dc;
    const float* features_rest;
    int32_t rest;
    const float* opacity_raw;
    const float* scaling_raw;
    const float* rotation_raw;
} DqoRastParamInputs;

typedef struct DqoRastParamGrads {
    float* dL_dfeatures_dc;
    float* dL_dfeatures_rest;
    float* dL_dopacity_raw;
    float* dL_dscaling_raw;
    float* dL_drotation_raw;
} DqoRastParamGrads;

int dqo_rast_forward_prepare_params(const DqoRastParams*, const DqoRastInputs*, const DqoRastParamInputs*, DqoRastOutputs*, DqoRastCtx*,
                                    void* hipStream);
int dqo_rast_forward_render_params(const DqoRastParams*, const DqoRastInputs*, const DqoRastParamInputs*, DqoRastOutputs*, DqoRastCtx*,
                                   void* hipStream);
int dqo_rast_forward_async_params(const DqoRastParams*, const DqoRastInputs*, const DqoRastParamInputs*, DqoRastOutputs*, DqoRastCtx*,
                                  DqoRastHeader* header_host, void* header_event, void* hipStream);
int dqo_rast_backward_params(const DqoRastParams*, const DqoRastInputs*, const DqoRastParamInputs*, const DqoRastCtx*,
                             const float* dL_dout_color, const float* dL_dout_depth, const int32_t* hit_image, DqoRastGrads*,
                             DqoRastParamGrads*, void* workspace, size_t workspace_bytes, void* hipStream);

size_t dqo_knn3_workspace_bytes(int32_t P);
int dqo_knn3(int32_t P, const float* xyz, float* mean_d2, int32_t* idx3, void* workspace, size_t workspace_bytes,
             void* hipStream);

size_t dqo_knn3_query_workspace_bytes(int32_t Q, int32_t R);
int dqo_knn3_query(int32_t Q, const float* query_xyz, int32_t R, const float* ref_xyz, float* dist2, int32_t* idx3, void* workspace,
                   size_t workspace_bytes, void* hipStream);
int dqo_knn3_query_within(int32_t Q, const float* query_xyz, int32_t R, const float* ref_xyz, float max_dist, float* dist2, int32_t* idx3,
                          void* workspace, size_t workspace_bytes, void* hipStream);
int dqo_knn3_query_grouped(int32_t Q, const float* query_xyz, const int32_t* query_group, int32_t R, const float* ref_xyz,
                           const int32_t* ref_group, const float* group_box, float max_dist, float* dist2, int32_t* idx3, void* workspace,
                           size_t workspace_bytes, void* hipStream);

int dqo_attach_pixels(int32_t n, const float* temp_xyz, const float* viewmatrix, float fx, float fy, float cx, float cy, int32_t W, int32_t H,
                      const int32_t* pixel_object, int32_t* lin, int32_t* sparse_pixel_object, uint64_t* tile_objects, void* hipStream);
int dqo_attach_decide(int32_t n, const float* temp_xyz, const float* temp_opacity, const int32_t* temp_object, const int32_t* lin,
                      const int32_t* hit_index, const float* hit_weight, const float* xyz, const float* scaling_raw,
                      const float* rotation_raw, const int32_t* gaussian_object, float plane_thr, float opacity_low, uint8_t* out,
                      void* hipStream);

int dqo_growth_scales(int32_t n, const float* xyz, const int32_t* object, const float* radius, const int32_t* i_new, const float* d2_old,
                      const int32_t* i_old, const float* extra_radius, float reach2, float min_radius, float max_radius, float* scales,
                      uint8_t* invalid, void* hipStream);
int dqo_growth_inside(int32_t n, const float* d2, const int32_t* idx, const float* radius, uint8_t* inside, void* hipStream);
int dqo_error_maps(int32_t H, int32_t W, const float* gt_color, const float* gt_depth, const float* render, const float* depth,
                   const int32_t* depth_index, const uint8_t* mask, float* color_err, float* depth_err, void* hipStream);

typedef struct DqoLifecycle {
    int32_t P, W, H;
    int32_t tick;
    int32_t unstable_time_window, delete_thresh;
    int32_t stable_oversized;
    int32_t use_votes;
    float stable_confidence_thres, add_color_thres, add_depth_thres;
    float* xyz;
    float* opacity_raw;
    float* scaling_raw;
    float* confidence;
    uint8_t* alive;
    uint8_t* row_flags;
    uint8_t* stable;
    int32_t* add_tick;
    int32_t* depth_error_counter;
    int32_t* color_error_counter;
    const float* park;
    uint32_t* vote;
    void* workspace;
    size_t workspace_bytes;
    int32_t* stats;
    const DqoRastHeader* render_header;
} DqoLifecycle;
size_t dqo_map_lifecycle_workspace_bytes(int32_t P);
int dqo_map_lifecycle_vote(const DqoLifecycle* step, const float* gt_color, const float* gt_depth, const float* render_color,
                           const float* render_depth, const int32_t* depth_index, const int32_t* color_index, void* hipStream);
int dqo_map_lifecycle_rows(const DqoLifecycle* step, void* hipStream);

typedef struct DqoGrowthSample {
    int32_t W, H;
    int32_t first_frame;
    int32_t uniform_sample_num;
    int32_t capacity;
    int32_t key_bits;
    int32_t M;
    int32_t identity_rotation;
    uint64_t seed;
    float add_transmission_thres, add_depth_thres, add_color_thres;
    float transmission_sample_ratio, error_sample_ratio, init_opacity;
    const float* vertex;
    const float* normal;
    const float* color;
    const float* depth;
    const float* instance;
    const float* T;
    const float* render_depth;
    const float* render_color;
    const int32_t* depth_index;
    float* xyz;
    float* scales;
    float* rotations;
    float* opacity;
    float* shs;
    int32_t* obj_id;
    float* out_normal;
    int32_t* pixel;
    int32_t* header;
    void* workspace;
    size_t workspace_bytes;
} DqoGrowthSample;
size_t dqo_growth_sample_workspace_bytes(int32_t W, int32_t H);
int dqo_growth_sample(const DqoGrowthSample* args, void* hipStream);

size_t dqo_eval_picture_workspace_bytes(int32_t W, int32_t H);
int dqo_eval_picture(int32_t W, int32_t H, const float* render, const float* gt_color, const float* depth, const float* gt_depth,
                     const int32_t* depth_index, float min_depth, float max_depth, const DqoRastHeader* render_header, float* out, int32_t row,
                     void* workspace, size_t workspace_bytes, void* hipStream);

size_t dqo_eval_ms_ssim_workspace_bytes(int32_t W, int32_t H);
int dqo_eval_ms_ssim(int32_t W, int32_t H, const float* render, const float* gt_color, const DqoRastHeader* render_header, float* out,
                     int32_t row, void* workspace, size_t workspace_bytes, void* hipStream);

size_t dqo_nn1_workspace_bytes(int32_t Q, int32_t R);
int dqo_nn1(int32_t Q, const float* query_xyz, const uint8_t* query_keep, int32_t R, const float* ref_xyz, const uint8_t* ref_keep,
            const float* query_xform, const float* ref_xform, float* dist2, int32_t* idx, void* workspace, size_t workspace_bytes,
            void* hipStream);

size_t dqo_eval_pcd_workspace_bytes(int32_t n_gt, int32_t n_rec);
int dqo_eval_pcd(int32_t n_gt, const float* gt_xyz, const uint8_t* gt_keep, int32_t n_rec, const float* rec_xyz, const uint8_t* rec_keep,
                 const float* rec_xform, int32_t n_thres, const float* thres_host, float* out_table, int32_t row, void* workspace,
                 size_t workspace_bytes, void* hipStream);

// ... 133 lines not shown
```

Measured before the change: 2391 iter/s.

## Precompute per-tile mask/object bitsets and stage them in LDS for binning cull

Adds a tile-bits table in the image buffer, built once per capture or whenever the mask or object tables change. It holds a mask row and per-object rows as packed bits, stamped with the pointers they were built from. The binning kernel checks the stamp, loads the bitsets into shared memory with global_load_lds, and does mask and object tests from LDS instead of global reads. It also switches the per-window live bits to a wave ballot with no atomics, dedups dead-tile flag writes via an LDS atomic, and halves the window size. The risk is a stale table if some path updates the masks without rebuilding it, plus extra LDS use that may cut occupancy.

New measurement: 2390 iter/s, median of 2. No clear change (-0.0%).

```diff
diff --git a/dqo-map_amd/_dqo_native.py b/dqo-map_amd/_dqo_native.py
--- a/dqo-map_amd/_dqo_native.py
+++ b/dqo-map_amd/_dqo_native.py
@@ -116,7 +116,7 @@
            "dqo_growth_sample_workspace_bytes", "dqo_growth_sample", "dqo_eval_picture_workspace_bytes", "dqo_eval_picture",
            "dqo_eval_ms_ssim_workspace_bytes", "dqo_eval_ms_ssim",
            "dqo_nn1_workspace_bytes", "dqo_nn1", "dqo_eval_pcd_workspace_bytes", "dqo_eval_pcd", "dqo_window_masks_workspace_bytes",
-           "dqo_window_masks")
+           "dqo_window_masks", "dqo_rast_tile_bits_bytes", "dqo_rast_tile_bits_build", "dqo_rast_tile_bits_clear")
 
 _lib = None
 
@@ -207,6 +207,10 @@
         L.dqo_window_masks_workspace_bytes.restype = ctypes.c_size_t
         L.dqo_window_masks_workspace_bytes.argtypes = [c_i32, c_i32]
         L.dqo_window_masks.argtypes = [c_i32, c_i32, c_i32, c_vp, c_vp, c_vp, c_f, c_i32, c_vp, c_vp, c_vp, c_vp, c_vp, ctypes.c_size_t, c_vp]
+        L.dqo_rast_tile_bits_bytes.restype = ctypes.c_size_t
+        L.dqo_rast_tile_bits_bytes.argtypes = [c_i32, c_i32]
+        L.dqo_rast_tile_bits_build.argtypes = [c_vp, ctypes.c_size_t, c_i32, c_i32, c_vp, c_vp, c_vp]
+        L.dqo_rast_tile_bits_clear.argtypes = [c_vp, ctypes.c_size_t, c_i32, c_i32, c_vp]
         L.dqo_map_history_merge.argtypes = [c_i32, c_i32, c_f, c_i32] + [c_vp] * 12
         L.dqo_map_lifecycle_workspace_bytes.restype = ctypes.c_size_t
         L.dqo_map_lifecycle_workspace_bytes.argtypes = [c_i32]
diff --git a/dqo-map_amd/csrc/dqo_capi.hip b/dqo-map_amd/csrc/dqo_capi.hip
--- a/dqo-map_amd/csrc/dqo_capi.hip
+++ b/dqo-map_amd/csrc/dqo_capi.hip
@@ -199,6 +199,30 @@
     return dqo_geom_layout(nullptr, P < 0 ? 0 : P).total;
 }
 DQO_API size_t dqo_rast_image_bytes(int32_t W, int32_t H) { return dqo_image_layout(nullptr, W, H).total; }
+DQO_API size_t dqo_rast_tile_bits_bytes(int32_t W, int32_t H) {
+    if (W <= 0 || H <= 0) return 0;
+    return dqo_tile_bits_bytes((size_t)((W + DQO_TILE - 1) / DQO_TILE) * (size_t)((H + DQO_TILE - 1) / DQO_TILE));
+}
+static int check_tile_bits(const void* image, size_t image_bytes, int32_t W, int32_t H) {
+    DQO_CHECK_ARG(W > 0 && H > 0 && (W + DQO_TILE - 1) / DQO_TILE < 65536 && (H + DQO_TILE - 1) / DQO_TILE < 65536, "bad image size %d x %d", W, H);
+    DQO_CHECK_ARG(image != nullptr && image_bytes >= dqo_rast_image_bytes(W, H), "image buffer too small (%zu < %zu)", image_bytes,
+                  dqo_rast_image_bytes(W, H));
+    return DQO_OK;
+}
+DQO_API int dqo_rast_tile_bits_build(void* image, size_t image_bytes, int32_t W, int32_t H, const int32_t* tile_mask, const uint64_t* tile_objects,
+                                     void* stream) {
+    const int rc = check_tile_bits(image, image_bytes, W, H);
+    if (rc) return rc;
+    const int T = ((W + DQO_TILE - 1) / DQO_TILE) * ((H + DQO_TILE - 1) / DQO_TILE);
+    return dqo_launch_tile_bits_build(dqo_image_layout(image, W, H), T, tile_mask, reinterpret_cast<const unsigned long long*>(tile_objects),
+                                      (hipStream_t)stream);
+}
+DQO_API int dqo_rast_tile_bits_clear(void* image, size_t image_bytes, int32_t W, int32_t H, void* stream) {
+    const int rc = check_tile_bits(image, image_bytes, W, H);
+    if (rc) return rc;
+    return dqo_launch_zero_words(dqo_image_layout(image, W, H).tile_bits, DQO_TB_HEAD_WORDS, (hipStream_t)stream);
+}
+
 DQO_API size_t dqo_rast_binning_bytes(int64_t cap) { return dqo_bin_layout(nullptr, cap < 0 ? 0 : cap, cap < 0 ? 0 : cap, 0).total; }
 DQO_API size_t dqo_rast_binning_bytes_bucketed(int64_t cap, int32_t W, int32_t H, int32_t bucket) {
     if (cap < 0) cap = 0;
diff --git a/dqo-map_amd/csrc/dqo_common.h b/dqo-map_amd/csrc/dqo_common.h
--- a/dqo-map_amd/csrc/dqo_common.h
+++ b/dqo-map_amd/csrc/dqo_common.h
@@ -233,8 +233,15 @@
     uint32_t* hit_pos;
     uint32_t* long_tiles;
     uint32_t* split_tiles;
+    uint32_t* tile_bits;
     size_t total;
 };
+
+#define DQO_TB_STAMP 0x711EB175u
+enum { DQO_TB_MAGIC = 0, DQO_TB_ROWS = 1, DQO_TB_W32 = 2, DQO_TB_TILES = 3, DQO_TB_MASK_LO = 4, DQO_TB_MASK_HI = 5, DQO_TB_OBJ_LO = 6,
+       DQO_TB_OBJ_HI = 7, DQO_TB_HEAD_WORDS = 64 };
+static inline size_t dqo_tile_bits_words(size_t T) { return dqo_align_up((size_t)(1 + DQO_GATE_OBJECTS) * ((T + 31) / 32), 256) + 256; }
+static inline size_t dqo_tile_bits_bytes(size_t T) { return dqo_align_up(4 * (DQO_TB_HEAD_WORDS + dqo_tile_bits_words(T)), 256); }
 
 static inline DqoImageLayout dqo_image_layout(void* base, int W, int H) {
     DqoImageLayout L;
@@ -258,6 +265,7 @@
     L.hit_pos = (uint32_t*)take(4 * HW);
     L.long_tiles = (uint32_t*)take(4 * T);
     L.split_tiles = (uint32_t*)take(4 * T);
+    L.tile_bits = (uint32_t*)take(dqo_tile_bits_bytes(T));
     L.total = (size_t)(p - (char*)base);
     return L;
 }
@@ -411,6 +419,7 @@
 
 int dqo_launch_zero_words(uint32_t* p, size_t n_words, hipStream_t s);
 
+int dqo_launch_tile_bits_build(const DqoImageLayout& img, int T, const int32_t* tile_mask, const unsigned long long* tile_objects, hipStream_t s);
 int dqo_launch_bin_count_k1(const DqoView& v, const DqoRastInputs* in, const DqoRastOutputs* out, const int32_t* gobj, const DqoGeomLayout& g,
                             const DqoImageLayout& img, const DqoBinLayout& bin, int64_t capacity, const unsigned long long* tile_objects,
                             hipStream_t s, bool pf = false);
diff --git a/dqo-map_amd/csrc/rast_binning.hip b/dqo-map_amd/csrc/rast_binning.hip
--- a/dqo-map_amd/csrc/rast_binning.hip
+++ b/dqo-map_amd/csrc/rast_binning.hip
@@ -6,7 +6,12 @@
 
 constexpr int BIN_THREADS = 256;
 constexpr int BIN_CHUNK = BIN_THREADS;
-constexpr int BIN_WINDOW = 16384;
+constexpr int BIN_WINDOW = 8192;
+#ifndef XTAB
+#define XTAB 1256
+#endif
+constexpr int BIN_TAB_WORDS = XTAB;
+constexpr int BIN_PIECE = 256;
 constexpr int BIN_FLIGHT = 4;
 #ifndef BIN_WAVES
 #define BIN_WAVES 8
@@ -49,6 +54,10 @@
 struct Cand {
     int gi, tile;
 };
+template <int N>
+struct TierTag {
+    static constexpr int value = N;
+};
 
 struct DqoK1Raw {
     DqoView v;
@@ -62,7 +71,8 @@
                                                                 uint32_t* __restrict__ tile_count, uint32_t* __restrict__ tile_flag,
                                                                 DqoBinLayout bin, int64_t capacity,
                                                                 const unsigned long long* __restrict__ tile_objects, const DqoK1Raw k1,
-                                                                const uint8_t* __restrict__ row_flags) {
+                                                                const uint8_t* __restrict__ row_flags, const uint32_t* __restrict__ tile_bits,
+                                                                int T) {
     static_assert(K1 || !PF, "the parameter form only differs in the early part");
     __shared__ uint32_t s_off[BIN_CHUNK + 1];
     __shared__ uint2 s_rect[BIN_CHUNK];
@@ -71,14 +81,47 @@
     __shared__ uint32_t s_cnt[BIN_CHUNK];
     __shared__ uint32_t s_prev[BIN_CHUNK];
     __shared__ uint32_t s_gb[BIN_CHUNK];
-    __shared__ uint32_t s_bits[BIN_WINDOW / 32];
+    __shared__ __attribute__((aligned(8))) uint32_t s_bits[BIN_WINDOW / 32];
     __shared__ uint32_t s_wave[BIN_THREADS / 64];
     __shared__ uint32_t s_base;
-    __shared__ int s_gobj[BIN_CHUNK];
+    __shared__ __attribute__((aligned(16))) uint32_t s_tab[BIN_TAB_WORDS];
+    __shared__ uint32_t s_tier[4];
     const int tid = threadIdx.x;
     const uint32_t lane = lane_id(), wave = tid >> 6;
     const int chunk0 = blockIdx.x * BIN_CHUNK;
     const int my_idx = dqo_spread_index(chunk0 + tid, P);
+
+    {
+        int tier = 0;
+        uint32_t W32 = 0, W32a = 0, n_obj = 0;
+        const uint32_t rows = tile_bits[DQO_TB_ROWS], w32 = tile_bits[DQO_TB_W32];
+        const unsigned long long mp = (unsigned long long)(uintptr_t)tile_mask, op = (unsigned long long)(uintptr_t)tile_objects;
+        const bool valid = tile_bits[DQO_TB_MAGIC] == DQO_TB_STAMP && tile_bits[DQO_TB_TILES] == (uint32_t)T && w32 == ((uint32_t)T + 31u) / 32u &&
+                           rows >= 1u && rows <= 1u + DQO_GATE_OBJECTS && tile_bits[DQO_TB_MASK_LO] == (uint32_t)mp &&
+                           tile_bits[DQO_TB_MASK_HI] == (uint32_t)(mp >> 32) && tile_bits[DQO_TB_OBJ_LO] == (uint32_t)op &&
+                           tile_bits[DQO_TB_OBJ_HI] == (uint32_t)(op >> 32);
+#ifdef XFORCE0
+        if (false) {
+#else
+        if (valid) {
+#endif
+            const uint32_t a = (w32 + 3u) & ~3u;
+            auto fits = [&](uint32_t words) { return a + (words + BIN_PIECE - 1) / BIN_PIECE * BIN_PIECE <= (uint32_t)BIN_TAB_WORDS; };
+            if (fits(rows * w32)) tier = 2, n_obj = rows - 1u;
+            else if (fits(w32)) tier = 1;
+            W32 = w32, W32a = a;
+        }
+        if (tier != 0) {
+            const uint32_t pieces = ((tier == 2 ? (n_obj + 1u) * W32 : W32) + BIN_PIECE - 1) / BIN_PIECE;
+            const uint32_t* const rows0 = tile_bits + DQO_TB_HEAD_WORDS;
+            for (uint32_t pc = wave; pc < pieces; pc += BIN_THREADS / 64)
+                __builtin_amdgcn_global_load_lds((const __attribute__((address_space(1))) void*)(rows0 + pc * BIN_PIECE + lane * 4u),
+                                                 (__attribute__((address_space(3))) void*)(s_tab + W32a + pc * BIN_PIECE), 16, 0, 0);
+            for (uint32_t i = tid; i < W32a; i += BIN_THREADS) s_tab[i] = 0u;
+            asm volatile("s_waitcnt vmcnt(0)" ::: "memory");
+        }
+        if (tid == 0) s_tier[0] = (uint32_t)tier, s_tier[1] = W32, s_tier[2] = W32a, s_tier[3] = n_obj;
+    }
 
     uint32_t area = 0;
     {
@@ -119,9 +162,8 @@
         }
         s_rect[tid] = rc;
         if (area) {
-            s_con[tid] = co;
+            s_con[tid] = make_float4(co.x, co.y, co.z, __uint_as_float(__float_as_uint(xy.w) & 63u));
             s_xyq[tid] = make_float4(xy.x, xy.y, dqo_q_threshold(co.w), xy.z);
-            s_gobj[tid] = __float_as_int(xy.w);
         }
         s_cnt[tid] = 0;
         s_prev[tid] = 0;
@@ -135,6 +177,9 @@
         if (my_idx < P) g.tiles_touched[my_idx] = 0, g.slot_base[my_idx] = 0;
         return;
     }
+    const int tier = (int)__builtin_amdgcn_readfirstlane((int)s_tier[0]);
+    const uint32_t W32 = (uint32_t)__builtin_amdgcn_readfirstlane((int)s_tier[1]), W32a = (uint32_t)__builtin_amdgcn_readfirstlane((int)s_tier[2]);
+    const uint32_t n_obj = (uint32_t)__builtin_amdgcn_readfirstlane((int)s_tier[3]);
 
     auto decode = [&](uint32_t w) {
         int lo = 0, hi = BIN_CHUNK;
@@ -152,24 +197,45 @@
         c.tile = (int)((miny + ry) * (uint32_t)gx + minx + rx);
         return c;
     };
+    auto cull_tier = [&](auto tier_tag, uint32_t win, uint32_t wend, bool flag_dead) {
+        constexpr int TIER = decltype(tier_tag)::value;
+        for (uint32_t wb = win + ((uint32_t)tid & ~63u); wb < wend; wb += BIN_THREADS) {
+            const uint32_t w = wb + lane;
+            bool live = false;
+            if (w < wend) {
+                const Cand c = decode(w);
+                const uint32_t tw = (uint32_t)c.tile >> 5, tb = 1u << (c.tile & 31);
+                bool unmasked;
+                if constexpr (TIER == 0) unmasked = tile_mask == nullptr || tile_mask[c.tile] != 0;
+                else unmasked = (s_tab[W32a + tw] & tb) != 0u;
+                if (unmasked) {
+                    const float4 co = s_con[c.gi], xyq = s_xyq[c.gi];
+                    const int x = c.tile % gx, y = c.tile / gx;
+                    live = dqo_splat_hits_rect(xyq.x, xyq.y, co.x, co.y, co.z, xyq.z, (float)(x * DQO_TILE), (float)(y * DQO_TILE),
+                                               (float)(x * DQO_TILE + DQO_TILE - 1), (float)(y * DQO_TILE + DQO_TILE - 1));
+                    if (tile_objects != nullptr) {
+                        const uint32_t ob = __float_as_uint(co.w) & 63u;
+                        if constexpr (TIER == 2) live = live && ob < n_obj && (s_tab[W32a + (1u + ob) * W32 + tw] & tb) != 0u;
+                        else live = live && ((tile_objects[c.tile] >> ob) & 1ull) != 0ull;
+                    }
+                    if (!live && flag_dead) {
+                        if constexpr (TIER == 0) {
+                            if (tile_flag[c.tile] == 0u) tile_flag[c.tile] = 1u;
+                        } else if ((atomicOr(&s_tab[tw], tb) & tb) == 0u) {
+                            tile_flag[c.tile] = 1u;
+                        }
+                    }
+                }
+            }
+            const unsigned long long votes = __builtin_amdgcn_ballot_w64(live);
+            if (lane == 0) *reinterpret_cast<uint2*>(&s_bits[(wb - win) >> 5]) = make_uint2((uint32_t)votes, (uint32_t)(votes >> 32));
+        }
+        __syncthreads();
+    };
     auto cull_window = [&](uint32_t win, uint32_t wend, bool flag_dead) {
-        for (int i = tid; i < BIN_WINDOW / 32; i += BIN_THREADS) s_bits[i] = 0;
-        __syncthreads();
-        for (uint32_t w = win + tid; w < wend; w += BIN_THREADS) {
-            const Cand c = decode(w);
-            if (tile_mask != nullptr && !tile_mask[c.tile]) continue;
-            const float4 co = s_con[c.gi], xyq = s_xyq[c.gi];
-            const int x = c.tile % gx, y = c.tile / gx;
-            bool live = dqo_splat_hits_rect(xyq.x, xyq.y, co.x, co.y, co.z, xyq.z, (float)(x * DQO_TILE), (float)(y * DQO_TILE),
-                                            (float)(x * DQO_TILE + DQO_TILE - 1), (float)(y * DQO_TILE + DQO_TILE - 1));
-            if (tile_objects != nullptr) live = live && ((tile_objects[c.tile] >> (s_gobj[c.gi] & 63)) & 1ull) != 0ull;
-            if (live) {
-                atomicOr(&s_bits[(w - win) >> 5], 1u << ((w - win) & 31));
-            } else if (flag_dead && tile_flag[c.tile] == 0u) {
-                tile_flag[c.tile] = 1u;
-            }
-        }
-        __syncthreads();
+        if (tier == 2) cull_tier(TierTag<2>{}, win, wend, flag_dead);
+        else if (tier == 1) cull_tier(TierTag<1>{}, win, wend, flag_dead);
+        else cull_tier(TierTag<0>{}, win, wend, flag_dead);
     };
     auto carry_window = [&](uint32_t win, uint32_t wend, uint32_t* acc) {
         const uint32_t a = max(my_off, win), b = min(my_off + area, wend);
@@ -185,8 +251,7 @@
     }
     const bool no_slots = bin.bucket > 0 && row_flags != nullptr && my_idx < P && (row_flags[my_idx] & DQO_ROW_FROZEN) != 0u;
     const uint32_t my_cnt = no_slots ? 0u : s_cnt[tid];
-    __shared__ uint8_t s_noslot[BIN_CHUNK];
-    s_noslot[tid] = no_slots ? (uint8_t)1 : (uint8_t)0;
+    if (no_slots) s_con[tid].w = __uint_as_float(__float_as_uint(s_con[tid].w) | 64u);
     if (row_flags != nullptr && bin.bucket > 0) {
         const uint32_t nf = dqo_wave_sum_u32(no_slots ? s_cnt[tid] : 0u, (int)lane);
         if (lane == 0 && nf != 0u) atomicAdd(&g.spread[(size_t)((blockIdx.x * (BIN_THREADS / 64) + wave) % DQO_SPREAD) * 64 + 5], nf);
@@ -225,7 +290,7 @@
 
     for (uint32_t win = 0; win < total; win += BIN_WINDOW) {
         const uint32_t wend = min(total, win + (uint32_t)BIN_WINDOW);
-        if (!one_window) cull_window(win, wend, false);
+        if (!one_window) cull_tier(TierTag<0>{}, win, wend, false);
         for (uint32_t w0 = win + tid; w0 < wend; w0 += BIN_THREADS * BIN_FLIGHT) {
             uint32_t slot[BIN_FLIGHT], rank[BIN_FLIGHT];
             int tile[BIN_FLIGHT], gid[BIN_FLIGHT];
@@ -238,7 +303,7 @@
                 if (ok[u]) {
                     const Cand c = decode(w);
                     const uint32_t first = max(s_off[c.gi], win);
-                    slot[u] = s_noslot[c.gi] ? 0xffffffffu : base + s_gb[c.gi] + s_prev[c.gi] + popcount_range(s_bits, first - win, w - win);
+                    slot[u] = (__float_as_uint(s_con[c.gi].w) & 64u) ? 0xffffffffu : base + s_gb[c.gi] + s_prev[c.gi] + popcount_range(s_bits, first - win, w - win);
                     tile[u] = c.tile;
                     gid[u] = dqo_spread_index(chunk0 + c.gi, P);
                     depth[u] = s_xyq[c.gi].w;
@@ -284,13 +349,64 @@
     bin.rec_valid[slot] = 0u;
 }
 
-}
-
-int dqo_launch_bin_count(int P, int gx, const int32_t* tile_mask, const DqoGeomLayout& g, const DqoImageLayout& img, const DqoBinLayout& bin,
+constexpr int TB_THREADS = 1024;
+__global__ __launch_bounds__(TB_THREADS) void tile_bits_build_kernel(int T, const int32_t* __restrict__ tile_mask,
+                                                                     const unsigned long long* __restrict__ tile_objects,
+                                                                     uint32_t* __restrict__ tb) {
+    __shared__ uint32_t s_any[2];
+    const uint32_t tid = threadIdx.x, W32 = ((uint32_t)T + 31u) / 32u;
+    if (tid < 2) s_any[tid] = 0u;
+    __syncthreads();
+    uint32_t n_obj = 0;
+    if (tile_objects != nullptr) {
+        unsigned long long any = 0ull;
+        for (uint32_t t = tid; t < (uint32_t)T; t += TB_THREADS) any |= tile_objects[t];
+        if ((uint32_t)any != 0u) atomicOr(&s_any[0], (uint32_t)any);
+        if ((uint32_t)(any >> 32) != 0u) atomicOr(&s_any[1], (uint32_t)(any >> 32));
+        __syncthreads();
+        const unsigned long long all = (unsigned long long)s_any[0] | ((unsigned long long)s_any[1] << 32);
+        n_obj = all != 0ull ? 64u - (uint32_t)__clzll((long long)all) : 0u;
+    }
+    const uint32_t rows = 1u + n_obj;
+    uint32_t* const out = tb + DQO_TB_HEAD_WORDS;
+    for (uint32_t i = tid; i < rows * W32; i += TB_THREADS) {
+        const uint32_t r = i / W32, w = i - r * W32;
+        uint32_t bits = 0u;
+        for (uint32_t b = 0; b < 32u; b++) {
+            const uint32_t t = w * 32u + b;
+            if (t >= (uint32_t)T) break;
+            const bool on = r == 0u ? (tile_mask == nullptr || tile_mask[t] != 0) : ((tile_objects[t] >> (r - 1u)) & 1ull) != 0ull;
+            bits |= (on ? 1u : 0u) << b;
+        }
+        out[i] = bits;
+    }
+    if (tid < DQO_TB_HEAD_WORDS) {
+        const unsigned long long mp = (unsigned long long)(uintptr_t)tile_mask, op = (unsigned long long)(uintptr_t)tile_objects;
+        uint32_t v = 0u;
+        if (tid == DQO_TB_MAGIC) v = DQO_TB_STAMP;
+        else if (tid == DQO_TB_ROWS) v = rows;
+        else if (tid == DQO_TB_W32) v = W32;
+        else if (tid == DQO_TB_TILES) v = (uint32_t)T;
+        else if (tid == DQO_TB_MASK_LO) v = (uint32_t)mp;
+        else if (tid == DQO_TB_MASK_HI) v = (uint32_t)(mp >> 32);
+        else if (tid == DQO_TB_OBJ_LO) v = (uint32_t)op;
+        else if (tid == DQO_TB_OBJ_HI) v = (uint32_t)(op >> 32);
+        tb[tid] = v;
+    }
+}
+
+}
+
+int dqo_launch_tile_bits_build(const DqoImageLayout& img, int T, const int32_t* tile_mask, const unsigned long long* tile_objects, hipStream_t s) {
+    DQO_LAUNCH("tile_bits_build_kernel", tile_bits_build_kernel, dim3(1), dim3(TB_THREADS), s, T, tile_mask, tile_objects, img.tile_bits);
+    return DQO_OK;
+}
+
+int dqo_launch_bin_count(int P, int gx, int T, const int32_t* tile_mask, const DqoGeomLayout& g, const DqoImageLayout& img, const DqoBinLayout& bin,
                          int64_t capacity, const unsigned long long* tile_objects, hipStream_t s, const uint8_t* row_flags) {
     DqoK1Raw none{};
     DQO_LAUNCH("bin_count_kernel", (bin_count_kernel<false, false>), dim3(dqo_spread_blocks(P)), dim3(BIN_THREADS), s, P, gx, tile_mask, g,
-               img.tile_count, img.tile_flag, bin, capacity, tile_objects, none, row_flags);
+               img.tile_count, img.tile_flag, bin, capacity, tile_objects, none, row_flags, img.tile_bits, T);
     return DQO_OK;
 }
 
@@ -302,7 +418,8 @@
     k1.gobj = gobj, k1.radii_out = out->radii, k1.n_touched_out = out->n_touched;
 #define DQO_BIN_K1(PF)                                                                                                                \
     DQO_LAUNCH(PF ? "bin_count_pf_kernel" : "bin_count_kernel", (bin_count_kernel<true, PF>), dim3(dqo_spread_blocks(v.P)), dim3(BIN_THREADS), \
-               s, v.P, v.gx, in->tile_mask, g, img.tile_count, img.tile_flag, bin, capacity, tile_objects, k1, v.row_flags)
+               s, v.P, v.gx, in->tile_mask, g, img.tile_count, img.tile_flag, bin, capacity, tile_objects, k1, v.row_flags, img.tile_bits,   \
+               v.gx * v.gy)
     if (pf) DQO_BIN_K1(true);
     else DQO_BIN_K1(false);
 #undef DQO_BIN_K1
diff --git a/dqo-map_amd/csrc/rast_forward.hip b/dqo-map_amd/csrc/rast_forward.hip
--- a/dqo-map_amd/csrc/rast_forward.hip
+++ b/dqo-map_amd/csrc/rast_forward.hip
@@ -576,7 +576,7 @@
 int dqo_launch_blend_forward(const DqoView& v, const DqoGeomLayout& g, const DqoImageLayout& img, const DqoBinLayout& bin,
                              const DqoRastOutputs& out, int T, const DqoTapDev& tap, const DqoGateDev& gate, int list_split, hipStream_t s,
                              int64_t header_capacity);
-int dqo_launch_bin_count(int P, int gx, const int32_t* tile_mask, const DqoGeomLayout& g, const DqoImageLayout& img, const DqoBinLayout& bin,
+int dqo_launch_bin_count(int P, int gx, int T, const int32_t* tile_mask, const DqoGeomLayout& g, const DqoImageLayout& img, const DqoBinLayout& bin,
                          int64_t capacity, const unsigned long long* tile_objects, hipStream_t s, const uint8_t* row_flags);
 int dqo_launch_bin_place(const DqoGeomLayout& g, const DqoImageLayout& img, const DqoBinLayout& bin, int64_t capacity, hipStream_t s);
 
@@ -637,7 +637,7 @@
         const unsigned long long* tobj = ctx->object_gate ? reinterpret_cast<const unsigned long long*>(ctx->object_gate->tile_objects) : nullptr;
         int rc = dqo_fuse_k1(p, ctx) ? dqo_launch_bin_count_k1(v, in, out, ctx->object_gate ? ctx->object_gate->gaussian_object : nullptr, g, img,
                                                                bin, cap, tobj, s, pf != nullptr)
-                                     : dqo_launch_bin_count(p->P, v.gx, in->tile_mask, g, img, bin, cap, tobj, s, v.row_flags);
+                                     : dqo_launch_bin_count(p->P, v.gx, T, in->tile_mask, g, img, bin, cap, tobj, s, v.row_flags);
         if (rc) return rc;
     }
     const int keep_order = (bucket > 0 && ctx->keep_tile_order != 0 && p->P > 0) ? 1 : 0;
diff --git a/dqo-map_amd/diff_gaussian_rasterization_depth/__init__.py b/dqo-map_amd/diff_gaussian_rasterization_depth/__init__.py
--- a/dqo-map_amd/diff_gaussian_rasterization_depth/__init__.py
+++ b/dqo-map_amd/diff_gaussian_rasterization_depth/__init__.py
@@ -106,6 +106,7 @@
     cs.cap, cs.bucket = int(cap * 1.2), bucket
     cs.geom = torch.empty((lib.dqo_rast_geom_bytes(key[1], W, H),), **u8)
     cs.img = torch.empty((lib.dqo_rast_image_bytes(W, H),), **u8)
+    N.check(lib.dqo_rast_tile_bits_clear(cs.img.data_ptr(), cs.img.numel(), W, H, stream))
     cs.binning = torch.empty((lib.dqo_rast_binning_bytes_bucketed(cs.cap, W, H, cs.bucket),), **u8)
     cs.order_valid = cs.clean = cs.leased = False
     if not pin:
@@ -341,6 +342,10 @@
         _, _, hit_color, hit_depth, _, _, _, n_touched, radii = out
         geomBuffer = torch.empty((lib.dqo_rast_geom_bytes(P, W, H),), **u8)
         imgBuffer = torch.empty((lib.dqo_rast_image_bytes(W, H),), **u8)
+
+        def own_image(img=imgBuffer):
+            N.check(lib.dqo_rast_tile_bits_clear(img.data_ptr(), img.numel(), W, H, stream))
+
         params = _params(rs, P, M)
         inputs = _inputs(rs, means3D, sh, colors_precomp, opacities, scales, rotations, cov3Ds_precomp, tile_mask, row_flags=row_flags)
         cctx = N.DqoRastCtx(geom=geomBuffer.data_ptr(), geom_bytes=geomBuffer.numel(), binning=None, binning_bytes=0,
@@ -374,6 +379,7 @@
                     pooled.captured = (int(cctx.keep_tile_order), int(cctx.frame_prezeroed))
                 else:
                     binningBuffer = torch.empty((lib.dqo_rast_binning_bytes(cap),), **u8)
+                    own_image()
             cctx.binning, cctx.binning_bytes, cctx.inst_capacity = binningBuffer.data_ptr(), binningBuffer.numel(), cap
             N.check(_forward_call(lib, "async", params, inputs, pinputs, outputs, cctx, None, None, stream))
             _last["header"] = geomBuffer
@@ -384,6 +390,7 @@
         if _sync_mode == "graph":
             pass
         elif cap is None:
+            own_image()
             N.check(_forward_call(lib, "prepare", params, inputs, pinputs, outputs, cctx, stream))
             hdr = N.DqoRastHeader()
             N.check(lib.dqo_rast_read_header(ctypes.byref(cctx), ctypes.byref(hdr), stream))
@@ -423,6 +430,7 @@
                     pooled.clean = False
                 else:
                     binningBuffer = torch.empty((lib.dqo_rast_binning_bytes(cap),), **u8)
+                    own_image()
                 cctx.binning, cctx.binning_bytes, cctx.inst_capacity = binningBuffer.data_ptr(), binningBuffer.numel(), cap
                 host, ev, host_ptr, ev_handle = _ring_slot(dev.index)
                 N.check(_forward_call(lib, "async", params, inputs, pinputs, outputs, cctx, host_ptr, ev_handle, stream))
diff --git a/dqo-map_amd/dqo_harness/fused_mapping.py b/dqo-map_amd/dqo_harness/fused_mapping.py
--- a/dqo-map_amd/dqo_harness/fused_mapping.py
+++ b/dqo-map_amd/dqo_harness/fused_mapping.py
@@ -468,6 +468,7 @@
             out, outputs = dgr._new_outputs(P, H, W, dev)
             c = dict(key=(P, H, W), out=out, outputs=outputs, geom=torch.empty((lib.dqo_rast_geom_bytes(P, W, H),), **u8),
                      img=torch.empty((lib.dqo_rast_image_bytes(W, H),), **u8))
+            N.check(lib.dqo_rast_tile_bits_clear(c["img"].data_ptr(), c["img"].numel(), W, H, stream))
         params = dgr._params(st, P, M)
         inputs = dgr._inputs(st, self.xyz, self.shs, self._empty, self.opacity, self.scales, self.rotations, self._empty, self.tile_mask,
                              row_flags=row_flags)
@@ -946,6 +947,19 @@
         g.adam = self._adam_step_args(gr, radii=g.out[8].data_ptr(), frame_header=g.geom.data_ptr(), step_dev=g.step_dev)
         g.adam.record_ctx = ctypes.addressof(g.cctx)
         g.adam.record_W, g.adam.record_H = int(st.image_width), int(st.image_height)
+        self._build_tile_bits(g)
+
+    def _build_tile_bits(self, g):
+        H, W = int(g.settings.image_height), int(g.settings.image_width)
+        tile_objects = g.tile_objects if self.gaussian_object is not None else None
+        N.check(N.lib().dqo_rast_tile_bits_build(g.img.data_ptr(), g.img.numel(), W, H, N.ptr(g.tile_mask), N.ptr(tile_objects),
+                                                 N.current_stream()))
+
+    def _rebuild_tile_bits(self, written):
+        for g in self._graphs():
+            if g.img is not None and (g.tile_mask.data_ptr() in written or
+                                      (g.tile_objects is not None and g.tile_objects.data_ptr() in written)):
+                self._build_tile_bits(g)
 
     def _warm_up_and_record(self, g, reuse_probe):
         self._step_dev.fill_(self.step_count + 1)
@@ -1080,6 +1094,7 @@
         cams = [self._frames[frame]] + [g for (k, m), g in self._mixed.items() if k == frame]
         masks = [self._frames[frame]] + [g for (k, m), g in self._mixed.items() if m == frame]
         done = set()
+        bits = set()
 
         def once(t):
             if t.data_ptr() in done:
@@ -1100,6 +1115,7 @@
                     g.mask.copy_(render_mask.to(torch.uint8))
             if tile_mask is not None and once(g.tile_mask):
                 g.tile_mask.copy_(_checked_tile_mask(tile_mask, self.device, int(g.settings.image_height), int(g.settings.image_width)))
+                bits.add(g.tile_mask.data_ptr())
         if settings is not None:
             new = _normalised_settings(settings, self.device)
             for g in cams:
@@ -1116,6 +1132,8 @@
                 if once(g.pixel_object):
                     g.pixel_object.copy_(torch.as_tensor(pixel_object).to(self.device, torch.int32).reshape(g.pixel_object.shape))
                     g.tile_objects.copy_(tile_object_sets(g.pixel_object))
+                    bits.add(g.tile_objects.data_ptr())
+        self._rebuild_tile_bits(bits)
         return self
 
     @torch.no_grad()
@@ -1181,6 +1199,7 @@
                         if dst is not None and dst.data_ptr() not in done and dst.data_ptr() != self.tile_mask.data_ptr():
                             done.add(dst.data_ptr())
                             dst.copy_(src.view(dst.shape))
+            self._rebuild_tile_bits(done)
         return table
 
     def capture_placed(self, *args, trials=4, probe_replays=12, **kw):
@@ -1239,6 +1258,8 @@
                              row_flags=self.row_flags)
         cctx = N.DqoRastCtx(geom=geom.data_ptr(), geom_bytes=geom.numel(), binning=None, binning_bytes=0, image=img.data_ptr(),
                             image_bytes=img.numel(), inst_capacity=0)
+        N.check(lib.dqo_rast_tile_bits_build(img.data_ptr(), img.numel(), W, H, N.ptr(tile_mask),
+                                             N.ptr(tile_objects) if self.gaussian_object is not None else None, N.current_stream()))
         if self.gaussian_object is not None:
             gate = N.DqoObjectGate(gaussian_object=N.ptr(self.gaussian_object), pixel_object=N.ptr(pixel_object), tile_objects=N.ptr(tile_objects))
             cctx.object_gate = ctypes.addressof(gate)
diff --git a/include/dqo_raster.h b/include/dqo_raster.h
--- a/include/dqo_raster.h
+++ b/include/dqo_raster.h
@@ -139,6 +139,11 @@
 size_t dqo_rast_binning_bytes(int64_t inst_capacity);
 size_t dqo_rast_binning_bytes_bucketed(int64_t inst_capacity, int32_t W, int32_t H, int32_t tile_bucket_capacity);
 size_t dqo_rast_backward_workspace_bytes(int64_t inst_capacity);
+
+size_t dqo_rast_tile_bits_bytes(int32_t W, int32_t H);
+int dqo_rast_tile_bits_build(void* image, size_t image_bytes, int32_t W, int32_t H, const int32_t* tile_mask, const uint64_t* tile_objects,
+                             void* hipStream);
+int dqo_rast_tile_bits_clear(void* image, size_t image_bytes, int32_t W, int32_t H, void* hipStream);
 
 int dqo_rast_forward_prepare(const DqoRastParams*, const DqoRastInputs*, DqoRastOutputs*, DqoRastCtx*, void* hipStream);
 int dqo_rast_read_header(const DqoRastCtx*, DqoRastHeader* host_out, void* hipStream);
```
